# lmb-freiburg/understanding_flow_robustness

Measured on AMD Instinct MI355X. Metric: attack-iters/s, higher is better.
Workload: dtype f32

## Files before the change

include/ufr_hip.h:

```cpp
#ifndef UFR_HIP_H_
#define UFR_HIP_H_

#include <stdint.h>

#ifdef __cplusplus
extern "C" {
#endif

#define UFR_ABI_VERSION 9

enum { UFR_F32 = 0, UFR_F64 = 1, UFR_F16 = 2 };
enum {
  UFR_OK = 0,
  UFR_EINVAL = -1,
  UFR_EUNSUPPORTED = -2,
  UFR_ELAUNCH = -3
};

typedef void* ufr_stream_t;

int ufr_abi_version(void);
const char* ufr_last_error(void);
int ufr_device_count(void);
const char* ufr_build_manifest(void);
// ... 233 lines not shown
                    ufr_stream_t stream);
int ufr_window_gather(const float* src, float* dst, const int* win, int n_win, int N, int C, int Hs, int Ws,
                      int wh, int ww, int level_stride, int margin, ufr_stream_t stream);
int ufr_window_gather_pair(const float* a, const float* b, float* xw, const int* win, float* zero, int N, int C, int Hs, int Ws,
                           int wh, int ww, ufr_stream_t stream);
int ufr_attack_place(const float* patch, const float* mask_p, const float* patch_init, const int* origins, const int* origins_host,
                     float* patch_dst, float* mask_dst, float* init_dst, float* loaded_dst, int* origins_dst, float* state, int B,
                     int H, int W, int ph, int pw, const ufr_cone_chain* chain, int win_h, int win_w, int* win, int* band_win,
                     int band_width, int band_reach, int corr_width, int corr_reach, ufr_stream_t stream);
int ufr_window_scatter(const float* src, float* dst, const int* win, int n_win, int N, int C, int Hd, int Wd,
                       int wh, int ww, int level_stride, int margin, ufr_stream_t stream);

int ufr_corr_backward_window(const float* input1, const float* input2, const float* grad_output,
                             float* grad_input1, float* grad_input2, int B, int C, int H, int W, int patch,
                             int dilation_patch, const int* win, int level_stride, int wh, int ww,
                             ufr_stream_t stream);

int ufr_bias_leaky_forward(float* x, const float* bias, int B, int C, long HW, float slope, ufr_stream_t stream);
int ufr_leaky_backward(const float* y, const float* grad_y, float* grad_x, long total, float slope,
                       ufr_stream_t stream);

long ufr_conv3x3_c2_workspace_floats(int B, int Cin, int H, int W);
int ufr_conv3x3_c2_forward(const float* x, const float* weight, const float* bias, float* y, float* workspace,
                           int B, int Cin, int H, int W, ufr_stream_t stream);
int ufr_conv3x3_c2_backward_data(const float* grad_y, const float* weight, float* grad_x, int B, int Cin, int H,
                                 int W, ufr_stream_t stream);
int ufr_deconv4x4s2_c2_forward(const float* x, const float* weight, const float* bias, float* y, int B, int H, int W,
                               ufr_stream_t stream);
int ufr_deconv4x4s2_c2_backward_data(const float* grad_y, const float* weight, float* grad_x, int B, int H, int W,
                                     ufr_stream_t stream);

int ufr_affine_resample_f64(const double* src, double* dst, int C, int Hs, int Ws, int Hd, int Wd,
                            double m00, double m01, double m10, double m11, double off0, double off1,
                            int order, ufr_stream_t stream);
int ufr_patch_place(const double* patch, const double* mask, const double* init, int C, int h, int w,
                    float* canvas_patch, float* canvas_mask, float* canvas_init, int H, int W, int y, int x,
                    ufr_stream_t stream);
int ufr_patch_crop_f64(const float* canvas, const float* factor, double* dst, int C, int H, int W, int y,
                       int x, int h, int w, ufr_stream_t stream);

int ufr_resample_u8_horizontal(const unsigned char* src, unsigned char* dst, int H, int Ws, int Wd, int C, int flip,
                               const int* bounds, const int* kk, int ksize, ufr_stream_t stream);
int ufr_resample_u8_vertical(const unsigned char* src, unsigned char* dst, int Hs, int Hd, int W, int C,
                             const int* bounds, const int* kk, int ksize, ufr_stream_t stream);
int ufr_u8_to_tensor(const unsigned char* src, float* dst, int H, int W, int C, int crop_y, int crop_x, int crop_h,
                     int crop_w, float divisor, ufr_stream_t stream);
int ufr_kitti_flow_decode(const unsigned short* src, float* dst, int H, int W, ufr_stream_t stream);

int ufr_host_png_unfilter(const unsigned char* data, unsigned char* out, int rows, int stride, int bpp);

#define UFR_IGEMM_MAX_TAPS 25
typedef struct {
  int ntaps, oy0, ox0;
  long w_off;
  signed char dy[UFR_IGEMM_MAX_TAPS], dx[UFR_IGEMM_MAX_TAPS];
} ufr_igemm_phase;
typedef struct {
  const void* x; long x_plane_stride; int in_chunk0, KC;
  int B, Hi, Wi, in_sy, in_sx;
  const int* in_x0; int in_x0_stride, in_x0_div, in_xw;
  const void* w; long w_plane_stride; int Npad, N;
  int Hr, Wr;
  const int* row_x0; int row_x0_stride, row_x0_div;
  int Ho, Wo, out_sy, out_sx;
  int nphase;
  ufr_igemm_phase phase[4];
  int act; const float* bias; float slope;
  const float* add; int add_chunk0;
  const void* mask; int mask_chunk0;
  void* out_planes; long out_plane_stride; int out_chunk0;
  float* out_f32; int out_f32_chunk0;
  float* tail; int tail_n0, tail_accumulate;
  int splitk; float* ws;
  int products;
  int variant;
  int k_order;
  float* out_rowmajor; long out_ld;
  int planes_chunks, f32_first_chunk;
  int no_reduce;
  int* tickets;
} ufr_igemm_desc;
int ufr_igemm(const ufr_igemm_desc* d, ufr_stream_t stream);
typedef struct {
  const void* x; long x_plane_stride; int in_chunk0, C;
  const void* gy; long gy_plane_stride; int g_chunk0, N;
  int B, Hi, Wi, Ho, Wo, kh, kw, sy, sx, py, px;
  float* dw;
  float* db;
  int accumulate;
  int splitm; float* ws; long ws_elems;
  int products;
} ufr_igemm_wgrad_desc;
int ufr_igemm_wgrad(const ufr_igemm_wgrad_desc* d, ufr_stream_t stream);
int ufr_igemm_wgrad_dilated(const ufr_igemm_wgrad_desc* d, int dy, int dx, ufr_stream_t stream);
int ufr_igemm_variant_fallbacks(void);
int ufr_igemm_clock_probe(unsigned long long* buf, int capacity_workgroups);
int ufr_rowmajor_to_planes(const float* src, long ld, long rows, int cols, float scale, void* planes, long plane_stride, int chunk0,
                           long plane_rows, ufr_stream_t stream);
int ufr_nchw_to_planes(const float* x, void* planes, long plane_stride, int chunk0, int B, int C, int H, int W,
                       float scale, float slope, const float* bias, ufr_stream_t stream);
int ufr_window_scatter_planes(const float* src, void* planes, long plane_stride, int chunk0, const int* win, int n_win,
                              int N, int C, int Hd, int Wd, int wh, int ww, int level_stride, int margin,
                              ufr_stream_t stream);
int ufr_window_features_planes(const void* c2w, long c2w_stride, const void* c3w, long c3w_stride, void* cat2, long cat2_stride,
                               void* c3a, long c3a_stride, void* c3b, long c3b_stride, float* c3_nchw, float* c3w_nchw,
                               const int* win, int B, int H, int W, int wh, int ww, int m2, int m3, ufr_stream_t stream);
int ufr_chunks_to_nchw(const void* planes, long plane_stride, const float* f32, int chunk0, const void* mask,
                       int mask_chunk0, float* out, int B, int C, int H, int W, float scale, float slope,
                       ufr_stream_t stream);
int ufr_nchw_cat_to_planes(const float* const* srcs, const int* channels, const int* dst_channel0, int nseg, void* planes,
                           long plane_stride, int chunk0, int chunks, int B, int H, int W, ufr_stream_t stream);
int ufr_chunks_to_nchw_cat(const float* g, int chunk0, int chunks, float* const* dsts, const int* channels, const int* src_channel0,
                           int nseg, const float* act0, float pos0, float neg0, int B, int H, int W, ufr_stream_t stream);
int ufr_grad_finalize(const float* g, int g_chunk0, const void* mask, int mask_chunk0, void* out, long out_plane_stride,
                      int out_chunk0, long M, int chunks, float slope, ufr_stream_t stream);

int ufr_conv1_direct(const float* frames_a, const float* frames_b, int Ba, int Bb, int H, int W, const double* mean,
                     const void* wimg, const float* bias, float slope, void* out_planes, long plane_stride, int out_chunk0,
                     ufr_stream_t stream);
int ufr_conv1_pack_planes(const float* frames_a, const float* frames_b, void* planes, long plane_stride, int Ba, int Bb, int H,
                          int W, const double* mean, ufr_stream_t stream);
int ufr_conv1_unpack_grad(const float* G, float* grad_frames, int N, int H, int W, ufr_stream_t stream);
int ufr_unshuffle_pack_planes(const float* x, void* planes, long plane_stride, int N, int C, int H, int W, ufr_stream_t stream);
int ufr_unshuffle_unpack_grad(const float* G, float* grad_x, int N, int C, int H, int W, ufr_stream_t stream);
int ufr_nchw_grad_to_planes(const float* grad, const float* act, void* planes, long plane_stride, int chunk0, int B, int C, int H,
                            int W, float slope, ufr_stream_t stream);
int ufr_window_gather_chunks(const float* src, float* dst, const int* win, int n_win, int N, int N_dst, int chunks, int Hs, int Ws,
                             int wh, int ww, int level_stride, int margin, ufr_stream_t stream);

int ufr_normalize_frames(const float* frames_a, const float* frames_b, float* out, int Ba, int Bb, int C, int H, int W,
                         const double* mean, ufr_stream_t stream);

int ufr_corr_forward_planes_window(const void* f1_planes, const void* f2_planes, long in_plane_stride, void* out_planes,
                                   long out_plane_stride, int out_chunk0, int B, int C, int H, int W, int patch,
                                   int dilation_patch, float scale, float slope, const int* win, int level_stride,
                                   int win_cells, ufr_stream_t stream);

int ufr_corr_forward_planes_changed(const void* f1_planes, const void* f2_planes, long in_plane_stride, void* out_planes,
                                    long out_plane_stride, int out_chunk0, int B, int C, int H, int W, int patch,
                                    int dilation_patch, float scale, float slope, const int* win, int level_stride,
                                    int win_cells_h, int win_cells_w, int margin, ufr_stream_t stream);

int ufr_corr_backward_window_fused(const float* f1, const float* f2, const float* G, int g_chunk0, float g_scale,
                                   const float* G_redir, float* grad_window, int B, int C, int H, int W, int patch,
                                   int dilation_patch, const int* win, int level_stride, int wh, int ww, int margin,
                                   ufr_stream_t stream);

int ufr_corr_forward_planes(const void* f1_planes, const void* f2_planes, long in_plane_stride, void* out_planes,
                            long out_plane_stride, int out_chunk0, int B, int C, int H, int W, int patch,
                            int dilation_patch, float scale, float slope, ufr_stream_t stream);
int ufr_flow_head_planes_forward(const void* planes, long plane_stride, int chunk0, int chunks, const float* wpk, int w_chunks,
                                 const float* bias, float* out, int B, int H, int W, ufr_stream_t stream);
int ufr_flow_head_planes_forward_mfma(const void* planes, long plane_stride, int chunk0, int chunks, const void* wmf, int w_chunks,
                                      const float* bias, float* out, int B, int H, int W, ufr_stream_t stream);
int ufr_deconv_flow_tail_backward_mfma(const void* grad_planes, long plane_stride, int chunk0, int chunks, const void* wmf,
                                       int w_chunks, float* G, int g_chunks, int out_chunk, int B, int H, int W, ufr_stream_t stream);
int ufr_flow_head_planes_backward(const float* grad_y, const float* wpk, int w_chunks, float* G, int g_chunks, int chunk0, int chunks,
                                  int B, int H, int W, int accumulate, ufr_stream_t stream);
int ufr_flow_head_planes_backward_finalize(const float* grad_y, const float* wpk, int w_chunks, float* G, int g_chunks, int chunk0,
                                           int chunks, int B, int H, int W, int accumulate, const void* mask_planes, void* out_planes,
                                           long out_plane_stride, int fin_chunk0, int fin_chunks, float slope, ufr_stream_t stream);
#define UFR_PF_REGION_BAND 1
#define UFR_PF_REGION_WINDOW 2
int ufr_flow_head_planes_backward_regions(const float* grad_y, const float* wpk, int w_chunks, float* G, int g_chunks, int chunk0,
                                          int chunks, int B, int H, int W, int accumulate, int head_chunks, int region,
                                          const int* origin, int origin_stride, int origin_div, int reg_h, int reg_w, int margin,
// ... 70 lines not shown
```

understanding_flow_robustness_amd/_lib.py:

```python
from __future__ import annotations

import ctypes as C
import os

import torch

_HERE = os.path.dirname(os.path.abspath(__file__))
LIB_PATH = os.environ.get("UFR_HIP_LIB") or os.path.join(_HERE, "lib", "libufr_hip.so")
UFR_F32, UFR_F64, UFR_F16 = 0, 1, 2
ABI_VERSION = 9
_lib = None


class CorrParams(C.Structure):
    _fields_ = [(n, C.c_int) for n in (
        "kH", "kW", "patchH", "patchW", "padH", "padW", "dilationH", "dilationW",
        "dilation_patchH", "dilation_patchW", "dH", "dW")]


UFR_MAX_LEVELS = 8


class Pyramid(C.Structure):
    _fields_ = [("num_levels", C.c_int),
                ("vol", C.c_void_p * UFR_MAX_LEVELS),
                ("grad_vol", C.c_void_p * UFR_MAX_LEVELS),
                ("Hl", C.c_int * UFR_MAX_LEVELS),
                ("Wl", C.c_int * UFR_MAX_LEVELS)]


class AltCorrLevels(C.Structure):
    _fields_ = [("num_levels", C.c_int), ("fmap2", C.c_void_p * 4), ("fmap2_grad", C.c_void_p * 4),
                ("H2", C.c_int * 4), ("W2", C.c_int * 4), ("coord_scale", C.c_float * 4)]


class AltCorrPlaneLevels(C.Structure):
    _fields_ = [("num_levels", C.c_int), ("planes", C.c_void_p * 4), ("plane_stride", C.c_long * 4),
                ("H2", C.c_int * 4), ("W2", C.c_int * 4), ("coord_scale", C.c_float * 4)]


UFR_IGEMM_MAX_TAPS = 25


class IgemmPhase(C.Structure):
    _fields_ = [("ntaps", C.c_int), ("oy0", C.c_int), ("ox0", C.c_int), ("w_off", C.c_long),
                ("dy", C.c_byte * UFR_IGEMM_MAX_TAPS), ("dx", C.c_byte * UFR_IGEMM_MAX_TAPS)]


class IgemmDesc(C.Structure):
    _fields_ = [("x", C.c_void_p), ("x_plane_stride", C.c_long), ("in_chunk0", C.c_int), ("KC", C.c_int),
                ("B", C.c_int), ("Hi", C.c_int), ("Wi", C.c_int), ("in_sy", C.c_int), ("in_sx", C.c_int),
                ("in_x0", C.c_void_p), ("in_x0_stride", C.c_int), ("in_x0_div", C.c_int), ("in_xw", C.c_int),
                ("w", C.c_void_p), ("w_plane_stride", C.c_long), ("Npad", C.c_int), ("N", C.c_int),
                ("Hr", C.c_int), ("Wr", C.c_int),
                ("row_x0", C.c_void_p), ("row_x0_stride", C.c_int), ("row_x0_div", C.c_int),
                ("Ho", C.c_int), ("Wo", C.c_int), ("out_sy", C.c_int), ("out_sx", C.c_int),
                ("nphase", C.c_int),
                ("phase", IgemmPhase * 4),
                ("act", C.c_int), ("bias", C.c_void_p), ("slope", C.c_float),
                ("add", C.c_void_p), ("add_chunk0", C.c_int),
                ("mask", C.c_void_p), ("mask_chunk0", C.c_int),
                ("out_planes", C.c_void_p), ("out_plane_stride", C.c_long), ("out_chunk0", C.c_int),
                ("out_f32", C.c_void_p), ("out_f32_chunk0", C.c_int),
                ("tail", C.c_void_p), ("tail_n0", C.c_int), ("tail_accumulate", C.c_int),
                ("splitk", C.c_int), ("ws", C.c_void_p),
                ("products", C.c_int), ("variant", C.c_int), ("k_order", C.c_int),
                ("out_rowmajor", C.c_void_p), ("out_ld", C.c_long),
                ("planes_chunks", C.c_int), ("f32_first_chunk", C.c_int), ("no_reduce", C.c_int),
                ("tickets", C.c_void_p)]


UFR_IGEMM_WGRAD_MAX_TAPS = 49


class IgemmWgradDesc(C.Structure):
    _fields_ = [("x", C.c_void_p), ("x_plane_stride", C.c_long), ("in_chunk0", C.c_int), ("C", C.c_int),
                ("gy", C.c_void_p), ("gy_plane_stride", C.c_long), ("g_chunk0", C.c_int), ("N", C.c_int),
                ("B", C.c_int), ("Hi", C.c_int), ("Wi", C.c_int), ("Ho", C.c_int), ("Wo", C.c_int),
                ("kh", C.c_int), ("kw", C.c_int), ("sy", C.c_int), ("sx", C.c_int), ("py", C.c_int), ("px", C.c_int),
                ("dw", C.c_void_p), ("db", C.c_void_p), ("accumulate", C.c_int),
                ("splitm", C.c_int), ("ws", C.c_void_p), ("ws_elems", C.c_long),
                ("products", C.c_int)]


UFR_TRAIN_LOSS_MAX_SCALES = 8


class TrainLossDesc(C.Structure):
    _fields_ = [("gt", C.c_void_p), ("B", C.c_int), ("H", C.c_int), ("W", C.c_int), ("nscale", C.c_int),
                ("pred", C.c_void_p * UFR_TRAIN_LOSS_MAX_SCALES), ("grad", C.c_void_p * UFR_TRAIN_LOSS_MAX_SCALES),
                ("h", C.c_int * UFR_TRAIN_LOSS_MAX_SCALES), ("w", C.c_int * UFR_TRAIN_LOSS_MAX_SCALES),
                ("weight", C.c_double * UFR_TRAIN_LOSS_MAX_SCALES),
                ("kind", C.c_int), ("div_flow", C.c_double),
                ("ws", C.c_void_p), ("ws_elems", C.c_long), ("out", C.c_void_p)]


class AdamwSeg(C.Structure):
    _fields_ = [("p", C.c_void_p), ("g", C.c_void_p), ("m", C.c_void_p), ("v", C.c_void_p), ("n", C.c_long)]


class AdamwHyper(C.Structure):
    _fields_ = [(n, C.c_double) for n in ("lr", "beta1", "beta2", "eps", "weight_decay", "bias1", "bias2")]


class FeatureStatsSeg(C.Structure):
    _fields_ = [("src", C.c_void_p), ("plane_stride", C.c_long), ("pixels", C.c_long), ("kind", C.c_int), ("images", C.c_int),
                ("image0", C.c_int), ("B", C.c_int), ("chunk0", C.c_int), ("channels", C.c_int), ("unleaky", C.c_double),
                ("out_col", C.c_long)]


UFR_FEATURE_STATS_MAX_SEGS = 32
UFR_MAX_CONE_LAYERS = 8
UFR_PF_REGION_BAND, UFR_PF_REGION_WINDOW = 1, 2


class ConeChain(C.Structure):
    _fields_ = [("n_layers", C.c_int),
                ("kernel", C.c_int * UFR_MAX_CONE_LAYERS), ("stride", C.c_int * UFR_MAX_CONE_LAYERS),
                ("pad", C.c_int * UFR_MAX_CONE_LAYERS),
                ("n_taps", C.c_int),
                ("tap_layer", C.c_int * UFR_MAX_CONE_LAYERS), ("tap_margin", C.c_int * UFR_MAX_CONE_LAYERS)]


_vp, _i, _f, _l, _d = C.c_void_p, C.c_int, C.c_float, C.c_long, C.c_double
LOSS_PARTIALS = 1024
SIGNATURES = {
    "ufr_corr_forward": [_vp, _vp, _vp, _i, _i, _i, _i, _i, C.POINTER(CorrParams), _vp],
    "ufr_corr_forward_fused": [_vp, _vp, _vp, _i, _i, _i, _i, _i, C.POINTER(CorrParams), _f, _f, _vp],
    "ufr_corr_backward": [_vp, _vp, _vp, _vp, _vp, _i, _i, _i, _i, _i, C.POINTER(CorrParams), _vp],
    "ufr_altcorr_forward": [_vp, _vp, _vp, _vp, _i, _i, _i, _i, _i, _i, _i, _i, _vp],
    "ufr_altcorr_backward": [_vp, _vp, _vp, _vp, _vp, _vp, _vp, _i, _i, _i, _i, _i, _i, _i, _i, _vp],
    "ufr_corr_lookup_forward": [C.POINTER(Pyramid), _vp, _vp, _i, _i, _i, _i, _vp],
    "ufr_corr_lookup_backward": [C.POINTER(Pyramid), _vp, _vp, _i, _i, _i, _i, _vp],
    "ufr_resample2d_forward": [_vp, _vp, _vp, _i, _i, _i, _i, _i, _i, _i, _i, _vp],
    "ufr_resample2d_backward_owner": [_vp, _vp, _vp, _vp, _vp, _vp, _l, _i, _i, _i, _i, _vp],
    "ufr_resample2d_backward": [_vp, _vp, _vp, _vp, _vp, _i, _i, _i, _i, _i, _i, _i, _i, _vp],
    "ufr_channelnorm_forward": [_vp, _vp, _i, _i, _i, _i, _i, _vp],
    "ufr_channelnorm_backward": [_vp, _vp, _vp, _vp, _i, _i, _i, _i, _i, _vp],
    "ufr_patch_paste": [_vp, _vp, _vp, _vp, _vp, _vp, _i, _i, _l, _l, _i, _f, _f, _vp],
    "ufr_patch_update": [_vp, _vp, _vp, _vp, _vp, _vp, _vp, _vp, _i, _i, _l, _l, _f, _f, _f, _f, _vp, _vp],
    "ufr_attack_gate": [_vp, _vp, _f, _vp],
    "ufr_gru_gates_forward": [_vp, _vp, _vp, _vp, _i, _i, _i, _l, _vp],
    "ufr_gru_gates_backward": [_vp, _vp, _vp, _vp, _vp, _vp, _i, _i, _i, _l, _vp],
    "ufr_gru_blend_forward": [_vp, _vp, _vp, _vp, _l, _vp],
    "ufr_gru_blend_backward": [_vp, _vp, _vp, _vp, _vp, _vp, _vp, _l, _vp],
    "ufr_flow_loss_ex": [_vp, _vp, _vp, _vp, _i, _i, _i, _i, _f, _vp, _vp, _vp],
    "ufr_universal_update": [_vp, _vp, _vp, _vp, _vp, _vp, _vp, _vp, _i, _i, _f, _f, _f, _f, _i, _i, _i, _i,
                             _i, _vp],
    "ufr_flow_loss": [_vp, _vp, _vp, _vp, _i, _i, _i, _f, _vp, _vp],
    "ufr_flow2_upsampled_loss": [_vp, _f, _vp, _vp, _vp, _i, _i, _i, _i, _f, _vp, _vp],
    "ufr_patch_grad_crop": [_vp, _vp, _vp, _vp, _vp, _vp, _vp, _i, _i, _i, _i, _i, _i, _vp],
    "ufr_patch_apply": [_vp, _i, _vp, _vp, _i, _i, _f, _f, _vp, _vp],
    "ufr_patch_grad_crop_window": [_vp, _vp, _vp, _vp, _vp, _vp, _i, _i, _i, _i, _i, _i, _i, _i, _vp],
    "ufr_patch_paste_placed_rect": [_vp, _vp, _vp, _vp, _vp, _vp, _vp, _i, _i, _i, _i, _i, _i, _f, _f, _vp, _vp],
    "ufr_patch_paste_placed": [_vp, _vp, _vp, _vp, _vp, _vp, _vp, _vp, _vp, _i, _i, _i, _i, _i, _i, _f, _f, _vp, _vp],
    "ufr_cone_window": [_vp, _i, _l, _i, _i, _i, C.POINTER(ConeChain), _i, _i, _vp, _vp, _vp],
    "ufr_attack_place": [_vp, _vp, _vp, _vp, _vp, _vp, _vp, _vp, _vp, _vp, _vp, _i, _i, _i, _i, _i, C.POINTER(ConeChain), _i, _i,
                         _vp, _vp, _i, _i, _i, _i, _vp],
    "ufr_attack_load_frames": [_vp, _vp, _vp, _vp, _vp, _vp, _vp, _vp, _vp, _i, _i, _i, _i, _i, _vp],
    "ufr_patch_mask_placed": [_vp, _vp, _vp, _i, _i, _i, _i, _i, _vp],
    "ufr_patch_grad_crop_packed": [_vp, _vp, _vp, _vp, _vp, _vp, _i, _i, _i, _i, _i, _i, _i, _i, _vp],
    "ufr_patch_apply_paste_rect": [_vp, _i, _vp, _vp, _vp, _vp, _vp, _vp, _vp, _vp, _i, _i, _i, _i, _i, _f, _f, _i, _f, _f, _vp, _vp],
    "ufr_window_gather_pair": [_vp, _vp, _vp, _vp, _vp, _i, _i, _i, _i, _i, _i, _vp],
    "ufr_window_features_planes": [_vp, _l, _vp, _l, _vp, _l, _vp, _l, _vp, _l, _vp, _vp, _vp, _i, _i, _i, _i, _i, _i, _i, _vp],
    "ufr_window_gather": [_vp, _vp, _vp, _i, _i, _i, _i, _i, _i, _i, _i, _i, _vp],
    "ufr_window_scatter": [_vp, _vp, _vp, _i, _i, _i, _i, _i, _i, _i, _i, _i, _vp],
    "ufr_conv1_pack_planes": [_vp, _vp, _vp, _l, _i, _i, _i, _i, _vp, _vp],
    "ufr_conv1_unpack_grad": [_vp, _vp, _i, _i, _i, _vp],
    "ufr_nchw_grad_to_planes": [_vp, _vp, _vp, _l, _i, _i, _i, _i, _i, _f, _vp],
    "ufr_window_gather_chunks": [_vp, _vp, _vp, _i, _i, _i, _i, _i, _i, _i, _i, _i, _i, _vp],
    "ufr_normalize_frames": [_vp, _vp, _vp, _i, _i, _i, _i, _i, _vp, _vp],
    "ufr_corr_backward_window_fused": [_vp, _vp, _vp, _i, _f, _vp, _vp, _i, _i, _i, _i, _i, _i, _vp, _i, _i, _i, _i, _vp],
    "ufr_corr_backward_window": [_vp, _vp, _vp, _vp, _vp, _i, _i, _i, _i, _i, _i, _vp, _i, _i, _i, _vp],
    "ufr_bias_leaky_forward": [_vp, _vp, _i, _i, _l, _f, _vp],
    "ufr_leaky_backward": [_vp, _vp, _vp, _l, _f, _vp],
    "ufr_conv3x3_c2_forward": [_vp, _vp, _vp, _vp, _vp, _i, _i, _i, _i, _vp],
    "ufr_conv3x3_c2_backward_data": [_vp, _vp, _vp, _i, _i, _i, _i, _vp],
    "ufr_deconv4x4s2_c2_forward": [_vp, _vp, _vp, _vp, _i, _i, _i, _vp],
    "ufr_deconv4x4s2_c2_backward_data": [_vp, _vp, _vp, _i, _i, _i, _vp],
    "ufr_pwc_warp_forward": [_vp, _vp, _vp, _i, _i, _i, _i, _vp],
    "ufr_pwc_warp_backward": [_vp, _vp, _vp, _vp, _vp, _i, _i, _i, _i, _vp],
    "ufr_pwc_warp_backward_owner": [_vp, _vp, _vp, _vp, _vp, _vp, _l, _i, _i, _i, _i, _vp],
    "ufr_raft_normalize_pair": [_vp, _vp, _vp, _l, _vp],
    "ufr_raft_normalize_pair_backward": [_vp, _vp, _vp, _l, _vp],
    "ufr_raft_fmap_pyramid_forward": [_vp, _vp, _i, _i, _i, _i, _i, _vp],
    "ufr_raft_fmap_pyramid_backward": [_vp, _i, _vp, _i, _i, _i, _i, _vp],
    "ufr_raft_context_split_forward": [_vp, _vp, _vp, _i, _i, _i, _l, _vp],
    "ufr_raft_context_split_backward": [_vp, _vp, _vp, _vp, _vp, _i, _i, _i, _l, _vp],
    "ufr_igemm": [C.POINTER(IgemmDesc), _vp],
    "ufr_igemm_wgrad": [C.POINTER(IgemmWgradDesc), _vp],
    "ufr_igemm_wgrad_dilated": [C.POINTER(IgemmWgradDesc), _i, _i, _vp],
    "ufr_flow_upscale4_forward": [_vp, _vp, _i, _i, _i, _i, _f, _i, _vp],
    "ufr_flow_upscale4_backward": [_vp, _vp, _i, _i, _i, _i, _f, _i, _vp],
    "ufr_fn2_stage_pack": [_vp, _vp, _vp, _vp, _i, _i, _i, _f, _vp],
    "ufr_fn2_stage_unpack_grad": [_vp, _vp, _vp, _vp, _i, _i, _i, _vp],
    "ufr_fn2_stage_finish_grad": [_vp, _vp, _vp, _vp, _vp, _i, _i, _i, _f, _vp],
    "ufr_fn2_fusion_pack": [_vp, _vp, _vp, _vp, _vp, _vp, _i, _i, _i, _vp],
    "ufr_fn2_fusion_unpack_grad": [_vp, _vp, _vp, _vp, _vp, _vp, _vp, _vp, _vp, _i, _i, _i, _vp],
    "ufr_fn2_fusion_finish_grad": [_vp, _vp, _vp, _vp, _vp, _vp, _vp, _i, _i, _i, _vp],
    "ufr_rowmajor_to_planes": [_vp, _l, _l, _i, _f, _vp, _l, _i, _l, _vp],
    "ufr_nchw_to_planes": [_vp, _vp, _l, _i, _i, _i, _i, _i, _f, _f, _vp, _vp],
    "ufr_window_scatter_planes": [_vp, _vp, _l, _i, _vp, _i, _i, _i, _i, _i, _i, _i, _i, _i, _vp],
    "ufr_chunks_to_nchw": [_vp, _l, _vp, _i, _vp, _i, _vp, _i, _i, _i, _i, _f, _f, _vp],
    "ufr_nchw_cat_to_planes": [_vp, _vp, _vp, _i, _vp, _l, _i, _i, _i, _i, _i, _vp],
    "ufr_chunks_to_nchw_cat": [_vp, _i, _i, _vp, _vp, _vp, _i, _vp, _f, _f, _i, _i, _i, _vp],
    "ufr_grad_finalize": [_vp, _i, _vp, _i, _vp, _l, _i, _l, _i, _f, _vp],
    "ufr_flow_head_planes_forward": [_vp, _l, _i, _i, _vp, _i, _vp, _vp, _i, _i, _i, _vp],
    "ufr_flow_head_planes_forward_mfma": [_vp, _l, _i, _i, _vp, _i, _vp, _vp, _i, _i, _i, _vp],
    "ufr_deconv_flow_tail_backward_mfma": [_vp, _l, _i, _i, _vp, _i, _vp, _i, _i, _i, _i, _i, _vp],
    "ufr_flow_head_planes_backward": [_vp, _vp, _i, _vp, _i, _i, _i, _i, _i, _i, _i, _vp],
    "ufr_flow_head_planes_backward_finalize": [_vp, _vp, _i, _vp, _i, _i, _i, _i, _i, _i, _i, _vp, _vp, _l, _i, _i, _f, _vp],
    "ufr_flow_head_planes_backward_regions": [_vp, _vp, _i, _vp, _i, _i, _i, _i, _i, _i, _i, _i, _i, _vp, _i, _i, _i, _i, _i, _vp, _i,
                                              _vp, _vp, _l, _i, _i, _f, _vp],
    "ufr_unshuffle_pack_planes": [_vp, _vp, _l, _i, _i, _i, _i, _vp],
    "ufr_unshuffle_unpack_grad": [_vp, _vp, _i, _i, _i, _i, _vp],
    "ufr_conv3x3s2_c3_planes": [_vp, _vp, _vp, _f, _vp, _l, _i, _i, _i, _i, _i, _vp],
    "ufr_conv3x3_c16_planes": [_vp, _l, _i, _vp, _vp, _f, _vp, _l, _i, _i, _i, _i, _vp],
    "ufr_cm_norm_stats": [_vp, _vp, _vp, _l, _i, _i, _f, _vp],
    "ufr_cm_norm_apply": [_vp, _vp, _vp, _l, _i, _vp, _l, _i, _l, _i, _i, _i, _i, _vp],
    "ufr_cm_norm_stats_apply": [_vp, _vp, _vp, _f, _vp, _l, _i, _vp, _l, _i, _l, _i, _i, _i, _i, _vp],
    "ufr_cm_norm_backward": [_vp, _vp, _vp, _i, _vp, _vp, _vp, _vp, _l, _i, _l, _i, _i, _i, _vp],
    "ufr_cm_masked_copy": [_vp, _vp, _l, _vp, _l, _vp],
    "ufr_raft_flow_patches": [_vp, _vp, _l, _i, _i, _i, _i, _vp],
    "ufr_raft_motion_finish_slabs": [_vp, _i, _i, _i, _vp, _f, _vp, _l, _vp, _l, _i, _vp, _i, _i, _i, _vp],
    "ufr_raft_motion_finish": [_vp, _l, _vp, _l, _i, _vp, _i, _i, _i, _vp],
    "ufr_raft_coords_step": [_vp, _vp, _vp, _vp, _vp, _l, _vp],
    "ufr_grad_finalize_consume": [_vp, _vp, _vp, _l, _l, _i, _f, _vp],
    "ufr_gru_gates_cm_forward": [_vp, _vp, _l, _i, _vp, _l, _i, _l, _i, _vp],
    "ufr_gru_gates_cm_forward_slabs": [_vp, _i, _i, _vp, _vp, _vp, _vp, _l, _i, _vp, _l, _i, _l, _i, _vp],
    "ufr_gru_blend_cm_forward_slabs": [_vp, _i, _i, _vp, _vp, _vp, _vp, _vp, _l, _i, _vp, _l, _i, _l, _i, _vp],
    "ufr_gru_blend_cm_forward": [_vp, _vp, _vp, _l, _i, _vp, _l, _i, _l, _i, _vp],
    "ufr_gru_blend_cm_backward": [_vp, _vp, _vp, _l, _i, _vp, _vp, _l, _i, _vp, _vp, _l, _i, _vp, _vp],
    "ufr_gru_gates_cm_backward": [_vp, _vp, _l, _i, _vp, _vp, _vp, _l, _i, _vp, _l, _i, _i, _vp, _vp],
    "ufr_altcorr_pyramid_forward": [_vp, _vp, _vp, _vp, _i, _i, _i, _i, _i, _f, _vp],
    "ufr_altcorr_pyramid_backward": [_vp, _vp, _vp, _vp, _vp, _vp, _i, _i, _i, _i, _i, _f, _i, _vp],
    "ufr_altcorr_pyramid_backward_cm": [_vp, _vp, _vp, _vp, _vp, _vp, _i, _i, _i, _i, _i, _f, _i, _vp],
    "ufr_upfeat_planes_forward_mfma": [_vp, _l, _i, _i, _vp, _i, _vp, _vp, _i, _i, _i, _vp],
    "ufr_upfeat_planes_backward": [_vp, _vp, _i, _vp, _i, _i, _i, _i, _i, _i, _i, _vp],
    "ufr_flow_up_planes_forward": [_vp, _vp, _vp, _vp, _l, _i, _i, _i, _i, _vp],
    "ufr_flow_up_planes_backward": [_vp, _i, _vp, _vp, _i, _i, _i, _i, _vp],
    "ufr_corr_forward_planes_changed": [_vp, _vp, _l, _vp, _l, _i, _i, _i, _i, _i, _i, _i, _f, _f, _vp, _i, _i, _i, _i, _vp],
    "ufr_corr_forward_planes_window": [_vp, _vp, _l, _vp, _l, _i, _i, _i, _i, _i, _i, _i, _f, _f, _vp, _i, _i, _vp],
    "ufr_corr_forward_planes": [_vp, _vp, _l, _vp, _l, _i, _i, _i, _i, _i, _i, _i, _f, _f, _vp],
    "ufr_convex_upsample_forward": [_vp, _vp, _vp, _i, _i, _i, _vp],
    "ufr_convex_upsample_backward": [_vp, _vp, _vp, _vp, _vp, _vp, _i, _i, _i, _vp],
    "ufr_affine_resample_f64": [_vp, _vp, _i, _i, _i, _i, _i, _d, _d, _d, _d, _d, _d, _i, _vp],
    "ufr_patch_place": [_vp, _vp, _vp, _i, _i, _i, _vp, _vp, _vp, _i, _i, _i, _i, _vp],
    "ufr_patch_crop_f64": [_vp, _vp, _vp, _i, _i, _i, _i, _i, _i, _i, _vp],
    "ufr_resample_u8_horizontal": [_vp, _vp, _i, _i, _i, _i, _i, _vp, _vp, _i, _vp],
    "ufr_resample_u8_vertical": [_vp, _vp, _i, _i, _i, _i, _vp, _vp, _i, _vp],
    "ufr_u8_to_tensor": [_vp, _vp, _i, _i, _i, _i, _i, _i, _i, _f, _vp],
    "ufr_kitti_flow_decode": [_vp, _vp, _i, _i, _vp],
    "ufr_host_png_unfilter": [_vp, _vp, _i, _i, _i],
    "ufr_igemm_clock_probe": [_vp, _i],
    "ufr_altcorr_planes_prepare": [_vp, _vp, _l, _l, _i, _vp],
    "ufr_altcorr_planes_forward": [_vp, _l, C.POINTER(AltCorrPlaneLevels), _vp, _vp, _i, _i, _i, _i, _i, _f, _vp],
    "ufr_conv1_direct": [_vp, _vp, _i, _i, _i, _i, _vp, _vp, _vp, _f, _vp, _l, _i, _vp],
    "ufr_train_loss": [C.POINTER(TrainLossDesc), _vp],
    "ufr_grad_norm": [C.POINTER(AdamwSeg), _i, _f, _vp, _l, _vp, _vp],
    "ufr_adamw_step": [C.POINTER(AdamwSeg), _i, C.POINTER(AdamwHyper), _vp, _vp],
    "ufr_sweep_paste": [_vp, _vp, _vp, _vp, _vp, _vp, _vp, _vp, _i, _i, _i, _i, _i, _f, _f, C.POINTER(ConeChain), _i, _i, _vp, _vp, _vp],
    "ufr_sweep_metrics": [_vp, _vp, _vp, _vp, _vp, _i, _i, _i, _i, _i, _i, _i, _i, _vp, _l, _vp, _i, _i, _vp],
    "ufr_feature_stats": [C.POINTER(FeatureStatsSeg), _i, _vp, _l, _vp, _i, _l, _l, _vp],
    "ufr_abs_sums": [_vp, _vp, _l, _vp, _l, _vp, _vp],
    "ufr_momentum_update": [_vp, _vp, _vp, _vp, _vp, _vp, _vp, _vp, _vp, _vp, _i, _i, _f, _f, _f, _f, _f, _f, _i, _i, _vp],
    "ufr_diverse_table_check": [_vp, _i, _i, _i],
    "ufr_diverse_forward": [_vp, _vp, _vp, _vp, _vp, _vp, _i, _i, _i, _i, _vp, _i, _vp, _vp, _vp, _l, _vp],
    "ufr_diverse_backward": [_vp, _vp, _vp, _vp, _i, _i, _i, _vp, _i, _vp, _vp],
    "ufr_step_advance": [_vp, _vp],
}
DIVERSE_COLS = 8
PLAIN = {"ufr_abi_version": (C.c_int, []), "ufr_last_error": (C.c_char_p, []),
# ... 276 lines not shown
```

understanding_flow_robustness_amd/csrc/igemm.hip:

```cpp
#include <atomic>
#include <cstdlib>

#include "ufr_common.h"

namespace {

typedef __attribute__((ext_vector_type(8))) __bf16 bf16x8;
typedef __attribute__((ext_vector_type(4))) float f32x4;
typedef __attribute__((ext_vector_type(4))) unsigned u32x4;

constexpr int BM = 128, BN = 128, BK = 32;
__device__ constexpr int PROD_A[6] = {2, 0, 1, 1, 0, 0};
__device__ constexpr int PROD_B[6] = {0, 2, 1, 0, 1, 0};

struct RowGeom {
  int B, Hr, Wr, M;
  const int* row_x0;
  int row_x0_stride, row_x0_div;
  int Ho, Wo, out_sy, out_sx;
};

__device__ __forceinline__ void split3(float v, __bf16& a, __bf16& b, __bf16& c) {
  a = (__bf16)v;
  const float r1 = v - (float)a;
// ... 74 lines not shown
    }
#pragma unroll
    for (int j = 0; j < 8; ++j) {
      v[j] += (n0 + j < e.N) ? e.bias[n0 + j] : 0.f;
      v[j] = v[j] > 0.f ? v[j] : v[j] * e.slope;
    }
  } else {
    if (e.add) {
      const float* ap = e.add + (long)e.add_chunk0 * e.Mout * 32 + cm;
      const float4 a0 = *reinterpret_cast<const float4*>(ap), a1 = *reinterpret_cast<const float4*>(ap + 4);
      v[0] += a0.x; v[1] += a0.y; v[2] += a0.z; v[3] += a0.w; v[4] += a1.x; v[5] += a1.y; v[6] += a1.z; v[7] += a1.w;
    }
    if (e.mask) {
      const bf16x8 m = *reinterpret_cast<const bf16x8*>(e.mask + (long)e.mask_chunk0 * e.Mout * 32 + cm);
#pragma unroll
      for (int j = 0; j < 8; ++j) v[j] = ((float)m[j] > 0.f) ? v[j] : v[j] * e.slope;
    }
  }
#pragma unroll
  for (int j = 0; j < 8; ++j)
    if (n0 + j >= e.N) v[j] = 0.f;
  if (e.out_rm && n0 < e.N) {
    float* op = e.out_rm + pout * e.out_ld + n0;
    *reinterpret_cast<float4*>(op) = make_float4(v[0], v[1], v[2], v[3]);
    *reinterpret_cast<float4*>(op + 4) = make_float4(v[4], v[5], v[6], v[7]);
  }
  if (e.out_f32 && (n0 >> 5) >= e.f32_first_chunk) {
    float* op = e.out_f32 + (long)e.out_f32_chunk0 * e.Mout * 32 + cm;
    *reinterpret_cast<float4*>(op) = make_float4(v[0], v[1], v[2], v[3]);
    *reinterpret_cast<float4*>(op + 4) = make_float4(v[4], v[5], v[6], v[7]);
  }
  if (e.out_planes && (n0 >> 5) < e.planes_chunks) {
    bf16x8 q0, q1, q2;
#pragma unroll
    for (int j = 0; j < 8; ++j) {
      __bf16 x, y, z;
      split3(v[j], x, y, z);
      q0[j] = x; q1[j] = y; q2[j] = z;
    }
    __bf16* o = e.out_planes + (long)e.out_chunk0 * e.Mout * 32 + cm;
    if (e.nostore) {
      asm volatile("" ::"v"(q0), "v"(q1), "v"(q2), "v"(o));
      return;
    }
    *reinterpret_cast<bf16x8*>(o) = q0;
    *reinterpret_cast<bf16x8*>(o + e.out_plane_stride) = q1;
    *reinterpret_cast<bf16x8*>(o + 2 * e.out_plane_stride) = q2;
  }
}

__device__ __forceinline__ void xcd_tile(int swz, int& bx, int& by, int& bz) {
  bx = blockIdx.x; by = blockIdx.y; bz = blockIdx.z;
  if (!swz) return;
  const int nx = gridDim.x, nxy = nx * gridDim.y, n = nxy * gridDim.z;
  const int orig = (bz * gridDim.y + by) * nx + bx;
  const int q = n / 8, r = n % 8, xcd = orig % 8, idx = orig / 8;
  const int w = (xcd < r ? xcd * (q + 1) : r * (q + 1) + (xcd - r) * q) + idx;
  bz = w % gridDim.z;
  const int rem = w / gridDim.z;
  by = rem / nx;
  bx = rem - by * nx;
}

struct Phase {
  int ntaps, oy0, ox0;
  long w_off;
  int dyx[UFR_IGEMM_MAX_TAPS];
  int run[UFR_IGEMM_MAX_TAPS];
};

struct Args {
  const __bf16* x; long x_plane_stride; int in_chunk0, KC;
  int Hi, Wi, in_sy, in_sx;
  const int* in_x0; int in_x0_stride, in_x0_div, in_xw;
  const __bf16* w; long w_plane_stride; int Npad;
  RowGeom g;
  Epilogue e;
  int nphase, splitk, xcd;
  int korder;
  int per_k, sk[4], zoff[4];
  float* ws;
  int* tickets;
  int skip_out;
  Phase ph[4];
};

__device__ __forceinline__ void sum_slabs(const float* src, long sstride, int S, float (&v)[8]) {
#pragma unroll
  for (int j = 0; j < 8; ++j) v[j] = 0.f;
  int s = 0;
  for (; s + 8 <= S; s += 8) {
    float4 lo[8], hi[8];
#pragma unroll
    for (int u = 0; u < 8; ++u) {
      lo[u] = *reinterpret_cast<const float4*>(src + (s + u) * sstride);
      hi[u] = *reinterpret_cast<const float4*>(src + (s + u) * sstride + 4);
    }
#pragma unroll
    for (int u = 0; u < 8; ++u) {
      v[0] += lo[u].x; v[1] += lo[u].y; v[2] += lo[u].z; v[3] += lo[u].w; v[4] += hi[u].x; v[5] += hi[u].y; v[6] += hi[u].z; v[7] += hi[u].w;
    }
  }
  if (S - s >= 5) {
    float4 lo[7], hi[7];
#pragma unroll
    for (int u = 0; u < 7; ++u) {
      const int su = min(s + u, S - 1);
      lo[u] = *reinterpret_cast<const float4*>(src + su * sstride);
      hi[u] = *reinterpret_cast<const float4*>(src + su * sstride + 4);
    }
#pragma unroll
    for (int u = 0; u < 7; ++u)
      if (s + u < S) {
        v[0] += lo[u].x; v[1] += lo[u].y; v[2] += lo[u].z; v[3] += lo[u].w; v[4] += hi[u].x; v[5] += hi[u].y; v[6] += hi[u].z; v[7] += hi[u].w;
      }
    s = S;
  }
  for (; s + 4 <= S; s += 4) {
    float4 lo[4], hi[4];
#pragma unroll
    for (int u = 0; u < 4; ++u) {
      lo[u] = *reinterpret_cast<const float4*>(src + (s + u) * sstride);
      hi[u] = *reinterpret_cast<const float4*>(src + (s + u) * sstride + 4);
    }
#pragma unroll
    for (int u = 0; u < 4; ++u) {
      v[0] += lo[u].x; v[1] += lo[u].y; v[2] += lo[u].z; v[3] += lo[u].w; v[4] += hi[u].x; v[5] += hi[u].y; v[6] += hi[u].z; v[7] += hi[u].w;
    }
  }
  for (; s < S; ++s) {
    const float4 lo = *reinterpret_cast<const float4*>(src + s * sstride), hi = *reinterpret_cast<const float4*>(src + s * sstride + 4);
    v[0] += lo.x; v[1] += lo.y; v[2] += lo.z; v[3] += lo.w; v[4] += hi.x; v[5] += hi.y; v[6] += hi.z; v[7] += hi.w;
  }
}

template <int NPL, int MT, int WGR, int BNT>
__device__ __forceinline__ void igemm_write_out(const Args& a, const Phase& ph, f32x4 (&acc)[MT][4], float* lds_f32, int* flag, int z, int phase,
                                                int tile_id, int bm0, int bm, int bn0, int bn, int wrow, int wcol, int lane, int wave) {
  if (a.skip_out) {
    float keep = 0.f;
#pragma unroll
    for (int m = 0; m < MT; ++m)
#pragma unroll
      for (int n = 0; n < 4; ++n) keep += acc[m][n][0] + acc[m][n][1] + acc[m][n][2] + acc[m][n][3];
    if (keep == 1.2345678e-30f && a.ws) a.ws[0] = keep;
    return;
  }
  if (a.splitk > 1) {
    float* slab = a.ws + (long)z * a.g.M * a.Npad;
#pragma unroll
    for (int m = 0; m < MT; ++m)
#pragma unroll
      for (int j = 0; j < 4; ++j) {
        const int row = bm + wrow + m * 16 + (lane >> 4) * 4 + j;
        if (row < a.g.M) {
#pragma unroll
          for (int n = 0; n < 4; ++n) slab[(long)row * a.Npad + bn + wcol + n * 16 + (lane & 15)] = acc[m][n][j];
        }
      }
    if (!a.tickets) return;
    asm volatile("s_waitcnt vmcnt(0)" ::: "memory");
    __syncthreads();
    if (threadIdx.x == 0) {
      __builtin_amdgcn_fence(__ATOMIC_RELEASE, "agent");
      asm volatile("s_waitcnt vmcnt(0)" ::: "memory");
      const int S = a.sk[phase];
      const int t = __hip_atomic_fetch_add(a.tickets + tile_id, 1, __ATOMIC_RELAXED, __HIP_MEMORY_SCOPE_AGENT);
      const int last = t == S - 1;
      if (last) {
        __hip_atomic_store(a.tickets + tile_id, 0, __ATOMIC_RELAXED, __HIP_MEMORY_SCOPE_AGENT);
        __builtin_amdgcn_fence(__ATOMIC_ACQUIRE, "agent");
        asm volatile("s_waitcnt vmcnt(0)" ::: "memory");
      }
      *flag = last;
    }
    __syncthreads();
    if (!*flag) return;
    const float* base = a.ws + (long)a.zoff[phase] * a.g.M * a.Npad;
    const long sstride = (long)a.g.M * a.Npad;
    const int S = a.sk[phase];
    for (int it = threadIdx.x; it < WGR * (BNT / 8); it += blockDim.x) {
      const int r = it / (BNT / 8), n0 = bn0 + (it - r * (BNT / 8)) * 8, row = bm0 + r;
      if (row >= a.g.M || n0 >= a.e.Nchunks32 * 32) continue;
      float v[8];
      sum_slabs(base + (long)row * a.Npad + n0, sstride, S, v);
      epilogue_store8(a.e, out_pixel(a.g, row, ph.oy0, ph.ox0), n0, v);
    }
    return;
  }
  {
    constexpr int TS = 68;
    float* tw = lds_f32 + wave * (32 * TS);
#pragma unroll
    for (int pass = 0; pass < MT / 2; ++pass) {
      __syncthreads();
#pragma unroll
      for (int mm = 0; mm < 2; ++mm)
#pragma unroll
        for (int n = 0; n < 4; ++n)
#pragma unroll
          for (int j = 0; j < 4; ++j)
            tw[(mm * 16 + (lane >> 4) * 4 + j) * TS + n * 16 + (lane & 15)] = acc[pass * 2 + mm][n][j];
      __syncthreads();
#pragma unroll
      for (int it = 0; it < 4; ++it) {
        const int item = it * 64 + lane, r = item >> 3, g8 = item & 7;
        const int row = bm + wrow + pass * 32 + r;
        if (row < a.g.M) {
          const float4 lo = *reinterpret_cast<const float4*>(tw + r * TS + g8 * 8), hi = *reinterpret_cast<const float4*>(tw + r * TS + g8 * 8 + 4);
          float v[8] = {lo.x, lo.y, lo.z, lo.w, hi.x, hi.y, hi.z, hi.w};
          epilogue_store8(a.e, out_pixel(a.g, row, ph.oy0, ph.ox0), bn + wcol + g8 * 8, v);
        }
      }
    }
  }
}

__device__ __attribute__((aligned(64))) unsigned ufr_zero_page[16];

__device__ unsigned long long* ufr_clock_probe_buf = nullptr;
__device__ int ufr_clock_probe_cap = 0;

__device__ __forceinline__ void glds16(const __bf16* src, __bf16* lds_wave_base) {
  __builtin_amdgcn_global_load_lds(src, lds_wave_base, 16, 0, 0);
}

template <int BM_, int BN_, bool PIPE_ = false, bool BUF_ = false, int NP_ = 6>
__global__ __launch_bounds__(256) __attribute__((amdgpu_waves_per_eu(PIPE_ ? 2 : (BM_ == 64 ? 4 : 3), PIPE_ ? 2 : (BM_ == 64 ? 4 : 3)))) void igemm_glds_kernel(const Args a) {
  static_assert(!(PIPE_ && BUF_), "the buffer-resource form exists for the single-stage kernel");
  static_assert(NP_ == 6 || NP_ == 3 || NP_ == 1, "six, three or one product");
  constexpr int NPL = NP_ == 6 ? 3 : (NP_ == 3 ? 2 : 1), FIRST = 6 - NP_;
  constexpr int MT = (BN_ == 128 && BM_ == 128) ? 4 : 2;
// ... 116 lines not shown
    for (int n = 0; n < 4; ++n) acc[m][n] = f32x4{0.f, 0.f, 0.f, 0.f};
  const int frow = lane & 15;
  const int foff = frow * BK + ((((lane >> 4)) ^ ((frow >> 1) & 3)) << 3);

  if (kt0 < kt1) set_tap(tap);
  if constexpr (PIPE_) {
    if (kt0 < kt1) {
      stage_A(0);
      stage_B();
    }
    for (int kt = kt0; kt < kt1; ++kt) {
      const int cur = (kt - kt0) & 1;
      asm volatile("s_waitcnt vmcnt(0)" ::: "memory");
      __builtin_amdgcn_s_barrier();
      __builtin_amdgcn_s_setprio(2);
      const __bf16* sA = lds_all + (cur ? STAGE : 0);
      bf16x8 fa[NPL][MT], fb[4][NPL];
#pragma unroll
      for (int p = 0; p < NPL; ++p) {
#pragma unroll
        for (int m = 0; m < MT; ++m) fa[p][m] = *reinterpret_cast<const bf16x8*>(sA + p * (BM_ * BK) + (wrow + m * 16) * BK + foff);
#pragma unroll
        for (int n = 0; n < 4; ++n) fb[n][p] = *reinterpret_cast<const bf16x8*>(&ldsB[p][(wcol + n * 16) * BK + foff]);
      }
      if (kt + 1 < kt1) stage_A(cur ? 0 : STAGE);
      asm volatile("s_waitcnt lgkmcnt(0)" ::: "memory");
      __builtin_amdgcn_s_barrier();
      if (kt + 1 < kt1) stage_B();
      __builtin_amdgcn_s_setprio(0);
#pragma unroll
      for (int n = 0; n < 4; ++n)
#pragma unroll
        for (int t = FIRST; t < 6; ++t)
#pragma unroll
          for (int m = 0; m < MT; ++m)
            acc[m][n] = __builtin_amdgcn_mfma_f32_16x16x32_bf16(fa[PROD_A[t]][m], fb[n][PROD_B[t]], acc[m][n], 0, 0, 0);
    }
  } else
  for (int kt = kt0; kt < kt1; ++kt) {
    __syncthreads();
    stage_tile();
    __syncthreads();
    bf16x8 fa[NPL][MT];
#pragma unroll
    for (int p = 0; p < NPL; ++p)
#pragma unroll
      for (int m = 0; m < MT; ++m)
        fa[p][m] = *reinterpret_cast<const bf16x8*>(&ldsA[p][(wrow + m * 16) * BK + foff]);
#pragma unroll
    for (int n = 0; n < 4; ++n) {
      bf16x8 fb[NPL];
#pragma unroll
      for (int p = 0; p < NPL; ++p) fb[p] = *reinterpret_cast<const bf16x8*>(&ldsB[p][(wcol + n * 16) * BK + foff]);
#pragma unroll
      for (int t = FIRST; t < 6; ++t)
#pragma unroll
        for (int m = 0; m < MT; ++m)
          acc[m][n] = __builtin_amdgcn_mfma_f32_16x16x32_bf16(fa[PROD_A[t]][m], fb[PROD_B[t]], acc[m][n], 0, 0, 0);
    }
  }
  static_assert(PIPE_ ? 4 * 32 * 68 * 4 <= STAGE * 2 : true, "epilogue staging does not fit");
  igemm_write_out<NPL, MT, BM_, BN_>(a, ph, acc, reinterpret_cast<float*>(lds_all), reinterpret_cast<int*>(lds_all), z, phase,
                                     (phase * gridDim.y + ty) * gridDim.x + tx, bm, bm, bn, bn, wrow, wcol, lane, wave);
}
constexpr int PIPE_LDS_BYTES = (3 * (128 + 128) * BK + 3 * 128 * BK) * 2;

constexpr int PP_IMG = 3 * 128 * BK;
constexpr int pp_lds_bytes(int bn) { return (4 * PP_IMG + 2 * 3 * bn * BK) * 2; }

template <int BN_, bool BUF_ = false, int NP_ = 6>
__global__ __launch_bounds__(512) __attribute__((amdgpu_waves_per_eu(2, 2))) void igemm_pp_kernel(const Args a) {
  static_assert(NP_ == 6 || NP_ == 3 || NP_ == 1, "six, three or one product");
  constexpr int NPL = NP_ == 6 ? 3 : (NP_ == 3 ? 2 : 1), FIRST = 6 - NP_;
  constexpr int MT = BN_ == 128 ? 4 : 2, BPT = BN_ / 64;
  constexpr int PP_IMG_B = 3 * BN_ * BK;
  extern __shared__ __attribute__((aligned(16))) __bf16 lds_pp[];
  unsigned long long* const probe = ufr_clock_probe_buf;
  const unsigned long long probe_c0 = probe ? __builtin_amdgcn_s_memtime() : 0, probe_r0 = probe ? __builtin_amdgcn_s_memrealtime() : 0;
  const int tid = threadIdx.x & 255, lane = tid & 63;
  const int wave = __builtin_amdgcn_readfirstlane(tid >> 6);
  const int grp = __builtin_amdgcn_readfirstlane(threadIdx.x >> 8);
  const int wrow = BN_ == 128 ? (wave >> 1) * 64 : wave * 32, wcol = BN_ == 128 ? (wave & 1) * 64 : 0;
  int tx, ty, z;
  xcd_tile(a.xcd, tx, ty, z);
  const int bm = ty * 256 + grp * 128, bn = tx * BN_;
  int phase = 0;
#pragma unroll
  for (int p = 1; p < 4; ++p)
    if (p < a.nphase && z >= a.zoff[p]) phase = p;
  const int ks = z - a.zoff[phase];
  const Phase& ph = a.ph[phase];
  const int KC = a.KC, KT = ph.ntaps * KC;
  const int kt0 = ks * a.per_k, kt1 = min(KT, kt0 + a.per_k);
  const int nk = max(kt1 - kt0, 0);
  const long Min = (long)a.g.B * a.Hi * a.Wi;
  const long cstride = Min * 32;

  const int srow0 = tid >> 2, sch = tid & 3;
  const int csw = sch ^ ((srow0 >> 1) & 3);
  int yb[2], xb[2], xlo[2], xhi[2];
  long ibase[2];
#pragma unroll
  for (int i = 0; i < 2; ++i) {
    const int pm = bm + srow0 + 64 * i;
    const int hw = a.g.Hr * a.g.Wr;
    const int b = pm / hw, r = pm - b * hw, yr = r / a.g.Wr, xr = r - yr * a.g.Wr;
    const bool live = pm < a.g.M;
    const int bb = live ? b : 0;
    const int xg = xr + (a.g.row_x0 ? a.g.row_x0[bb * a.g.row_x0_stride] / a.g.row_x0_div : 0);
    yb[i] = live ? yr * a.in_sy : -(1 << 20);
    xb[i] = xg * a.in_sx;
    ibase[i] = (long)bb * a.Hi * a.Wi;
    xlo[i] = a.in_x0 ? a.in_x0[bb * a.in_x0_stride] / a.in_x0_div : 0;
    xhi[i] = a.in_x0 ? min(a.Wi, xlo[i] + a.in_xw) : a.Wi;
    xlo[i] = max(xlo[i], 0);
  }
  const __bf16* gx = a.x + (long)a.in_chunk0 * cstride + csw * 8;
  const __bf16* zero = reinterpret_cast<const __bf16*>(ufr_zero_page);
  int tap = a.korder ? kt0 % ph.ntaps : kt0 / KC, kc = a.korder ? kt0 / ph.ntaps : kt0 - tap * KC;
  const __bf16* wp = a.w + ph.w_off + ((long)kt0 * a.Npad + bn + srow0) * BK + csw * 8;
  const long wstep = (long)a.Npad * BK;
  const __bf16* xk = gx + (long)kc * cstride;
  bool ok[2];
  long aoff[2];
  unsigned voff[2];
  const unsigned rowbase[2] = {(unsigned)(ibase[0] * 64 + csw * 16), (unsigned)(ibase[1] * 64 + csw * 16)};
  __amdgpu_buffer_rsrc_t rsrc = __builtin_amdgcn_make_buffer_rsrc(const_cast<__bf16*>(a.x), 0, (int)min(6L * a.x_plane_stride, 0x7fffffffL),
                                                                   0x00020000);
  long xkoff = (long)(a.in_chunk0 + kc) * cstride;
  auto set_tap = [&](int t) {
    const int dyx = ph.dyx[t], dyo = (int)(short)(dyx & 0xffff), dxo = dyx >> 16;
#pragma unroll
    for (int i = 0; i < 2; ++i) {
      const int yi = yb[i] + dyo, xi = xb[i] + dxo;
      ok[i] = (unsigned)yi < (unsigned)a.Hi && xi >= xlo[i] && xi < xhi[i];
      if (BUF_) voff[i] = ok[i] ? rowbase[i] + (unsigned)(yi * a.Wi + xi) * 64u : 0x80000000u;
      else aoff[i] = ok[i] ? (ibase[i] + (long)yi * a.Wi + xi) * 32 : 0;
    }
  };
  const int imgA0 = grp * 2 * PP_IMG, imgB0 = 4 * PP_IMG;
  auto stage_A = [&](int img) {
#pragma unroll
    for (int i = 0; i < 2; ++i)
#pragma unroll
      for (int p = 0; p < NPL; ++p) {
        if (BUF_) {
          typedef __attribute__((address_space(3))) void* lds_void;
          __builtin_amdgcn_raw_ptr_buffer_load_lds(rsrc, (lds_void)(lds_pp + img + p * (128 * BK) + (64 * i + wave * 16) * BK), 16, (int)voff[i],
                                                   (unsigned)((xkoff + p * a.x_plane_stride) * 2), 0, 0);
        } else {
          const __bf16* src = ok[i] ? xk + aoff[i] + p * a.x_plane_stride : zero;
          glds16(src, lds_pp + img + p * (128 * BK) + (64 * i + wave * 16) * BK);
        }
      }
    if (a.korder) {
      if (++tap == ph.ntaps) {
        tap = 0;
        xk += cstride;
        xkoff += cstride;
      }
      set_tap(tap);
    } else {
      xk += cstride;
      xkoff += cstride;
      if (++kc == KC) {
        kc = 0;
        xk = gx;
        xkoff = (long)a.in_chunk0 * cstride;
        if (++tap < ph.ntaps) set_tap(tap);
      }
    }
  };
  auto stage_B = [&](int img) {
#pragma unroll
    for (int i = 0; i < BPT; ++i)
#pragma unroll
      for (int p = 0; p < NPL; ++p)
        glds16(wp + p * a.w_plane_stride + (long)(64 * i) * BK, lds_pp + img + p * (BN_ * BK) + (64 * i + wave * 16) * BK);
    wp += wstep;
  };

  f32x4 acc[MT][4];
#pragma unroll
  for (int m = 0; m < MT; ++m)
#pragma unroll
    for (int n = 0; n < 4; ++n) acc[m][n] = f32x4{0.f, 0.f, 0.f, 0.f};
  const int frow = lane & 15;
  const int foff = frow * BK + ((((lane >> 4)) ^ ((frow >> 1) & 3)) << 3);

  if (nk > 0) {
    set_tap(tap);
    stage_A(imgA0);
    if (grp == 0) stage_B(imgB0);
  }
  if (grp == 1) {
    asm volatile("s_waitcnt vmcnt(0)" ::: "memory");
    __builtin_amdgcn_s_barrier();
  }
  const unsigned long long probe_c2 = probe ? __builtin_amdgcn_s_memtime() : 0;
  for (int i = 0; i < nk; ++i) {
    const int cur = i & 1;
    asm volatile("s_waitcnt vmcnt(0)" ::: "memory");
    __builtin_amdgcn_s_barrier();
    __builtin_amdgcn_s_setprio(2);
    const __bf16* sA = lds_pp + imgA0 + cur * PP_IMG;
    const __bf16* sB = lds_pp + imgB0 + cur * PP_IMG_B;
    bf16x8 fa[NPL][MT], fb[4][NPL];
#pragma unroll
    for (int p = 0; p < NPL; ++p) {
#pragma unroll
      for (int m = 0; m < MT; ++m) fa[p][m] = *reinterpret_cast<const bf16x8*>(sA + p * (128 * BK) + (wrow + m * 16) * BK + foff);
#pragma unroll
      for (int n = 0; n < 4; ++n) fb[n][p] = *reinterpret_cast<const bf16x8*>(sB + p * (BN_ * BK) + (wcol + n * 16) * BK + foff);
    }
    if (i + 1 < nk) {
      stage_A(imgA0 + (cur ^ 1) * PP_IMG);
      if (grp == 0) stage_B(imgB0 + (cur ^ 1) * PP_IMG_B);
    }
    asm volatile("s_waitcnt lgkmcnt(0)" ::: "memory");
    __builtin_amdgcn_s_setprio(0);
    __builtin_amdgcn_s_barrier();
#pragma unroll
    for (int n = 0; n < 4; ++n)
#pragma unroll
      for (int t = FIRST; t < 6; ++t)
#pragma unroll
        for (int m = 0; m < MT; ++m)
          acc[m][n] = __builtin_amdgcn_mfma_f32_16x16x32_bf16(fa[PROD_A[t]][m], fb[n][PROD_B[t]], acc[m][n], 0, 0, 0);
  }
  if (grp == 0) __builtin_amdgcn_s_barrier();
  const unsigned long long probe_c3 = probe ? __builtin_amdgcn_s_memtime() : 0;
  static_assert(4 * 32 * 68 * 4 <= 2 * PP_IMG * 2, "epilogue staging does not fit a group's activation images");
  igemm_write_out<NPL, MT, 256, BN_>(a, ph, acc, reinterpret_cast<float*>(lds_pp + imgA0), reinterpret_cast<int*>(lds_pp), z, phase,
                                     (phase * gridDim.y + ty) * gridDim.x + tx, ty * 256, bm, bn, bn, wrow, wcol, lane, wave);
  if (probe && threadIdx.x == 0) {
    const int wg = (blockIdx.z * gridDim.y + blockIdx.y) * gridDim.x + blockIdx.x;
    if (wg < ufr_clock_probe_cap) {
      unsigned long long* o = probe + 8L * wg;
      o[0] = probe_c0; o[1] = __builtin_amdgcn_s_memtime(); o[2] = probe_r0; o[3] = __builtin_amdgcn_s_memrealtime();
      o[4] = probe_c2; o[5] = probe_c3; o[6] = __builtin_amdgcn_s_getreg((4 << 0) | (0 << 6) | (31 << 11)); o[7] = (unsigned long long)nk;
    }
  }
}

constexpr int PP3_ROWS = 144;
constexpr int PP3_IMG = 3 * PP3_ROWS * BK;
constexpr int pp3_lds_bytes(int bn) { return (4 * PP3_IMG + 2 * 3 * bn * BK) * 2; }

template <int BN_>
__global__ __launch_bounds__(512) __attribute__((amdgpu_waves_per_eu(2, 2))) void igemm_pp3_kernel(const Args a) {
  constexpr int NPL = 3, MT = BN_ == 128 ? 4 : 2, BPT = BN_ / 64, PP_IMG_B = 3 * BN_ * BK;
  extern __shared__ __attribute__((aligned(16))) __bf16 lds_pp[];
  const int tid = threadIdx.x & 255, lane = tid & 63, wave = __builtin_amdgcn_readfirstlane(tid >> 6);
  const int grp = __builtin_amdgcn_readfirstlane(threadIdx.x >> 8);
  const int wrow = BN_ == 128 ? (wave >> 1) * 64 : wave * 32, wcol = BN_ == 128 ? (wave & 1) * 64 : 0;
  int tx, ty, z;
  xcd_tile(a.xcd, tx, ty, z);
  const int bm = ty * 256 + grp * 128, bn = tx * BN_;
  int phase = 0;
#pragma unroll
  for (int p = 1; p < 4; ++p)
    if (p < a.nphase && z >= a.zoff[p]) phase = p;
  const int ks = z - a.zoff[phase];
  const Phase& ph = a.ph[phase];
  const int ntaps = ph.ntaps, KT = ntaps * a.KC;
  const int kt0 = ks * a.per_k, kt1 = min(KT, kt0 + a.per_k);
  const int nk = max(kt1 - kt0, 0);
  const long Min = (long)a.g.B * a.Hi * a.Wi;
  const long cstride = Min * 32;
  const int Wr = a.g.Wr, hw = a.g.Hr * Wr;

  const int srow0 = tid >> 2, sch = tid & 3;
  const int csw = sch ^ ((srow0 >> 1) & 3);
  const int xrow = lane >> 2, cswx = sch ^ ((xrow >> 1) & 3);
  int yb[3], xb[3], xlo[3], xhi[3];
  long ibase[3];
  auto cell_geometry = [&](int i, long cell, int xr_override) {
    const bool live = cell >= 0 && cell < a.g.M;
    const int c = live ? (int)cell : 0;
    const int b = c / hw, r = c - b * hw, yr = r / Wr;
    const int xr = xr_override >= 0 ? xr_override : r - yr * Wr;
    const int xg = xr + (a.g.row_x0 ? a.g.row_x0[b * a.g.row_x0_stride] / a.g.row_x0_div : 0);
    yb[i] = live ? yr * a.in_sy : -(1 << 20);
    xb[i] = xg * a.in_sx;
    ibase[i] = (long)b * a.Hi * a.Wi;
    xlo[i] = a.in_x0 ? a.in_x0[b * a.in_x0_stride] / a.in_x0_div : 0;
    xhi[i] = a.in_x0 ? min(a.Wi, xlo[i] + a.in_xw) : a.Wi;
    xlo[i] = max(xlo[i], 0);
  };
  cell_geometry(0, (long)bm + srow0, -1);
  cell_geometry(1, (long)bm + srow0 + 64, -1);
  const int grow0 = bm / Wr;
  if (xrow < 2) {
    cell_geometry(2, (long)bm + 128 + xrow, -1);
  } else {
    const int e = (xrow - 2) >> 1, w = (xrow - 2) & 1;
    const long rowcell = (long)(grow0 + e) * Wr;
    cell_geometry(2, rowcell < a.g.M ? rowcell : -1, Wr + w);
  }
  const __bf16* gx = a.x + (long)a.in_chunk0 * cstride + csw * 8;
  const __bf16* gxx = a.x + (long)a.in_chunk0 * cstride + cswx * 8;
  const __bf16* zero = reinterpret_cast<const __bf16*>(ufr_zero_page);
  const __bf16* wp = a.w + ph.w_off + ((long)kt0 * a.Npad + bn + srow0) * BK + csw * 8;
  const long wstep = (long)a.Npad * BK;

  const int imgA0 = grp * 2 * PP3_IMG, imgB0 = 4 * PP3_IMG;
  auto stage_A = [&](int img, int kc, int tap) {
    const int dyx = ph.dyx[tap], dyo = (int)(short)(dyx & 0xffff), dxo = (dyx >> 16) - (ph.run[tap] & 3) * a.in_sx;
    const long coff = (long)kc * cstride;
#pragma unroll
    for (int i = 0; i < 2; ++i) {
      const int yi = yb[i] + dyo, xi = xb[i] + dxo;
      const bool ok = (unsigned)yi < (unsigned)a.Hi && xi >= xlo[i] && xi < xhi[i];
      const long off = ok ? (ibase[i] + (long)yi * a.Wi + xi) * 32 + coff : 0;
#pragma unroll
      for (int p = 0; p < NPL; ++p)
        glds16(ok ? gx + off + p * a.x_plane_stride : zero, lds_pp + img + p * (PP3_ROWS * BK) + (64 * i + wave * 16) * BK);
// ... 103 lines not shown
  const int H = a.Hi, W = a.Wi;
  const int tiles_x = (W + TW - 1) / TW, tiles_y = (H + TH - 1) / TH;
  int t;
  {
    const int n = gridDim.x, orig = blockIdx.x, q = n / 8, r = n % 8, xcd = orig % 8, idx = orig / 8;
    t = (xcd < r ? xcd * (q + 1) : r * (q + 1) + (xcd - r) * q) + idx;
  }
  const int b = t / (tiles_x * tiles_y), rem = t - b * tiles_x * tiles_y, y0 = (rem / tiles_x) * TH, x0 = (rem % tiles_x) * TW;
  const Phase& ph = a.ph[0];
  const long Min = (long)a.g.B * H * W;
  const __bf16* zero = reinterpret_cast<const __bf16*>(ufr_zero_page);

  f32x4 acc[MTW];
#pragma unroll
  for (int m = 0; m < MTW; ++m) acc[m] = f32x4{0.f, 0.f, 0.f, 0.f};
  const int pi = lane & 15, kgrp = lane >> 4;
  for (int kc = 0; kc < a.KC; ++kc) {
    __syncthreads();
    for (int blk = wave; blk < 3 * HBLK; blk += 4) {
      const int p = blk / HBLK, hb = blk - p * HBLK;
      const int hp = hb * 16 + (lane >> 2), slot = lane & 3;
      const int hy = hp / HW_, hx = hp - hy * HW_;
      const int gy = y0 - 1 + hy, gx = x0 - 1 + hx;
      const bool ok = hp < HPIX && (unsigned)gy < (unsigned)H && (unsigned)gx < (unsigned)W;
      const int piece = slot ^ ((hp >> 1) & 3);
      const __bf16* src = ok ? a.x + (long)p * a.x_plane_stride + ((long)(a.in_chunk0 + kc) * Min + ((long)b * H + gy) * W + gx) * BK + piece * 8 : zero;
      glds16(src, sH + ((long)p * HROWS + hb * 16) * BK);
    }
    bf16x8 wr[9][3];
    const __bf16* wl = a.w + ph.w_off + ((long)kc * 9 * a.Npad + nt * 16 + pi) * BK + kgrp * 8;
#pragma unroll
    for (int tt = 0; tt < 9; ++tt)
#pragma unroll
      for (int p = 0; p < 3; ++p) wr[tt][p] = *reinterpret_cast<const bf16x8*>(wl + (long)p * a.w_plane_stride + (long)tt * a.Npad * BK);
    asm volatile("s_waitcnt vmcnt(0)" ::: "memory");
    __syncthreads();
#pragma unroll
    for (int tt = 0; tt < 9; ++tt) {
      const int dyx = ph.dyx[tt], dy = (int)(short)(dyx & 0xffff), dx = dyx >> 16;
#pragma unroll
      for (int m = 0; m < MTW; ++m) {
        const int g = pg * MTW + m;
        const int hp = ((g >> 1) + dy + 1) * HW_ + 16 * (g & 1) + pi + dx + 1;
        const int off = hp * BK + ((kgrp ^ ((hp >> 1) & 3)) << 3);
        bf16x8 fa[3];
#pragma unroll
        for (int p = 0; p < 3; ++p) fa[p] = *reinterpret_cast<const bf16x8*>(sH + p * (HROWS * BK) + off);
#pragma unroll
        for (int q = 0; q < 6; ++q) acc[m] = __builtin_amdgcn_mfma_f32_16x16x32_bf16(fa[PROD_A[q]], wr[tt][PROD_B[q]], acc[m], 0, 0, 0);
      }
    }
  }
  constexpr int TS = 20;
  __syncthreads();
  float* tw = reinterpret_cast<float*>(lds_d33) + wave * (MTW * 16 * TS);
#pragma unroll
  for (int m = 0; m < MTW; ++m)
#pragma unroll
    for (int j = 0; j < 4; ++j) tw[(m * 16 + kgrp * 4 + j) * TS + pi] = acc[m][j];
  __syncthreads();
  const int G8 = NT == 1 ? max(2, a.e.Nchunks32 * 4) : 2;
  for (int it = lane; it < MTW * 16 * G8; it += 64) {
    const int r = it / G8, g8 = it - r * G8, g = pg * MTW + (r >> 4);
    const int y = y0 + (g >> 1), x = x0 + 16 * (g & 1) + (r & 15);
    if (y < H && x < W) {
      float v[8] = {0.f, 0.f, 0.f, 0.f, 0.f, 0.f, 0.f, 0.f};
      if (g8 < 2) {
        const float4 lo = *reinterpret_cast<const float4*>(tw + r * TS + g8 * 8), hi = *reinterpret_cast<const float4*>(tw + r * TS + g8 * 8 + 4);
        v[0] = lo.x; v[1] = lo.y; v[2] = lo.z; v[3] = lo.w; v[4] = hi.x; v[5] = hi.y; v[6] = hi.z; v[7] = hi.w;
      }
      epilogue_store8(a.e, ((long)b * H + y) * W + x, nt * 16 + g8 * 8, v);
    }
  }
}

template <int NT>
constexpr int d33_lds_bytes() {
  constexpr int HROWS = ((6 * 34 + 15) / 16) * 16, stage = 3 * HROWS * BK * 2, epi = 4 * (2 * NT) * 16 * 20 * 4;
  return stage > epi ? stage : epi;
}

__global__ __launch_bounds__(256) void igemm_reduce_kernel(const Args a) {
  const int n8 = a.Npad / 8;
  const long total = (long)a.nphase * a.g.M * n8;
  for (long i = (long)blockIdx.x * blockDim.x + threadIdx.x; i < total; i += (long)gridDim.x * blockDim.x) {
    const int n0 = (int)(i % n8) * 8;
    const long rest = i / n8;
    const int row = (int)(rest % a.g.M), phase = (int)(rest / a.g.M);
    if (n0 >= a.e.Nchunks32 * 32) continue;
    float v[8];
    sum_slabs(a.ws + ((long)a.zoff[phase] * a.g.M + row) * a.Npad + n0, (long)a.g.M * a.Npad, a.sk[phase], v);
    epilogue_store8(a.e, out_pixel(a.g, row, a.ph[phase].oy0, a.ph[phase].ox0), n0, v);
  }
}

}

extern "C" int ufr_igemm_clock_probe(unsigned long long* buf, int capacity_workgroups) {
  UFR_REQUIRE((buf == nullptr) == (capacity_workgroups == 0) && capacity_workgroups >= 0, "igemm clock probe: buffer and capacity disagree");
  if (hipMemcpyToSymbol(HIP_SYMBOL(ufr_clock_probe_cap), &capacity_workgroups, sizeof(int)) != hipSuccess ||
      hipMemcpyToSymbol(HIP_SYMBOL(ufr_clock_probe_buf), &buf, sizeof(buf)) != hipSuccess)
    return ufr::fail(UFR_ELAUNCH, "igemm clock probe: %s", hipGetErrorString(hipGetLastError()));
  return UFR_OK;
}

namespace {
std::atomic<int> g_variant_fallbacks{0};
}
extern "C" int ufr_igemm_variant_fallbacks(void) { return g_variant_fallbacks.load(); }

extern "C" int ufr_igemm(const ufr_igemm_desc* d, ufr_stream_t stream) {
  UFR_REQUIRE(d, "igemm: null descriptor");
  UFR_REQUIRE(d->x && d->w, "igemm: null operand");
  UFR_REQUIRE(d->B > 0 && d->Hi > 0 && d->Wi > 0 && d->Hr > 0 && d->Wr > 0 && d->Ho > 0 && d->Wo > 0, "igemm: bad grid");
  UFR_REQUIRE(d->KC > 0 && d->in_chunk0 >= 0 && d->N > 0 && d->Npad % 64 == 0 && d->Npad >= d->N, "igemm: bad channel counts");
  UFR_REQUIRE(d->in_sy > 0 && d->in_sx > 0 && d->out_sy > 0 && d->out_sx > 0, "igemm: bad strides");
  UFR_REQUIRE(d->nphase >= 1 && d->nphase <= 4 && d->splitk >= 1 && d->splitk <= 64, "igemm: bad phase / split count");
  UFR_REQUIRE(d->products == 6 || d->products == 3 || d->products == 1, "igemm: products must be 6, 3 or 1");
  UFR_REQUIRE(d->splitk == 1 || d->ws, "igemm: split-K needs a workspace");
  UFR_REQUIRE(!d->no_reduce || (d->splitk > 1 && d->nphase == 1), "igemm: no_reduce is for single-phase split-K launches");
  UFR_REQUIRE(d->out_planes || d->out_f32 || d->out_rowmajor, "igemm: no output");
  UFR_REQUIRE(!d->out_rowmajor || (d->out_ld >= d->N && d->N % 8 == 0 && d->out_ld % 4 == 0), "igemm: bad row-major output");
  UFR_REQUIRE(!d->act || d->bias, "igemm: the forward epilogue needs the bias");
  UFR_REQUIRE(d->planes_chunks >= 0 && d->f32_first_chunk >= 0 && ((d->planes_chunks == 0 && d->f32_first_chunk == 0) || (d->out_planes && d->out_f32)),
              "igemm: planes_chunks / f32_first_chunk need both outputs");
  UFR_REQUIRE(!d->tail || (d->tail_n0 > 0 && d->tail_n0 % 32 == 0 && d->tail_n0 < d->N), "igemm: bad tail column");
  UFR_REQUIRE(!d->row_x0 || (d->row_x0_div > 0), "igemm: bad band divisor");
  UFR_REQUIRE(!d->in_x0 || (d->in_x0_div > 0 && d->in_xw > 0), "igemm: bad input band");
  const long M = (long)d->B * d->Hr * d->Wr;
  UFR_REQUIRE(M < (1L << 30) && (long)d->B * d->Hi * d->Wi < (1L << 30) && (long)d->B * d->Ho * d->Wo < (1L << 30),
              "igemm: too many pixels");
  UFR_REQUIRE((d->Hr - 1) * d->out_sy + 1 <= d->Ho && (d->row_x0 || (d->Wr - 1) * d->out_sx + 1 <= d->Wo),
              "igemm: the row grid does not fit the output grid");
  Args a;
  a.x = static_cast<const __bf16*>(d->x); a.x_plane_stride = d->x_plane_stride; a.in_chunk0 = d->in_chunk0; a.KC = d->KC;
  a.Hi = d->Hi; a.Wi = d->Wi; a.in_sy = d->in_sy; a.in_sx = d->in_sx;
  a.in_x0 = d->in_x0; a.in_x0_stride = d->in_x0_stride; a.in_x0_div = d->in_x0_div; a.in_xw = d->in_xw;
  a.w = static_cast<const __bf16*>(d->w); a.w_plane_stride = d->w_plane_stride; a.Npad = d->Npad;
  a.g.B = d->B; a.g.Hr = d->Hr; a.g.Wr = d->Wr; a.g.M = (int)M;
  a.g.row_x0 = d->row_x0; a.g.row_x0_stride = d->row_x0_stride; a.g.row_x0_div = d->row_x0_div;
  a.g.Ho = d->Ho; a.g.Wo = d->Wo; a.g.out_sy = d->out_sy; a.g.out_sx = d->out_sx;
  a.e.bias = d->bias; a.e.slope = d->slope; a.e.act = d->act;
  a.e.add = d->add; a.e.add_chunk0 = d->add_chunk0;
  a.e.mask = static_cast<const __bf16*>(d->mask); a.e.mask_chunk0 = d->mask_chunk0;
  a.e.out_planes = static_cast<__bf16*>(d->out_planes); a.e.out_plane_stride = d->out_plane_stride; a.e.out_chunk0 = d->out_chunk0;
  a.e.out_f32 = d->out_f32; a.e.out_f32_chunk0 = d->out_f32_chunk0;
  a.e.out_rm = d->out_rowmajor; a.e.out_ld = d->out_ld;
  a.e.planes_chunks = d->planes_chunks > 0 ? d->planes_chunks : (1 << 30); a.e.f32_first_chunk = d->f32_first_chunk;
  a.e.tail = d->tail; a.e.tail_n0 = d->tail_n0; a.e.tail_acc = d->tail_accumulate;
  a.e.Mout = (long)d->B * d->Ho * d->Wo; a.e.N = d->N; a.e.Nchunks32 = (d->N + 31) / 32;
  a.nphase = d->nphase; a.splitk = d->splitk; a.ws = d->ws;
  a.tickets = (d->splitk > 1 && !d->no_reduce) ? d->tickets : nullptr;
  static const int skip_out = [] { const char* e = getenv("UFR_IGEMM_DEBUG_SKIP_EPILOGUE"); return e ? atoi(e) : 0; }();
  a.skip_out = skip_out == 1;
  a.e.nostore = skip_out == 2;
  a.xcd = 1;
  a.korder = d->k_order ? 1 : 0;
  for (int z = 0; z < 4; ++z) {
    const ufr_igemm_phase& p = d->phase[z < d->nphase ? z : 0];
    UFR_REQUIRE(p.ntaps >= 1 && p.ntaps <= UFR_IGEMM_MAX_TAPS && p.w_off >= 0, "igemm: bad phase %d", z);
    UFR_REQUIRE(p.oy0 >= 0 && p.oy0 < d->out_sy && p.ox0 >= 0 && p.ox0 < d->out_sx, "igemm: bad phase offset");
    UFR_REQUIRE(p.w_off + (long)p.ntaps * d->KC * d->Npad * BK <= d->w_plane_stride, "igemm: phase %d weights out of range", z);
    a.ph[z].ntaps = p.ntaps; a.ph[z].oy0 = p.oy0; a.ph[z].ox0 = p.ox0; a.ph[z].w_off = p.w_off;
    for (int t = 0; t < UFR_IGEMM_MAX_TAPS; ++t)
      a.ph[z].dyx[t] = t < p.ntaps ? (int)(((unsigned)(int)p.dy[t] & 0xffffu) | ((unsigned)(int)p.dx[t] << 16)) : 0;
    for (int t = 0; t < UFR_IGEMM_MAX_TAPS; ++t) a.ph[z].run[t] = 1 << 4;
    for (int t = 0; t < p.ntaps;) {
      int len = 1, dir = 0;
      while (len < 3 && t + len < p.ntaps && p.dy[t + len] == p.dy[t]) {
        const int step = p.dx[t + len] - p.dx[t + len - 1];
        if ((step != d->in_sx && step != -d->in_sx) || (dir && step != dir)) break;
        dir = step;
        ++len;
      }
      int dmin = p.dx[t];
      for (int i = 1; i < len; ++i) dmin = p.dx[t + i] < dmin ? p.dx[t + i] : dmin;
      for (int i = 0; i < len; ++i) a.ph[z].run[t + i] = ((p.dx[t + i] - dmin) / d->in_sx) | (i << 2) | (len << 4);
      t += len;
    }
  }
  int ktmax = 0, nz = 0;
  for (int z = 0; z < d->nphase; ++z) ktmax = a.ph[z].ntaps * d->KC > ktmax ? a.ph[z].ntaps * d->KC : ktmax;
  a.per_k = (ktmax + d->splitk - 1) / d->splitk;
  for (int z = 0; z < 4; ++z) {
    a.zoff[z] = nz;
    a.sk[z] = z < d->nphase ? (a.ph[z].ntaps * d->KC + a.per_k - 1) / a.per_k : 0;
    nz += a.sk[z];
  }
  hipStream_t st = ufr::as_stream(stream);
  const int bn = d->Npad % BN == 0 ? BN : 64;
  const dim3 grid(d->Npad / bn, (unsigned)((M + BM - 1) / BM), nz);
  const int variant = d->variant ? d->variant : 2;
  UFR_REQUIRE(variant == 2 || variant == 4 || variant == 5 || variant == 6 || variant == 7 || variant == 8, "igemm: unknown kernel variant %d",
              d->variant);
  const bool use_buf = 6L * d->x_plane_stride < 0x7fffffffL;
  int dev = 0;
  if (hipGetDevice(&dev) != hipSuccess || dev < 0 || dev >= 64) return ufr::fail(UFR_ELAUNCH, "igemm: no current device");
  static std::atomic<bool> raised[64] = {};
  if (!raised[dev].load(std::memory_order_acquire)) {
    hipError_t e = ufr::ensure_dynamic_lds(reinterpret_cast<const void*>(igemm_pp_kernel<128>), pp_lds_bytes(128));
    if (e == hipSuccess) e = ufr::ensure_dynamic_lds(reinterpret_cast<const void*>(igemm_pp_kernel<128, true>), pp_lds_bytes(128));
    if (e == hipSuccess) e = ufr::ensure_dynamic_lds(reinterpret_cast<const void*>(igemm_glds_kernel<128, 128, true>), PIPE_LDS_BYTES);
    if (e == hipSuccess) e = ufr::ensure_dynamic_lds(reinterpret_cast<const void*>(igemm_pp3_kernel<128>), pp3_lds_bytes(128));
    if (e == hipSuccess) e = ufr::ensure_dynamic_lds(reinterpret_cast<const void*>(igemm_pp3_kernel<64>), pp3_lds_bytes(64));
    if (e != hipSuccess) return ufr::fail(UFR_ELAUNCH, "igemm: %s", hipGetErrorString(e));
    raised[dev].store(true, std::memory_order_release);
  }
  bool d33 = variant == 8 && d->nphase == 1 && d->phase[0].ntaps == 9 && d->in_sx == 1 && d->in_sy == 1 && d->out_sx == 1 && d->out_sy == 1 &&
             d->Hr == d->Hi && d->Wr == d->Wi && d->Ho == d->Hi && d->Wo == d->Wi && !d->row_x0 && !d->in_x0 && d->splitk == 1 && !d->tail &&
             !d->out_rowmajor && d->k_order && d->N <= 64 && d->products == 6;
  for (int t = 0; d33 && t < 9; ++t)
    d33 = d->phase[0].dy[t] >= -1 && d->phase[0].dy[t] <= 1 && d->phase[0].dx[t] >= -1 && d->phase[0].dx[t] <= 1;
  if ((variant == 8 && !d33) || (variant == 7 && !(d->k_order && (d->in_sx == 1 || d->in_sx == 2) && d->Wr >= 22 && d->products == 6)))
    g_variant_fallbacks.fetch_add(1);
  if (d33) {
    const int nt = d->N <= 16 ? 1 : (d->N <= 32 ? 2 : 4);
    const int tiles = d->B * ((d->Hi + 3) / 4) * ((d->Wi + 31) / 32);
    hipError_t e = hipSuccess;
#define UFR_D33(NT_)                                                                                                  \
    e = ufr::ensure_dynamic_lds(reinterpret_cast<const void*>(igemm_d33_kernel<NT_>), d33_lds_bytes<NT_>());          \
    if (e == hipSuccess) igemm_d33_kernel<NT_><<<tiles, 256, d33_lds_bytes<NT_>(), st>>>(a)
    if (nt == 1) { UFR_D33(1); } else if (nt == 2) { UFR_D33(2); } else { UFR_D33(4); }
#undef UFR_D33
    if (e != hipSuccess) return ufr::fail(UFR_ELAUNCH, "igemm (direct 3 x 3): %s", hipGetErrorString(e));
    return ufr::launched("igemm_d33_kernel");
  }
  if (d->products != 6) {
    UFR_REQUIRE(use_buf, "igemm: the reduced-product forms need activation planes below 2 GB");
#define UFR_NP_LAUNCH(NP_)                                                                                                    \
    if ((variant == 6 || variant == 7 || variant == 5) && bn == BN) {                                                          \
      const dim3 gpp(d->Npad / BN, (unsigned)((M + 255) / 256), nz);                                                           \
      hipError_t e = ufr::ensure_dynamic_lds(reinterpret_cast<const void*>(igemm_pp_kernel<128, true, NP_>), pp_lds_bytes(128)); \
      if (e != hipSuccess) return ufr::fail(UFR_ELAUNCH, "igemm: %s", hipGetErrorString(e));                                   \
      igemm_pp_kernel<128, true, NP_><<<gpp, 512, pp_lds_bytes(128), st>>>(a);                                                 \
    } else if (variant == 4 && bn == BN) {                                                                                     \
      const dim3 g64(d->Npad / BN, (unsigned)((M + 63) / 64), nz);                                                             \
      igemm_glds_kernel<64, 128, false, true, NP_><<<g64, 256, 0, st>>>(a);                                                    \
    } else if (bn == BN) {                                                                                                     \
      igemm_glds_kernel<128, 128, false, true, NP_><<<grid, 256, 0, st>>>(a);                                                  \
    } else {                                                                                                                   \
      igemm_glds_kernel<128, 64, false, true, NP_><<<grid, 256, 0, st>>>(a);                                                   \
    }
    if (d->products == 3) { UFR_NP_LAUNCH(3) } else { UFR_NP_LAUNCH(1) }
#undef UFR_NP_LAUNCH
  } else
  if (variant == 7 && d->k_order && (d->in_sx == 1 || d->in_sx == 2) && d->Wr >= 22) {
    const dim3 gpp(d->Npad / bn, (unsigned)((M + 255) / 256), nz);
    if (bn == BN) igemm_pp3_kernel<128><<<gpp, 512, pp3_lds_bytes(128), st>>>(a);
    else igemm_pp3_kernel<64><<<gpp, 512, pp3_lds_bytes(64), st>>>(a);
  } else if (variant == 4 && bn == BN) {
    const dim3 g64(d->Npad / BN, (unsigned)((M + 63) / 64), nz);
    if (use_buf) igemm_glds_kernel<64, 128, false, true><<<g64, 256, 0, st>>>(a);
    else igemm_glds_kernel<64, 128><<<g64, 256, 0, st>>>(a);
  } else if ((variant == 6 || variant == 7) && bn == BN) {
    const dim3 gpp(d->Npad / BN, (unsigned)((M + 255) / 256), nz);
    if (use_buf) igemm_pp_kernel<128, true><<<gpp, 512, pp_lds_bytes(128), st>>>(a);
    else igemm_pp_kernel<128><<<gpp, 512, pp_lds_bytes(128), st>>>(a);
  } else if (variant == 5 && bn == BN) {
    igemm_glds_kernel<128, 128, true><<<grid, 256, PIPE_LDS_BYTES, st>>>(a);
  } else if (bn == BN) {
    if (use_buf) igemm_glds_kernel<128, 128, false, true><<<grid, 256, 0, st>>>(a);
    else igemm_glds_kernel<128, 128><<<grid, 256, 0, st>>>(a);
  } else {
    if (use_buf) igemm_glds_kernel<128, 64, false, true><<<grid, 256, 0, st>>>(a);
    else igemm_glds_kernel<128, 64><<<grid, 256, 0, st>>>(a);
  }
  int rc = ufr::launched("igemm_kernel");
  if (rc != UFR_OK || d->splitk == 1 || d->no_reduce || a.tickets) return rc;
  const long total = (long)d->nphase * M * (d->Npad / 8);
  igemm_reduce_kernel<<<ufr::stream_grid(total, 256), 256, 0, st>>>(a);
  return ufr::launched("igemm_reduce_kernel");
}
```

understanding_flow_robustness_amd/flownetc_engine.py:

```python
from __future__ import annotations

import os

import torch
from ._lib import engine_cache as _engine_cache

from . import _lib as L
from . import igemm as ig

_HEADS = ((6, 1024), (5, 1026), (4, 770), (3, 386), (2, 194))


def _pack_flow_head(weight: torch.Tensor) -> torch.Tensor:
    cin = weight.shape[1]
    chunks = ig.pad32(cin) // 32
    w = torch.zeros(2, chunks * 32, 9, dtype=torch.float32, device=weight.device)
    w[:, :cin] = weight.detach().float().reshape(2, cin, 9)
    return w.view(2, chunks, 32, 9).permute(1, 3, 0, 2).contiguous()


def _pack_flow_head_mfma(weight: torch.Tensor) -> torch.Tensor:
    cin = weight.shape[1]
    chunks = ig.pad32(cin) // 32
    w = torch.zeros(chunks * 32, 32, dtype=torch.float32, device=weight.device)
# ... 44 lines not shown
        self.flow_out, self.flow_scale = self.flow[2], float(getattr(net, "div_flow", 20.0))
        self._wprefixes, self._wprefix = {}, None
        self._win_m3 = 0
        self._build_launches()

    def _conv(self, name):
        return getattr(self.net, name)[0]

    def _bias(self, conv):
        if conv.bias is None:
            return torch.zeros(conv.out_channels, dtype=torch.float32, device=self.dev)
        return conv.bias.detach().float().contiguous()

    def _stem_layers(self):
        from .plane_graph import stem_stages
        return [(name, block[0], lvl) for lvl, stage in enumerate(stem_stages(self.net), 1) for name, block in stage]

    def _build_launches(self):
        net, g, B = self.net, self.grid, self.B
        plans = []

        def plan(wi, x, in_chunk0, rows, out_hw, **kw):
            M = B * rows[0] * rows[1]
            pk = [len(t) * wi.KC for _, _, t in wi.phases]
            kw.setdefault("variant", self._variant_for(wi))
            bm, target = self._tile_rows_and_slots(wi, kw)
            S = ig.splitk_for(M, wi.Npad, max(pk), len(wi.phases), phase_ktiles=pk, bm=bm, target=target)
            kw["variant"], S = ig.tuned(wi, M, kw, kw["variant"], S, rows=rows)
            plans.append((wi, x, in_chunk0, rows, out_hw, S, kw))
            return len(plans) - 1

        self._pipe_variant = {"0": 2, "5": 5}.get(os.environ.get("UFR_IGEMM_PIPE", "6"), 6)

        fwd, bwd = {}, {}
        cw = lambda n, s, p: ig.conv_forward_weights(self._conv(n).weight, s, p)
        cb = lambda n, s, p: ig.conv_backward_weights(self._conv(n).weight, s, p)
        bias = lambda n: self._bias(self._conv(n))
        if self.siamese:
            fwd["conv_redir"] = plan(cw("conv_redir", 1, 0), self.c3a_p, 0, g[8], g[8], out_planes=self.in31, out_chunk0=0,
                                     bias=bias("conv_redir"))
        fwd["conv3_1"] = plan(cw("conv3_1", 1, 1), self.in31, 0, g[8], g[8], out_planes=self.cat3, out_chunk0=0, bias=bias("conv3_1"))
        fwd["conv4"] = plan(cw("conv4", 2, 1), self.cat3, 0, g[16], g[16], out_planes=self.c4a, bias=bias("conv4"))
        fwd["conv4_1"] = plan(cw("conv4_1", 1, 1), self.c4a, 0, g[16], g[16], out_planes=self.cat4, out_chunk0=0, bias=bias("conv4_1"))
        fwd["conv5"] = plan(cw("conv5", 2, 1), self.cat4, 0, g[32], g[32], out_planes=self.c5a, bias=bias("conv5"))
        fwd["conv5_1"] = plan(cw("conv5_1", 1, 1), self.c5a, 0, g[32], g[32], out_planes=self.cat5, out_chunk0=0, bias=bias("conv5_1"))
        fwd["conv6"] = plan(cw("conv6", 2, 1), self.cat5, 0, g[64], g[64], out_planes=self.c6a, bias=bias("conv6"))
        fwd["conv6_1"] = plan(cw("conv6_1", 1, 1), self.c6a, 0, g[64], g[64], out_planes=self.c6, bias=bias("conv6_1"))
        dec = {5: (self.c6, 64, self.cat5, 16), 4: (self.cat5, 32, self.cat4, 16), 3: (self.cat4, 16, self.cat3, 8),
               2: (self.cat3, 8, self.cat2, 4)}
        for k, (src, s_in, dst, chunk0) in dec.items():
            n = f"deconv{k}"
            fwd[n] = plan(ig.deconv_forward_weights(self._conv(n).weight, 1), src, 0, g[s_in], g[s_in // 2], out_planes=dst,
                          out_chunk0=chunk0, bias=bias(n))
        gz = {5: (self.gz_cat5, 16, 16), 4: (self.gz_cat4, 16, 8), 3: (self.gz_cat3, 8, 4), 2: (self.gz_cat2, 4, 2)}
        Gabove = {2: self.G_cat3, 3: self.G_cat4, 4: self.G_cat5}
        self.tail_w, self.tail_args = {}, {}
        for k in (2, 3, 4):
            src, chunk0, _ = gz[k]
            s_in = {2: 8, 3: 16, 4: 32}[k]
            w = self._conv(f"deconv{k}").weight
            main = w.shape[0] - 2
            bwd[f"deconv{k}"] = plan(ig.deconv_backward_weights(w[:main], 1), src, chunk0, g[s_in], g[s_in], out_f32=Gabove[k])
            self.tail_w[k] = _pack_flow_tail_mfma(w[main:])
            self.tail_args[k] = (src, chunk0, ig.pad32(w.shape[1]) // 32, Gabove[k], main // 32, g[s_in])
        bwd["deconv5"] = plan(ig.deconv_backward_weights(self._conv("deconv5").weight, 1), self.gz_cat5, 16, g[64], g[64],
                              add=self.G_c6, mask=self.c6, out_planes=self.gz_c6)
        bwd["conv6_1"] = plan(cb("conv6_1", 1, 1), self.gz_c6, 0, g[64], g[64], mask=self.c6a, out_planes=self.gz_c6a)
        bwd["conv6"] = plan(cb("conv6", 2, 1), self.gz_c6a, 0, g[64], g[32], add=self.G_cat5, mask=self.cat5, out_planes=self.gz_cat5)
        bwd["conv5_1"] = plan(cb("conv5_1", 1, 1), self.gz_cat5, 0, g[32], g[32], mask=self.c5a, out_planes=self.gz_c5a)
        bwd["conv5"] = plan(cb("conv5", 2, 1), self.gz_c5a, 0, g[32], g[16], add=self.G_cat4, mask=self.cat4, out_planes=self.gz_cat4)
        bwd["conv4_1"] = plan(cb("conv4_1", 1, 1), self.gz_cat4, 0, g[16], g[16], mask=self.c4a, out_planes=self.gz_c4a)
        bwd["conv4"] = plan(cb("conv4", 2, 1), self.gz_c4a, 0, g[16], g[8], add=self.G_cat3, mask=self.cat3, out_planes=self.gz_cat3)
        if self.siamese:
            bwd["conv3_1"] = plan(cb("conv3_1", 1, 1), self.gz_cat3, 0, g[8], g[8], mask=self.in31, out_planes=self.gz_in31,
                                  out_f32=self.G_in31, planes_chunks=1, f32_first_chunk=1)
            bwd["conv_redir"] = plan(cb("conv_redir", 1, 0), self.gz_in31, 0, g[8], g[8], out_f32=self.G_c3a)
        else:
            bwd["conv3_1"] = plan(cb("conv3_1", 1, 1), self.gz_cat3, 0, g[8], g[8], out_f32=self.G_in31)
        need = max([len(wi.phases) * S * B * rows[0] * rows[1] * wi.Npad for wi, _, _, rows, _, S, _ in plans if S > 1] + [1])
        self.ws = torch.empty(need, dtype=torch.float32, device=self.dev)
        launches = [ig.make_launch(wi, x, c0, rows, out_hw, splitk=S, ws=self.ws if S > 1 else None, **kw)
                    for wi, x, c0, rows, out_hw, S, kw in plans]
        self.fwd = {k: launches[i] for k, i in fwd.items()}
        self.bwd = {k: launches[i] for k, i in bwd.items()}
        self._plans = {("fwd", k): plans[i] for k, i in fwd.items()}
        self._plans.update({("bwd", k): plans[i] for k, i in bwd.items()})
        self._band, self.fwd_band, self.bwd_band = None, {}, {}
        self.bwd_band_wide, self.bwd_rest, self._band_plans, self._pf_band, self._split_w = {}, {}, {}, {}, {}
        self.pf_w = {k: _pack_flow_head(getattr(net, f"predict_flow{k}").weight) for k, _ in _HEADS}
        self.pf_wm = {k: _pack_flow_head_mfma(getattr(net, f"predict_flow{k}").weight) for k, _ in _HEADS}
        self.pf_b = {k: getattr(net, f"predict_flow{k}").bias.detach().float().contiguous() for k, _ in _HEADS}
        self.up = {k: getattr(net, f"upsampled_flow{k}_to_{k - 1}") for k in (6, 5, 4, 3)}
        self.up_w = {k: m.weight.detach().float().contiguous() for k, m in self.up.items()}
        self.up_b = {k: (m.bias.detach().float().contiguous() if m.bias is not None else None) for k, m in self.up.items()}
        self.pf_src = {6: (self.c6, 32), 5: (self.cat5, 33), 4: (self.cat4, 25), 3: (self.cat3, 13), 2: (self.cat2, 7)}
        self.pf_G = {6: self.G_c6, 5: self.G_cat5, 4: self.G_cat4, 3: self.G_cat3, 2: self.G_cat2}
        self.up_dst = {6: (self.cat5, 32), 5: (self.cat4, 24), 4: (self.cat3, 12), 3: (self.cat2, 6)}
        self.up_G = {6: (self.G_cat5, 32), 5: (self.G_cat4, 24), 4: (self.G_cat3, 12), 3: (self.G_cat2, 6)}

    def _variant_for(self, wi):
        return self._pipe_variant if wi.Npad % 128 == 0 else 2

    @staticmethod
    def _tile_rows_and_slots(wi, kw):
        v = kw.get("variant", 0)
        if wi.Npad % 128:
            return 128, 768
        if v == 4:
            return 64, 1024
        if v == 5:
            return 128, 512
        if v == 6:
            return 256, 256
        return 128, 768

    def _build_prefix(self):
        B, dev = self.B, self.dev
        H, W = self.H, self.W
        layers = self._stem_layers()
        wis = [None] + [ig.conv_forward_weights(conv.weight, conv.stride[0], conv.padding[0]) for _, conv, _ in layers[1:]]
        scratch = {}

        def level_buffer(lvl, slot, chunks):
            if (lvl, slot) not in scratch:
                scratch[(lvl, slot)] = ig.Planes(B, H >> lvl, W >> lvl, chunks, dev)
            return scratch[(lvl, slot)]
        halves = {}
        for h, taps in (("a", {2: self.cat2, 3: self.c3a_p}), ("b", {3: self.c3b_p})):
            outs = []
            for i, (_, conv, lvl) in enumerate(layers):
                later = sum(1 for _, _, l in layers[i + 1:] if l == lvl)
                outs.append(taps[lvl] if later == 0 and lvl in taps else level_buffer(lvl, later % 2, ig.pad32(conv.out_channels) // 32))
            chain = []
            for i in range(1, len(layers)):
                name, conv, lvl = layers[i]
                launch = ig.make_launch(wis[i], outs[i - 1], 0, (H >> lvl, W >> lvl), (H >> lvl, W >> lvl), out_planes=outs[i],
                                        out_chunk0=0, bias=self._bias(conv), variant=self._variant_for(wis[i]))
                chain.append((name, launch, wis[i]))
            conv1 = layers[0][1]
            P = dict(c1=outs[0], layers=chain, b1=self._bias(conv1), w1=conv1.weight.detach())
            P.update({name: launch for name, launch, _ in chain})
            P.update({name + "_wi": wi for name, _, wi in chain})
            P.update(self._conv1_launch(B, H, W, outs[0]))
            halves[h] = P
        self._prefix = halves

    def _conv1_launch(self, n: int, H: int, W: int, c1: ig.Planes) -> dict:
        conv1 = self._stem_layers()[0][1]
        bias = self._bias(conv1)
        if os.environ.get("UFR_CONV1_DIRECT", "1") != "0":
            return dict(direct=dict(wimg=ig.conv1_direct_weights(conv1.weight), bias=bias, c1=c1, n=n, hw=(H, W),
                                    gflop=2.0 * n * (H // 2) * (W // 2) * 147 * 64 / 1e9))
        packed = ig.Planes(n, H // 2 + 3, W // 2 + 2, 1, self.dev)
        wi = ig.conv1_packed_weights(conv1.weight)
        launch = ig.make_launch(wi, packed, 0, (H // 2, W // 2), (H // 2, W // 2), out_planes=c1, bias=bias, variant=2)
        return dict(packed=packed, conv1=launch, conv1_wi=wi)

    def _conv1(self, P: dict, a: torch.Tensor, b: torch.Tensor | None):
        a = a.contiguous()
        L.require_hip(a, "frames")
        nb = 0 if b is None else int(b.shape[0])
        mean = self.net._mean64.reshape(-1).contiguous()
        D = P.get("direct")
        if D is not None:
            c1 = D["c1"]
            L.check(L.lib().ufr_conv1_direct(L.ptr(a), L.ptr(b.contiguous()) if b is not None else None, int(a.shape[0]), nb,
                                             int(a.shape[2]), int(a.shape[3]), L.ptr(mean), L.ptr(D["wimg"]), L.ptr(D["bias"]),
                                             float(ig.LEAKY), L.ptr(c1.t), c1.plane_stride, 0, L.stream()), "conv1 direct")
            return
        pk = P["packed"]
        L.check(L.lib().ufr_conv1_pack_planes(L.ptr(a), L.ptr(b.contiguous()) if b is not None else None, L.ptr(pk.t),
                                              pk.plane_stride, int(a.shape[0]), nb, int(a.shape[2]), int(a.shape[3]),
                                              L.ptr(mean), L.stream()), "conv1 pack")
        P["conv1"]()

    def prefix_full(self, frames_a: torch.Tensor, frames_b: torch.Tensor):
        if self._prefix is None:
            self._build_prefix()
        B = self.B

        def chain(h, frames, out):
# ... 57 lines not shown
        for wi, x, rows, out_hw, kw in plans:
            pk = [len(t) * wi.KC for _, _, t in wi.phases]
            kw.setdefault("variant", self._variant_for(wi))
            bm, target = self._tile_rows_and_slots(wi, kw) if kw.get("variant") in (5, 6) else (128, 768)
            sized.append(ig.splitk_for(B2 * rows[0] * rows[1], wi.Npad, max(pk), len(wi.phases), phase_ktiles=pk, bm=bm, target=target))
        need = max([len(wi.phases) * S * B2 * rows[0] * rows[1] * wi.Npad for (wi, _, rows, _, _), S in zip(plans, sized) if S > 1] + [1])
        ws = torch.empty(need, **f32)
        launches = [ig.make_launch(wi, x, 0, rows, out_hw, splitk=S, ws=ws if S > 1 else None, **kw)
                    for (wi, x, rows, out_hw, kw), S in zip(plans, sized)]
        chain = [(name, launch, p[0]) for name, launch, p in zip(names, launches, plans)]
        P = dict(hw=(wh, ww), c1=acts[0], c2=acts[tap2], c3=acts[-1], gz_c3=gz[-1], gz_c2=gz[tap2], G_gw2=G_gw2, ws=ws,
                 acts=acts, gz=gz, fwd=chain[:n - 1], bwd=chain[n - 1:],
                 G_p=G_p, gxw=torch.zeros(B2, 3, wh, ww, **f32),
                 c2_nchw=torch.zeros(B2, 128, h4, w4, **f32), c3_nchw=torch.zeros(B2, 256, h8, w8, **f32))
        P.update({name: launch for name, launch, _ in chain})
        P.update({name + "_wi": wi for name, _, wi in chain})
        P.update(self._conv1_launch(B2, wh, ww, acts[0]))
        self._wprefixes[(wh, ww)] = P
        self._bound_wprefixes()
        return P

    MAX_WINDOW_PREFIXES = 4

    def _bound_wprefixes(self):
        while len(self._wprefixes) > self.MAX_WINDOW_PREFIXES:
            del self._wprefixes[next(iter(self._wprefixes))]

    def window_prefix(self, wh: int, ww: int) -> dict:
        P = self._wprefixes.pop((int(wh), int(ww)), None)
        if P is None:
            P = self._build_window_prefix(int(wh), int(ww))
        else:
            self._wprefixes[(int(wh), int(ww))] = P
        self._wprefix = P
        return P

    def window_prefix_forward(self, xw: torch.Tensor, win: torch.Tensor, m2: int, m3: int, c2_nchw: bool = True):
        wh, ww = int(xw.shape[2]), int(xw.shape[3])
        P = self.window_prefix(wh, ww)
        self._win_m3 = int(m3)
        self._conv1(P, xw.detach(), None)
        for _, launch, _ in P["fwd"]:
            launch()
        c2, c3, H, W = P["c2"], P["c3"], self.H, self.W
        L.check(L.lib().ufr_window_features_planes(
            L.ptr(c2.t), c2.plane_stride, L.ptr(c3.t), c3.plane_stride, L.ptr(self.cat2.t), self.cat2.plane_stride,
            L.ptr(self.c3a_p.t), self.c3a_p.plane_stride, L.ptr(self.c3b_p.t), self.c3b_p.plane_stride, L.ptr(self.c3_nchw),
            L.ptr(P["c3_nchw"]), L.ptr(win), self.B, H, W, wh, ww, int(m2), int(m3), L.stream()), "window features -> planes")
        if c2_nchw:
            c2.to_nchw(128, 0, out=P["c2_nchw"])

    def window_gather_conv2_gradient(self, win: torch.Tensor, m2: int):
        P = self._wprefix
        wh, ww = P["hw"]
        h4, w4 = self.grid[4]
        L.check(L.lib().ufr_window_gather_chunks(L.ptr(self.G_cat2.t), L.ptr(P["G_gw2"].t), L.ptr(win), self.B, self.B, 2 * self.B, 4,
                                                 h4, w4, wh // 4, ww // 4, 4, int(m2), L.stream()), "window gather (chunks)")

    def window_prefix_backward(self, gw3: torch.Tensor, gw2: torch.Tensor | None = None, unpack: bool = True) -> torch.Tensor:
        P, B = self._wprefix, self.B
        wh, ww = P["hw"]
        if gw2 is not None:
            full = torch.zeros(2 * B, 128, wh // 4, ww // 4, dtype=torch.float32, device=self.dev)
            full[:B] = gw2
            P["G_gw2"].t.copy_(full.view(2 * B, 4, 32, wh // 4, ww // 4).permute(1, 0, 3, 4, 2).reshape(4, -1, 32))
        gz = P["gz_c3"]
        L.check(L.lib().ufr_nchw_grad_to_planes(L.ptr(gw3), L.ptr(P["c3_nchw"]), L.ptr(gz.t), gz.plane_stride, 0, 2 * B, 256, wh // 8,
                                                ww // 8, ig.LEAKY, L.stream()), "window gradient -> planes")
        for _, launch, _ in P["bwd"]:
            launch()
        if not unpack:
            return P["G_p"].t
        L.check(L.lib().ufr_conv1_unpack_grad(L.ptr(P["G_p"].t), L.ptr(P["gxw"]), 2 * B, wh, ww, L.stream()), "conv1 unpack")
        return P["gxw"]

    _FWD_BAND = {"conv_redir": (8, 8), "conv3_1": (8, 8), "conv4": (16, 8), "conv4_1": (16, 16)}
    _BWD_BAND = {"conv5": (32, None), "conv4_1": (16, 16), "conv4": (16, 16), "conv3_1": (8, 8), "conv_redir": (8, 8)}

    def attach_band(self, band):
        if self._band is band:
            return
        self._band, self.fwd_band, self.bwd_band = band, {}, {}
        self.bwd_band_wide, self.bwd_rest, self._band_plans, self._pf_band = {}, {}, {}, {}
        if not band.width:
            return
        W = self.W
        if band.width % 32 or band.width > W:
            raise ValueError("band width must be a multiple of 32 pixels inside the frame")
        origin = band.win[:, 1]

        def derive(kind, name, ls_rows, ls_in):
            wi, x, c0, rows, out_hw, S, kw = self._plans[(kind, name)]
            rows_b = (rows[0], band.width // ls_rows)
            extra = dict(row_band=(origin, 8, ls_rows))
            if ls_in is not None:
                extra["in_band"] = (origin, 8, ls_in, band.width // ls_in)
            M = self.B * rows_b[0] * rows_b[1]
            pk = [len(t) * wi.KC for _, _, t in wi.phases]
            bm, target = self._tile_rows_and_slots(wi, kw)
            Sb = ig.splitk_for(M, wi.Npad, max(pk), len(wi.phases), phase_ktiles=pk, bm=bm, target=target)
            if len(wi.phases) * Sb * M * wi.Npad > self.ws.numel():
                Sb = 1
            return ig.make_launch(wi, x, c0, rows_b, out_hw, splitk=Sb, ws=self.ws if Sb > 1 else None, **kw, **extra)

        for name, (ls_rows, _) in self._FWD_BAND.items():
            if ("fwd", name) in self._plans:
                self.fwd_band[name] = derive("fwd", name, ls_rows, None)
        for name, (ls_rows, ls_in) in self._BWD_BAND.items():
            if ("bwd", name) in self._plans:
                self.bwd_band[name] = derive("bwd", name, ls_rows, ls_in)
        if self.siamese:
            self._attach_unread(band, origin)

    _SPLIT_DECONV = {2: ("conv3_1", 8), 3: ("conv4_1", 16)}

    def _attach_unread(self, band, origin):
        B = self.B

        def planned(name, wi, x, c0, rows, out_hw, kw):
            M = B * rows[0] * rows[1]
            pk = [len(t) * wi.KC for _, _, t in wi.phases]
            kw.setdefault("variant", self._variant_for(wi))
            bm, target = self._tile_rows_and_slots(wi, kw)
            S = ig.splitk_for(M, wi.Npad, max(pk), len(wi.phases), phase_ktiles=pk, bm=bm, target=target)
            kw["variant"], S = ig.tuned(wi, M, kw, kw["variant"], S, rows=rows)
            if len(wi.phases) * S * M * wi.Npad > self.ws.numel():
                S = 1
            self._band_plans[name] = (wi, x, c0, rows, out_hw, kw)
            return ig.make_launch(wi, x, c0, rows, out_hw, splitk=S, ws=self.ws if S > 1 else None, **kw)

        for k, (lead, ls) in self._SPLIT_DECONV.items():
            src, chunk0, _, Gd, _, rows = self.tail_args[k]
            w = self._conv(f"deconv{k}").weight
            main, n_band = w.shape[0] - 2, self._conv(lead).out_channels
            if n_band % 32 or not 0 < n_band < main:
                continue
            name = f"deconv{k}"
            if name not in self._split_w:
                self._split_w[name] = (ig.deconv_backward_weights(w[:n_band], 1), ig.deconv_backward_weights(w[n_band:main], 1))
            w_band, w_rest = self._split_w[name]
            self.bwd_band[name] = planned(name, w_band, src, chunk0, (rows[0], band.width // ls), rows,
                                          dict(out_f32=Gd, out_f32_chunk0=0, row_band=(origin, 8, ls)))
            self.bwd_rest[name + " rest"] = planned(name + " rest", w_rest, src, chunk0, rows, rows,
                                                    dict(out_f32=Gd, out_f32_chunk0=n_band // 32))
            self._pf_band[k + 1] = (n_band // 32, ls)
        cw = int(getattr(band, "corr_width", 0))
        if cw:
            if cw % 8 or cw > band.width:
                raise ValueError("correlation band: a multiple of 8 pixels inside the band")
            for name in ("conv3_1", "conv_redir"):
                wi, x, c0, rows, out_hw, _, kw = self._plans[("bwd", name)]
                self.bwd_band_wide[name] = self.bwd_band[name]
                kw = dict(kw, row_band=(band.win[:, 2], 8, 8), in_band=(origin, 8, 8, band.width // 8))
                self.bwd_band[name] = planned(name, wi, x, c0, (rows[0], cw // 8), out_hw, kw)

    def replan(self, kind: str, name: str, tag: str):
        if kind == "bwd" and name in self._band_plans and tag == ("full" if name in self.bwd_rest else "band"):
            wi, x, c0, rows, out_hw, kw = self._band_plans[name]
            return wi, x, c0, rows, out_hw, dict(kw)
        wi, x, c0, rows, out_hw, _, kw = self._plans[(kind, name)]
        kw = dict(kw)
        if tag == "band":
            band = self._band
            ls_rows, ls_in = (self._FWD_BAND[name][0], None) if kind == "fwd" else self._BWD_BAND[name]
            origin = band.win[:, 1]
            rows = (rows[0], band.width // ls_rows)
            kw["row_band"] = (origin, 8, ls_rows)
            if ls_in is not None:
                kw["in_band"] = (origin, 8, ls_in, band.width // ls_in)
        return wi, x, c0, rows, out_hw, kw

    def launch_table(self):
        rows = []
        for kind, table, tag in (("fwd", self.fwd, "full"), ("bwd", self.bwd, "full"), ("fwd", self.fwd_band, "band"),
                                 ("bwd", self.bwd_band, "band"), ("bwd", self.bwd_rest, "full")):
            for name, launch in table.items():
                wi = self._band_plans[name][0] if kind == "bwd" and table is not self.bwd and name in self._band_plans else \
                    self._plans[(kind, name)][0]
                d = launch.desc
                rows.append((name, kind, tag, launch, wi.flops(d.B * d.Hr * d.Wr) / 1e9))
        if self._prefix is not None:
            for h, suffix in (("a", ""), ("b", " 2nd frames")):
                F = self._prefix[h]
                packed = [("conv1", F["conv1"], F["conv1_wi"])] if "conv1" in F else []
                for key, launch, wi in packed + F["layers"]:
                    d = launch.desc
                    rows.append((key + suffix, "fwd", "prefix", launch, wi.flops(d.B * d.Hr * d.Wr) / 1e9))
        P = getattr(self, "_wprefix", None)
        if P is not None:
            packed = [("conv1", P["conv1"], P["conv1_wi"])] if "conv1" in P else []
            for kind, chain in (("fwd", packed + P["fwd"]), ("bwd", P["bwd"])):
                for key, launch, wi in chain:
                    d = launch.desc
                    rows.append((key[:-4] if kind == "bwd" else key, kind, "window", launch, wi.flops(d.B * d.Hr * d.Wr) / 1e9))
        return rows

    def conv1_direct_table(self):
        rows = []
        sets = []
        if self._prefix is not None:
            sets += [("conv1 direct" + sfx, "prefix", self._prefix[h]) for h, sfx in (("a", ""), ("b", " 2nd frames"))]
        if getattr(self, "_wprefix", None) is not None:
            sets.append(("conv1 direct", "window", self._wprefix))
        for label, tag, P in sets:
            D = P.get("direct")
            if D is None:
                continue
            n, (H, W) = D["n"], D["hw"]
            frames = torch.rand(n, 3, H, W, device=self.dev)
            nbytes = n * 3 * H * W * 4 + n * (H // 2) * (W // 2) * 64 * 6
            rows.append((label, tag, (lambda P=P, frames=frames: self._conv1(P, frames, None)), float(nbytes), D["gflop"]))
        return rows

    def _pf_forward(self, k):
        src, chunks = self.pf_src[k]
        L.check(L.lib().ufr_flow_head_planes_forward_mfma(L.ptr(src.t), src.plane_stride, 0, chunks, L.ptr(self.pf_wm[k]),
                                                          self.pf_wm[k].shape[0], L.ptr(self.pf_b[k]), L.ptr(self.flow[k]), self.B, src.H, src.W,
                                                          L.stream()), "predict_flow forward (mfma)")

    def _pf_backward(self, k, gy, accumulate, finalize=None, region=None):
        src, chunks = self.pf_src[k]
        if region is not None:
            head, kind, origin, stride, div, rh, rw, margin, wout = region
            act, out, c0, n = finalize if finalize is not None else (None, None, 0, 0)
            L.check(L.lib().ufr_flow_head_planes_backward_regions(
                L.ptr(gy), L.ptr(self.pf_w[k]), self.pf_w[k].shape[0], L.ptr(self.pf_G[k].t), self.pf_G[k].chunks, 0, chunks, self.B,
                src.H, src.W, int(accumulate), int(head), int(kind), L.ptr(origin), int(stride), int(div), int(rh), int(rw), int(margin),
                L.ptr(wout.t) if wout is not None else None, wout.B if wout is not None else 0,
                L.ptr(act.t) if act is not None else None, L.ptr(out.t) if out is not None else None,
                out.plane_stride if out is not None else 0, int(c0), int(n), float(ig.LEAKY), L.stream()),
                "predict_flow backward (regions)")
            return
        if finalize is not None:
            act, out, c0, n = finalize
            L.check(L.lib().ufr_flow_head_planes_backward_finalize(L.ptr(gy), L.ptr(self.pf_w[k]), self.pf_w[k].shape[0], L.ptr(self.pf_G[k].t),
# ... 9 lines not shown
    def _up_forward(self, k):
        dst, chunk = self.up_dst[k]
        f = self.flow[k]
        L.check(L.lib().ufr_flow_up_planes_forward(L.ptr(f), L.ptr(self.up_w[k]), L.ptr(self.up_b[k]) if self.up_b[k] is not None else None,
                                                   L.ptr(dst.t), dst.plane_stride, chunk, self.B, f.shape[2], f.shape[3],
                                                   L.stream()), "upsampled_flow forward")

    def _deconv_tail(self, k):
        src, chunk0, chunks, Gd, out_chunk, (h, w) = self.tail_args[k]
        L.check(L.lib().ufr_deconv_flow_tail_backward_mfma(L.ptr(src.t), src.plane_stride, chunk0, chunks, L.ptr(self.tail_w[k]),
                                                           self.tail_w[k].shape[0], L.ptr(Gd.t), Gd.chunks, out_chunk, self.B, h, w, L.stream()),
                "deconv data gradient, flow channels")

    def _up_backward(self, k):
        G, chunk = self.up_G[k]
        f = self.g_flow[k]
        L.check(L.lib().ufr_flow_up_planes_backward(L.ptr(G.t), chunk, L.ptr(self.up_w[k]), L.ptr(f), self.B, f.shape[2],
                                                    f.shape[3], 0, L.stream()), "upsampled_flow backward")

    def _finalize(self, Gs, mask, out, chunk0, chunks):
        L.check(L.lib().ufr_grad_finalize(L.ptr(Gs.t), chunk0, L.ptr(mask.t), chunk0, L.ptr(out.t), out.plane_stride, chunk0,
                                          Gs.M, chunks, ig.LEAKY, L.stream()), "gradient finalize")

    def _forward_trunk(self, c2: torch.Tensor, c3: torch.Tensor) -> torch.Tensor:
        L.require_hip(c2, "c2")
        L.require_hip(c3, "c3")
        self.cat2.load_nchw(c2, 0)
        self.in31.load_nchw(c3, 0)
        for name in ("conv3_1", "conv4", "conv4_1", "conv5", "conv5_1", "conv6", "conv6_1"):
            self.fwd[name]()
        self._pf_forward(6)
        for k in (5, 4, 3, 2):
            self._up_forward(k + 1)
            self.fwd[f"deconv{k}"]()
            self._pf_forward(k)
        return self.flow[2]

    def forward_cached(self, band=None, corr_changed: bool = True) -> torch.Tensor:
        return self.forward(None, self._c3a, self._c3b, band, corr_changed=corr_changed)

    def forward(self, c2a: torch.Tensor | None, c3a: torch.Tensor, c3b: torch.Tensor, band=None,
                corr_changed: bool = True) -> torch.Tensor:
        if not self.siamese:
            return self._forward_trunk(c2a, c3a)
        for t, name in ((c3a, "c3a"), (c3b, "c3b")):
            L.require_hip(t, name)
        self._c3a, self._c3b = c3a, c3b
        inc = False
        if band is not None:
            self.attach_band(band)
            inc = bool(band.width and band.incremental and band.inc_layers)
        if c2a is not None:
            L.require_hip(c2a, "c2a")
            self.cat2.load_nchw(c2a, 0)
            self.c3a_p.load_nchw(c3a, 0)
            self.c3b_p.load_nchw(c3b, 0)
        if inc and band.cone_win is not None and band.cone_hw[1] // 8 <= 23:
            if corr_changed:
                L.check(L.lib().ufr_corr_forward_planes_changed(L.ptr(self.c3a_p.t), L.ptr(self.c3b_p.t), self.c3a_p.plane_stride,
                                                                L.ptr(self.in31.t), self.in31.plane_stride, 1, self.B, 256, *self.grid[8],
                                                                21, 2, 1.0 / 256.0, ig.LEAKY, L.ptr(band.cone_win), 8,
                                                                band.cone_hw[0] // 8, band.cone_hw[1] // 8, self._win_m3, L.stream()),
                        "correlation forward (planes, changed)")
            else:
                L.check(L.lib().ufr_corr_forward_planes_window(L.ptr(self.c3a_p.t), L.ptr(self.c3b_p.t), self.c3a_p.plane_stride,
                                                               L.ptr(self.in31.t), self.in31.plane_stride, 1, self.B, 256, *self.grid[8],
                                                               21, 2, 1.0 / 256.0, ig.LEAKY, L.ptr(band.cone_win), 8,
                                                               band.cone_hw[1] // 8, L.stream()), "correlation forward (planes, window)")
        else:
            L.check(L.lib().ufr_corr_forward_planes(L.ptr(self.c3a_p.t), L.ptr(self.c3b_p.t), self.c3a_p.plane_stride,
                                                    L.ptr(self.in31.t), self.in31.plane_stride, 1, self.B, 256, *self.grid[8], 21, 2,
                                                    1.0 / 256.0, ig.LEAKY, L.stream()), "correlation forward (planes)")
        for name in ("conv_redir", "conv3_1", "conv4", "conv4_1"):
            (self.fwd_band if inc else self.fwd)[name]()
        for name in ("conv5", "conv5_1", "conv6", "conv6_1"):
            self.fwd[name]()
        self._pf_forward(6)
        for k in (5, 4, 3, 2):
            self._up_forward(k + 1)
            self.fwd[f"deconv{k}"]()
            self._pf_forward(k)
        return self.flow[2]

    def backward(self, g_flow2: torch.Tensor, band=None, fused_window: bool = True, skip_unread: bool = True):
        L.require_hip(g_flow2, "g_flow2")
        B = self.B
        banded = band is not None and bool(band.width)
        if band is not None:
            self.attach_band(band)
        gz = {2: (self.G_cat2, self.cat2, self.gz_cat2, 4, 2), 3: (self.G_cat3, self.cat3, self.gz_cat3, 8, 4),
              4: (self.G_cat4, self.cat4, self.gz_cat4, 16, 8), 5: (self.G_cat5, self.cat5, self.gz_cat5, 16, 16)}
        fuse = os.environ.get("UFR_FUSE_FINALIZE", "1") != "0"
        fin = lambda k: (gz[k][1], gz[k][2], gz[k][3], gz[k][4]) if fuse else None
        eng_window = bool(fused_window and band is not None and getattr(band, "eng_window", False)
                          and getattr(self, "_wprefix", None) is not None)
        skip = bool(skip_unread and banded and fused_window and self.siamese)
        if skip and eng_window:
            P = self._wprefix
            wh, ww = P["hw"]
            self._pf_backward(2, g_flow2, accumulate=False, finalize=fin(2),
                              region=(4, L.UFR_PF_REGION_WINDOW, band.cone_win, 8, 4, wh // 4, ww // 4, band.g2_margin, P["G_gw2"]))
        else:
            self._pf_backward(2, g_flow2, accumulate=False, finalize=fin(2))
            if eng_window:
                self.window_gather_conv2_gradient(band.cone_win, band.g2_margin)
            else:
                self.G_cat2.to_nchw(128, 0, out=self.g_c2a)
        for k in (2, 3, 4):
            Gs, act, out, chunk0, chunks = gz[k]
            if not fuse:
                self._finalize(Gs, act, out, chunk0, chunks)
            self._up_backward(k + 1)
            region = None
            if skip and k + 1 in self._pf_band:
                self.bwd_band[f"deconv{k}"]()
                self.bwd_rest[f"deconv{k} rest"]()
                head, ls = self._pf_band[k + 1]
                region = (head, L.UFR_PF_REGION_BAND, band.win[:, 1], 8, ls, self.grid[ls][0], band.width // ls, 0, None)
            else:
                self.bwd[f"deconv{k}"]()
            self._deconv_tail(k)
            self._pf_backward(k + 1, self.g_flow[k + 1], accumulate=True, finalize=fin(k + 1), region=region)
        Gs, act, out, chunk0, chunks = gz[5]
        if not fuse:
            self._finalize(Gs, act, out, chunk0, chunks)
        self._up_backward(6)
        self._pf_backward(6, self.g_flow[6], accumulate=False)
        for name in ("deconv5", "conv6_1", "conv6", "conv5_1"):
            self.bwd[name]()
        if not self.siamese:
            for name in ("conv5", "conv4_1", "conv4", "conv3_1"):
                self.bwd[name]()
            self.G_in31.to_nchw(256, 0, out=self.g_c3a)
            return self.g_c2a, self.g_c3a, None
        for name in ("conv5", "conv4_1", "conv4", "conv3_1", "conv_redir"):
            if banded and not skip and name in self.bwd_band_wide:
                self.bwd_band_wide[name]()
            else:
                (self.bwd_band if banded else self.bwd)[name]()
        gw = getattr(band, "g3_window", None) if (band is not None and fused_window) else None
        h8, w8 = self.grid[8]
        if gw is not None and band.cone_win is not None and band.cone_hw[1] // 8 <= 16 and w8 % 4 == 0:
            L.check(L.lib().ufr_corr_backward_window_fused(L.ptr(self._c3a), L.ptr(self._c3b), L.ptr(self.G_in31.t), 1, 1.0 / 256.0,
                                                           L.ptr(self.G_c3a.t), L.ptr(gw), B, 256, h8, w8, 21, 2,
                                                           L.ptr(band.cone_win), 8, band.cone_hw[0] // 8, band.cone_hw[1] // 8,
                                                           int(band.g3_margin), L.stream()), "correlation backward (window, fused)")
            return (None if eng_window else self.g_c2a), None, None
        self.G_c3a.to_nchw(256, 0, out=self.g_c3a_redir)
        self.G_in31.to_nchw(441, 1, scale=1.0 / 256.0, out=self.g_corr.view(B, 441, *self.grid[8]))
        self._corr_backward(self.g_corr, band)
        return (None if eng_window else self.g_c2a), self.g_c3a, self.g_c3b

    def _corr_backward(self, g_corr, band):
        from . import spatial_correlation_sampler_backend as correlation
        import ctypes as C
        h8, w8 = self.grid[8]
        if band is not None and band.cone_win is not None:
            L.check(L.lib().ufr_corr_backward_window(L.ptr(self._c3a), L.ptr(self._c3b), L.ptr(g_corr), L.ptr(self.g_c3a),
                                                     L.ptr(self.g_c3b), self.B, 256, h8, w8, 21, 2, L.ptr(band.cone_win), 8,
                                                     band.cone_hw[0] // 8, band.cone_hw[1] // 8, L.stream()),
                    "correlation backward (window)")
        else:
            p = correlation._params(1, 1, 21, 21, 0, 0, 1, 1, 2, 2, 1, 1)
            L.check(L.lib().ufr_corr_backward(L.ptr(self._c3a), L.ptr(self._c3b), L.ptr(g_corr), L.ptr(self.g_c3a),
                                              L.ptr(self.g_c3b), L.UFR_F32, self.B, 256, h8, w8, C.byref(p), L.stream()),
                    "correlation backward")
        self.g_c3a.add_(self.g_c3a_redir)

    REPLACEABLE = ("conv3a", "conv3b", "corr", "conv_redir", "conv3_1")
    _HEAD_SEGMENTS = {
        "conv_redir": ("in31", 0, 32), "corr": ("in31", 1, 441), "conv3_1": ("cat3", 0, 256), "deconv3": ("cat3", 8, 128),
        "upsampled_flow4_to_3": ("cat3", 12, 2), "conv4": ("c4a", 0, 512), "conv4_1": ("cat4", 0, 512), "deconv4": ("cat4", 16, 256),
        "upsampled_flow5_to_4": ("cat4", 24, 2), "conv5": ("c5a", 0, 512), "conv5_1": ("cat5", 0, 512), "deconv5": ("cat5", 16, 512),
        "upsampled_flow6_to_5": ("cat5", 32, 2), "conv6": ("c6a", 0, 1024), "conv6_1": ("c6", 0, 1024), "deconv2": ("cat2", 4, 64),
        "upsampled_flow3_to_2": ("cat2", 6, 2)}
    _FLOW_KEYS = {"flow6": 6, "flow5": 5, "flow4": 4, "flow3": 3, "predict": 2}

    def segment_map(self, stem=None) -> dict:
        if not self.siamese:
            raise RuntimeError("feature-map segments: the FlowNetC head (the FlowNetS trunk has no correlation)")
        seg = {}
        if stem is not None:
            for lvl, cn in ((1, 64), (2, 128), (3, 256)):
                p = stem.bufs[f"c{lvl}"].planes
                seg[f"conv{lvl}a"], seg[f"conv{lvl}b"] = (p, 0, cn, 0, None), (p, 0, cn, self.B, None)
        for key, (buf, c0, cn) in self._HEAD_SEGMENTS.items():
            seg[key] = (getattr(self, buf), c0, cn, 0, "unleaky" if key == "corr" else None)
        for key, k in self._FLOW_KEYS.items():
            seg[key] = (self.flow[k], 0, 2, 0, None)
        return seg

    def capture(self, keys=None, stem=None) -> dict:
        seg = self.segment_map(stem)
        out = {}
        for key in (list(seg) if keys is None else keys):
            if key not in seg:
                raise KeyError(f"capture: {key!r} is not a feature map of this forward ({', '.join(seg)})")
            src, c0, cn, img0, post = seg[key]
            if isinstance(src, ig.Planes):
                t = src.to_nchw(cn, c0)[img0:img0 + self.B]
                out[key] = _unleaky(t, ig.LEAKY) if post == "unleaky" else (t if t.shape[0] == src.B else t.clone())
            else:
                out[key] = src[:, c0:c0 + cn].clone()
        return out

    def forward_replaced(self, c2a, c3a, c3b, overwrite=None, keep=(), computed=None) -> torch.Tensor:
        if not self.siamese:
            raise RuntimeError("feature-map replacement: the FlowNetC head")
        ow = {k: v for k, v in (overwrite or {}).items() if k in self.REPLACEABLE}
        keep = {k for k in keep if k in self.REPLACEABLE and k not in ow}
        pair = lambda d: "conv3a" in d and "conv3b" in d
        for t, name in ((c2a, "c2a"), (c3a, "c3a"), (c3b, "c3b")):
            L.require_hip(t, name)
        self.generation = getattr(self, "generation", 0) + 1
        self._c3a, self._c3b = c3a, c3b
        self.cat2.load_nchw(c2a, 0)
        if pair(ow):
            self.c3a_p.load_nchw(ow["conv3a"].contiguous(), 0)
            self.c3b_p.load_nchw(ow["conv3b"].contiguous(), 0)
        elif not pair(keep):
            self.c3a_p.load_nchw(c3a, 0)
            self.c3b_p.load_nchw(c3b, 0)
# ... 85 lines not shown
```

understanding_flow_robustness_amd/igemm.py:

```python
from __future__ import annotations

import ctypes as C

import os

import torch

from . import _lib as L

LEAKY = 0.1


def pad32(c: int) -> int:
    return (c + 31) // 32 * 32


def pad128(c: int) -> int:
    return (c + 127) // 128 * 128


def pad_n(c: int) -> int:
    p64, p128 = (c + 63) // 64 * 64, pad128(c)
    return p64 if p64 * 4 <= p128 * 3 else p128

# ... 145 lines not shown
def planes_as_weights(p: Planes, N: int | None = None) -> WeightImage:
    if p.M % 64:
        raise ValueError("planes_as_weights: the pixel count must be a multiple of 64")
    planes = p.t.view(3, -1)
    wi = WeightImage(planes, [0], [(0, 0, [(0, 0)])], p.M if N is None else N, p.M, p.chunks, dict(in_s=1, out_s=1), C=p.chunks * 32.0)
    wi._keep = p
    return wi


def conv1_direct_weights(weight: torch.Tensor) -> torch.Tensor:
    N, Cn, k, _ = weight.shape
    if (N, Cn, k) != (64, 3, 7):
        raise ValueError("conv1_direct_weights: Conv2d(3, 64, 7, 2, 3) only")
    w = weight.detach().float()
    img = torch.zeros(7, 64, 32, dtype=torch.float32, device=weight.device)
    for kx in range(7):
        for c in range(3):
            img[:, :, (kx >> 1) * 8 + (kx & 1) * 4 + c] = w[:, c, :, kx].t()
    return _split3(img).view(3, 7, 64, 32).contiguous()


def conv1_packed_backward_weights(weight: torch.Tensor) -> WeightImage:
    N, Cn, k, _ = weight.shape
    if (Cn, k) != (3, 7):
        raise ValueError("conv1_packed_backward_weights: Conv2d(3, N, 7, 2, 3) only")
    w = weight.detach().float()
    mat = torch.zeros(24, 8, N, dtype=torch.float32, device=weight.device)
    for a in range(4):
        for b2 in range(2):
            for j in range(2):
                for c in range(3):
                    for p in range(2):
                        for q in range(2):
                            ky, kx = 2 * a - 1 + p, 4 * b2 - 1 + 2 * j + q
                            if 0 <= ky < 7 and 0 <= kx < 7:
                                mat[j * 12 + (c * 2 + p) * 2 + q, a * 2 + b2, :] = w[:, c, ky, kx]
    taps = [(-a, -2 * b2) for a in range(4) for b2 in range(2)]
    planes, offsets, n, npad, KC, _ = _pack([mat], weight.device)
    return WeightImage(planes, offsets, [(0, 0, taps)], n, npad, KC, dict(in_s=1, out_s=1), C=147.0 * N / (8.0 * 24.0))


def conv_backward_weights(weight: torch.Tensor, stride: int, padding, dilation: int = 1) -> WeightImage:
    N, Cn, kh, kw = weight.shape
    ph, pw = _pair(padding)
    w = weight.detach().float()
    if stride == 1:
        mat = w.permute(1, 2, 3, 0).reshape(Cn, kh * kw, N)
        taps = [(ph - ky * dilation, pw - kx * dilation) for ky in range(kh) for kx in range(kw)]
        planes, offsets, n, npad, KC, cr = _pack([mat], weight.device)
        return WeightImage(planes, offsets, [(0, 0, taps)], n, npad, KC, dict(in_s=1, out_s=1), cr)
    k, padding = kh, ph
    if kh != kw or ph != pw:
        raise NotImplementedError("data gradient of a strided convolution: square kernels only")
    if stride != 2 or dilation != 1:
        raise NotImplementedError("data gradient: stride 1 (any dilation) or 2")
    phases = _deconv_phases(k, padding)
    mats = [torch.stack([w[:, :, ky, kx].t() for ky, kx, _, _ in taps], dim=1) for _, _, taps in phases]
    planes, offsets, n, npad, KC, cr = _pack(mats, weight.device)
    return WeightImage(planes, offsets, [(oy, ox, [(dy, dx) for _, _, dy, dx in taps]) for oy, ox, taps in phases], n, npad, KC,
                       dict(in_s=1, out_s=2), cr)


def deconv_forward_weights(weight: torch.Tensor, padding: int) -> WeightImage:
    cin, cout, k, _ = weight.shape
    w = weight.detach().float()
    phases = _deconv_phases(k, padding)
    mats = [torch.stack([w[:, :, ky, kx].t() for ky, kx, _, _ in taps], dim=1) for _, _, taps in phases]
    planes, offsets, n, npad, KC, cr = _pack(mats, weight.device)
    return WeightImage(planes, offsets, [(oy, ox, [(dy, dx) for _, _, dy, dx in taps]) for oy, ox, taps in phases], n, npad, KC,
                       dict(in_s=1, out_s=2), cr)


def deconv_backward_weights(weight: torch.Tensor, padding: int) -> WeightImage:
    cin, cout, k, _ = weight.shape
    w = weight.detach().float()
    mat = w.permute(0, 2, 3, 1).reshape(cin, k * k, cout)
    taps = [(ky - padding, kx - padding) for ky in range(k) for kx in range(k)]
    planes, offsets, n, npad, KC, cr = _pack([mat], weight.device)
    return WeightImage(planes, offsets, [(0, 0, taps)], n, npad, KC, dict(in_s=2, out_s=1), cr)


class Launch:

    def __init__(self, desc, keep):
        self.desc, self._keep = desc, keep

    def __call__(self):
        L.check(L.lib().ufr_igemm(C.byref(self.desc), L.stream()), "igemm")

    def algorithmic_bytes(self) -> float:
        d = self.desc
        rows = d.B * d.Hr * d.Wr
        pix_in = min(d.B * d.Hi * d.Wi, rows * d.in_sy * d.in_sx)
        taps = sum(d.phase[z].ntaps for z in range(d.nphase))
        out_el = rows * d.nphase * ((d.tail_n0 if d.tail else d.N) + 31) // 32 * 32
        b = pix_in * d.KC * 32 * 6 + taps * d.KC * d.Npad * 32 * 6
        b += out_el * ((4 if d.add else 0) + (2 if d.mask else 0))
        nch = out_el // (rows * d.nphase * 32)
        pl = min(nch, d.planes_chunks) if d.planes_chunks else nch
        b += rows * d.nphase * 32 * ((6 * pl if d.out_planes else 0) + (4 * (nch - min(nch, d.f32_first_chunk)) if d.out_f32 else 0))
        if d.tail:
            b += rows * (d.N - d.tail_n0) * 4
        return float(b)


_TUNING = None
FUSE_REDUCE = os.environ.get("UFR_IGEMM_FUSE_REDUCE", "0") == "1"
_PRODUCTS = [6]


class products:
    def __init__(self, n: int):
        if n not in (6, 3, 1):
            raise ValueError("igemm.products: 6, 3 or 1")
        self.n = n

    def __enter__(self):
        _PRODUCTS.append(self.n)

    def __exit__(self, *exc):
        _PRODUCTS.pop()


RECORD = None


def launch_signature(wi: "WeightImage", M: int, kw: dict, rows=None) -> str:
    out = ("slabs" if kw.get("no_reduce") else "rowmajor" if kw.get("out_rowmajor") is not None else
           ("planes" if kw.get("out_planes") is not None else "") + ("f32" if kw.get("out_f32") is not None else ""))
    out += ("+add" if kw.get("add") is not None else "") + ("+mask" if kw.get("mask") is not None else "") + ("+tail" if kw.get("tail") is not None else "")
    taps = "-".join(str(len(t)) for _, _, t in wi.phases)
    grid = f"_g{int(rows[0])}x{int(rows[1])}" if rows is not None else ""
    return f"M{M}_N{wi.Npad}_KC{wi.KC}_t{taps}_s{wi.geometry['in_s']}{wi.geometry['out_s']}_{out}{grid}"


def _tuning_table() -> dict:
    global _TUNING
    if _TUNING is None:
        _TUNING = {}
        path = os.environ.get("UFR_IGEMM_TUNING_FILE") or os.path.join(os.path.dirname(os.path.abspath(__file__)), "igemm_tuning.json")
        if os.environ.get("UFR_IGEMM_TUNING", "1") != "0" and os.path.exists(path):
            import json
            with open(path) as f:
                raw = json.load(f)
            if raw.get("_arch", "gfx950") == "gfx950":
                _TUNING = {k: tuple(v) for k, v in raw.items() if not k.startswith("_")}
    return _TUNING


def variant_fallbacks() -> int:
    return int(L.lib().ufr_igemm_variant_fallbacks())


def tuned(wi: "WeightImage", M: int, kw: dict, variant: int, splitk: int, rows=None):
    table, sig = _tuning_table(), launch_signature(wi, M, kw)
    if rows is not None and launch_signature(wi, M, kw, rows) in table:
        return table[launch_signature(wi, M, kw, rows)]
    if sig in table:
        return table[sig]
    head, _, out = sig.rpartition("_")
    twin = out.replace("+add", "") if "+add" in out else (out.replace("+mask", "+add+mask") if "+mask" in out else
                                                         (out.replace("+tail", "+add+tail") if "+tail" in out else out + "+add"))
    return table.get(f"{head}_{twin}", (variant, splitk))


def make_launch(wi: WeightImage, x: Planes, in_chunk0: int, rows_hw, out_hw, *, out_planes: Planes | None = None,
                out_chunk0: int = 0, out_f32: GradSum | None = None, out_f32_chunk0: int = 0, bias: torch.Tensor | None = None,
                add: GradSum | None = None, add_chunk0: int = 0, mask: Planes | None = None, mask_chunk0: int = 0,
                slope: float = LEAKY, splitk: int = 1, ws: torch.Tensor | None = None, row_band=None, in_band=None,
                products: int | None = None, variant: int = 0, tail: GradSum | None = None, tail_n0: int = 0, tail_chunk0: int = 0,
                tail_accumulate: bool = False, out_rowmajor=None, planes_chunks: int = 0, f32_first_chunk: int = 0,
                no_reduce: bool = False, fuse_reduce: bool | None = None) -> Launch:
    if RECORD is not None:
        RECORD.append(dict(wi=wi, x=x, in_chunk0=in_chunk0, rows=tuple(rows_hw), out_hw=tuple(out_hw), splitk=splitk, variant=variant,
                           kw=dict(out_planes=out_planes, out_chunk0=out_chunk0, out_f32=out_f32, out_f32_chunk0=out_f32_chunk0, bias=bias,
                                   add=add, add_chunk0=add_chunk0, mask=mask, mask_chunk0=mask_chunk0, slope=slope, row_band=row_band,
                                   in_band=in_band, tail=tail, tail_n0=tail_n0, tail_chunk0=tail_chunk0, tail_accumulate=tail_accumulate,
                                   out_rowmajor=out_rowmajor, planes_chunks=planes_chunks, f32_first_chunk=f32_first_chunk,
                                   no_reduce=no_reduce)))
    d = L.IgemmDesc()
    d.x, d.x_plane_stride, d.in_chunk0, d.KC = x.t.data_ptr(), x.plane_stride, int(in_chunk0), wi.KC
    if in_chunk0 + wi.KC > x.chunks:
        raise RuntimeError("igemm: the reduced chunks leave the input buffer")
    d.B, d.Hi, d.Wi = x.B, x.H, x.W
    d.in_sy = d.in_sx = int(wi.geometry["in_s"])
    if in_band is not None:
        d.in_x0, d.in_x0_stride, d.in_x0_div, d.in_xw = in_band[0].data_ptr(), int(in_band[1]), int(in_band[2]), int(in_band[3])
    d.w, d.w_plane_stride, d.Npad, d.N = wi.planes.data_ptr(), wi.planes.stride(0), wi.Npad, wi.N
    d.Hr, d.Wr = int(rows_hw[0]), int(rows_hw[1])
    if row_band is not None:
        d.row_x0, d.row_x0_stride, d.row_x0_div = row_band[0].data_ptr(), int(row_band[1]), int(row_band[2])
    d.Ho, d.Wo = int(out_hw[0]), int(out_hw[1])
    d.out_sy = d.out_sx = int(wi.geometry["out_s"])
    d.nphase = len(wi.phases)
    for z, ((oy0, ox0, taps), off) in enumerate(zip(wi.phases, wi.offsets)):
        ph = d.phase[z]
        if len(taps) > L.UFR_IGEMM_MAX_TAPS:
            raise RuntimeError("igemm: too many taps")
        ph.ntaps, ph.oy0, ph.ox0, ph.w_off = len(taps), oy0, ox0, off
        for t, (dy, dx) in enumerate(taps):
            ph.dy[t], ph.dx[t] = dy, dx
    Mout = x.B * d.Ho * d.Wo
    nch = pad32(wi.N) // 32
    if tail is not None:
        if tail_n0 % 32 or not 0 < tail_n0 < wi.N or tail.M != Mout or tail_chunk0 + (wi.N - tail_n0 + 31) // 32 > tail.chunks:
            raise RuntimeError("igemm: tail geometry")
        d.tail, d.tail_n0 = tail.t.data_ptr() + int(tail_chunk0) * tail.M * 32 * 4, int(tail_n0)
        d.tail_accumulate = 1 if tail_accumulate else 0
        nch = tail_n0 // 32
    keep = [wi, x, bias, add, mask, out_planes, out_f32, ws, row_band, in_band, tail]
    if bias is not None:
        d.act, d.bias = 1, bias.data_ptr()
    d.slope = float(slope)
    if add is not None:
        if add.M != Mout or add_chunk0 + nch > add.chunks:
            raise RuntimeError("igemm: addend geometry")
        d.add, d.add_chunk0 = add.t.data_ptr(), int(add_chunk0)
    if mask is not None:
        if mask.M != Mout or mask_chunk0 + nch > mask.chunks:
            raise RuntimeError("igemm: mask geometry")
        d.mask, d.mask_chunk0 = mask.t.data_ptr(), int(mask_chunk0)
    if out_planes is not None:
        if out_planes.M != Mout or out_chunk0 + nch > out_planes.chunks:
            raise RuntimeError("igemm: output plane geometry")
        d.out_planes, d.out_plane_stride, d.out_chunk0 = out_planes.t.data_ptr(), out_planes.plane_stride, int(out_chunk0)
    if out_f32 is not None:
        if out_f32.M != Mout or out_f32_chunk0 + nch > out_f32.chunks:
            raise RuntimeError("igemm: fp32 output geometry")
        d.out_f32, d.out_f32_chunk0 = out_f32.t.data_ptr(), int(out_f32_chunk0)
    if out_rowmajor is not None:
        rm, rm_off, ld = out_rowmajor
        if rm.dtype != torch.float32 or wi.N % 8 or ld < wi.N or ld % 4 or rm_off % 4 or rm.numel() < rm_off + (Mout - 1) * ld + wi.N:
            raise RuntimeError("igemm: row-major output geometry")
        d.out_rowmajor, d.out_ld = rm.data_ptr() + 4 * int(rm_off), int(ld)
        keep.append(rm)
    if planes_chunks or f32_first_chunk:
        if out_planes is None or out_f32 is None:
            raise RuntimeError("igemm: planes_chunks / f32_first_chunk need both outputs")
        d.planes_chunks, d.f32_first_chunk = int(planes_chunks), int(f32_first_chunk)
    d.splitk = int(splitk)
    if splitk > 1:
        need = d.nphase * splitk * x.B * d.Hr * d.Wr * wi.Npad
        if ws is None or ws.numel() < need or ws.dtype != torch.float32:
            raise RuntimeError(f"igemm: split-K workspace of {need} floats needed")
        d.ws = ws.data_ptr()
    d.no_reduce = 1 if (no_reduce and splitk > 1) else 0
    if splitk > 1 and not d.no_reduce and (FUSE_REDUCE if fuse_reduce is None else fuse_reduce):
        tickets = torch.zeros(d.nphase * (-(-(x.B * d.Hr * d.Wr) // 64)) * (wi.Npad // 64), dtype=torch.int32, device=x.t.device)
        d.tickets = tickets.data_ptr()
        keep.append(tickets)
    d.products = int(_PRODUCTS[-1] if products is None else products)
    d.k_order = int(wi.k_order)
    d.variant = int(variant)
    return Launch(d, keep)


def splitk_for(M: int, Npad: int, ktiles: int, phases: int = 1, target: int = 768, phase_ktiles=None, bm: int = 128,
               min_ktiles: int = 16) -> int:
    tiles_mn = -(-M // bm) * (Npad // (128 if Npad % 128 == 0 else 64))
    if phase_ktiles is not None and len(set(phase_ktiles)) > 1:
        best, best_cost = 1, None
        s = 1
        while s <= 16:
            per = -(-max(phase_ktiles) // s)
            if s > 1 and per < min(8, min_ktiles):
                break
            wgs = tiles_mn * sum(-(-k // per) for k in phase_ktiles)
            cost = -(-wgs // target) * (per + 6) + (10 if s > 1 else 0)
            if best_cost is None or cost < best_cost:
                best, best_cost = s, cost
            s *= 2
        return best
    tiles = tiles_mn * phases
    s = 1
    while tiles * s * 2 <= target and ktiles // (s * 2) >= min_ktiles and s < 32:
        s *= 2
    return s


class WgradLaunch(Launch):

    def __init__(self, descs, keep, dilation=(1, 1)):
        super().__init__(descs[0], keep)
        self.descs = descs
        self.dilation = dilation

    def __call__(self):
        dy, dx = self.dilation
        for d in self.descs:
            L.check(L.lib().ufr_igemm_wgrad_dilated(C.byref(d), dy, dx, L.stream()), "igemm wgrad")

    def algorithmic_bytes(self) -> float:
        d = self.desc
        return float(6 * 32 * (d.B * d.Hi * d.Wi * (pad32(d.C) // 32) + d.B * d.Ho * d.Wo * (pad32(d.N) // 32)) + 4 * d.N * d.C * d.kh * d.kw)


def splitm_for(M: int, N: int, Cn: int, taps: int, target: int = 1024) -> int:
    nch = pad32(N) // 32
    tiles = -(-nch // (4 if nch > 2 else 2)) * -(-pad32(Cn) // 64) * taps
    return max(1, min(-(-target // tiles), M // 128, 256))


def _wgrad_desc(x, in_chunk0, Cn, gy, g_chunk0, N, kernel, stride, padding, dw, db, accumulate, splitm, keep):
    kh, kw = _pair(kernel)
    sy, sx = _pair(stride)
    py, px = _pair(padding)
    if x.B != gy.B:
        raise RuntimeError("igemm wgrad: the operands' batch sizes differ")
    if in_chunk0 + pad32(Cn) // 32 > x.chunks or g_chunk0 + pad32(N) // 32 > gy.chunks:
        raise RuntimeError("igemm wgrad: the reduced chunks leave an operand's buffer")
    if kh * kw > L.UFR_IGEMM_WGRAD_MAX_TAPS:
        raise RuntimeError("igemm wgrad: too many taps")
    if dw.dtype != torch.float32 or not dw.is_contiguous() or dw.numel() != N * Cn * kh * kw or not dw.is_cuda:
        raise RuntimeError(f"igemm wgrad: dw must be a contiguous HIP float32 tensor of {N} x {Cn} x {kh} x {kw} elements")
    if db is not None and (db.dtype != torch.float32 or not db.is_contiguous() or db.numel() != N or not db.is_cuda):
        raise RuntimeError(f"igemm wgrad: db must be a contiguous HIP float32 tensor of {N} elements")
    d = L.IgemmWgradDesc()
    d.x, d.x_plane_stride, d.in_chunk0, d.C = x.t.data_ptr(), x.plane_stride, int(in_chunk0), int(Cn)
    d.gy, d.gy_plane_stride, d.g_chunk0, d.N = gy.t.data_ptr(), gy.plane_stride, int(g_chunk0), int(N)
    d.B, d.Hi, d.Wi, d.Ho, d.Wo = x.B, x.H, x.W, gy.H, gy.W
    d.kh, d.kw, d.sy, d.sx, d.py, d.px = kh, kw, sy, sx, py, px
    d.dw, d.db = dw.data_ptr(), (db.data_ptr() if db is not None else None)
    d.accumulate = 1 if accumulate else 0
    d.splitm = int(splitm) if splitm is not None else splitm_for(gy.M, N, Cn, kh * kw)
    if d.splitm > 1:
        slab = N * Cn * kh * kw + (N if db is not None else 0)
        ws = torch.empty(d.splitm * slab, dtype=torch.float32, device=dw.device)
        d.ws, d.ws_elems = ws.data_ptr(), ws.numel()
        keep.append(ws)
    d.products = 6
    return d


def make_wgrad_launch(x: Planes, in_chunk0: int, C: int, gy: Planes, g_chunk0: int, N: int, kernel, stride, padding, *,
                      transposed: bool = False, dw: torch.Tensor, db: torch.Tensor | None = None, accumulate: bool = False,
                      splitm: int | None = None, dilation=1) -> Launch:
    keep = [x, gy, dw, db]
# ... 15 lines not shown
```

understanding_flow_robustness_amd/patch_attack.py:

```python
from __future__ import annotations

import ctypes as C
import os
from argparse import Namespace

import numpy as np
import torch
from ._lib import engine_cache as _engine_cache

from . import _lib as L
from .flownets.utils_model import predict_flow

LOSS_THRESHOLD = 0.1
CLAMP_BOUND = 2.0


def _pixel_range(flownet: str):
    return (0.0, 1.0) if any(k in flownet for k in ("FlowNetC", "FlowNetS", "FlowNet2", "RAFT", "PWC")) else (-1.0, 1.0)


class ShardedExchange:

    def __init__(self, group=None):
        import torch.distributed as dist
        self.dist, self.group = dist, group
        self.world = dist.get_world_size(group) if dist.is_initialized() else 1
        self.rank = dist.get_rank(group) if dist.is_initialized() else 0

    def __call__(self, packed: torch.Tensor) -> torch.Tensor:
        if self.world > 1:
            self.dist.all_reduce(packed, op=self.dist.ReduceOp.SUM, group=self.group)
        return packed

    def gather(self, rows_local: torch.Tensor, rows_all: torch.Tensor) -> torch.Tensor:
        if self.world > 1:
            self.dist.all_gather_into_tensor(rows_all, rows_local, group=self.group)
        return rows_all


class PatchAttackStep:

    def __init__(self, flow_net, args, batch, height, width, device="cuda:0", shared_patch=True,
                 exchange: ShardedExchange | None = None, use_graph=True, warmup=3, use_cone=None, patch_hw=None,
                 sum_groups=1, skip_unread=True, corr_changed=True):
        L.lib()
        self.net, self.args = flow_net, args
        self.skip_unread = bool(skip_unread)
        self.corr_changed = bool(corr_changed)
        self.B, self.H, self.W = batch, height, width
        self.dev = torch.device(device)
        self.shared = shared_patch
        self.exchange = exchange
        self.world = exchange.world if exchange is not None else 1
        if self.world > 1 and not shared_patch:
            raise ValueError("per-sample patches need no exchange; shard them as independent replicas")
        self.placed = patch_hw is not None
        if shared_patch and batch * self.world > 1 and not self.placed:
            raise ValueError("one patch behind several pairs is defined in patch coordinates: pass patch_hw=(ph, pw) "
                             "and load() a [1,3,ph,pw] patch / mask with per-pair origins (SURVEY.md 8e)")
        if self.placed and not shared_patch:
            raise ValueError("patch_hw: per-sample patches stay canvas-sized like the reference's")
        self.groups = int(sum_groups)
        if self.groups < 1 or batch % self.groups or (self.groups > 1 and not self.placed):
            raise ValueError("sum_groups must divide the pairs of a patch-coordinate step")
        self.lo, self.hi = _pixel_range(args.flownet)
        self.kind = 1 if getattr(args, "l2", False) else 0
        self.alpha = float(getattr(args, "alpha", 0.0))
        self.step = 0.5 * float(args.lr)
        self.CHW = 3 * height * width
        f32 = dict(dtype=torch.float32, device=self.dev)
        pb = 1 if shared_patch else batch
        self.tgt = torch.zeros(batch, 3, height, width, **f32)
        self.ref = torch.zeros_like(self.tgt)
        self._mask_canvas = None if self.placed else torch.zeros_like(self.tgt)
        self._mask_stale = self.placed
        if self.placed:
            ph, pw = (int(v) for v in patch_hw)
            if not (0 < ph <= height and 0 < pw <= width):
                raise ValueError("patch_hw does not fit the frame")
            self.ph, self.pw, self.n_p = ph, pw, 3 * ph * pw
            self.patch = torch.zeros(1, 3, ph, pw, **f32)
            self.mask_p = torch.zeros(1, 3, ph, pw, **f32)
            self.origins = torch.zeros(batch, 2, dtype=torch.int32, device=self.dev)
            self.origins_host = None
            self.rows_local = torch.zeros(self.groups, self.n_p + 1, **f32)
            self.rows_all = torch.zeros(self.world * self.groups, self.n_p + 1, **f32) if self.world > 1 else self.rows_local
            self.loss_local = torch.zeros(1, **f32)
            self.loss_cur = torch.zeros(1, **f32)
        else:
            self.patch = torch.zeros(pb, 3, height, width, **f32)
            self.loss_cur = torch.zeros(1, **f32)
            self.loss_local = self.loss_cur
        self.patch_init = torch.zeros_like(self.patch)
        self.target = torch.zeros(batch, 2, height, width, **f32)
        self.adv_tgt = torch.zeros_like(self.tgt).requires_grad_(True)
        self.adv_ref = torch.zeros_like(self.tgt).requires_grad_(True)
        self.g_flow = torch.zeros_like(self.target)
        self.loss_ws = torch.zeros(L.LOSS_PARTIALS, **f32)
        self._fused_loss = (batch * -(-(height // 4) // 16) * -(-(width // 4) // 16) <= L.LOSS_PARTIALS
                            and height % 4 == 0 and width % 4 == 0)
        self.g_flow2 = torch.zeros(batch, 2, height // 4, width // 4, **f32)
        self.state = torch.zeros(4, **f32)
        L.freeze_parameters(self.net)
        self.net.eval()
        self.graph = self.graph_b = self.graph_next = self.graph_b_next = None
        self._first = True
        self._rect_paste = False
        self.use_graph = use_graph
        self._warmup = warmup
        if use_cone is None:
            use_cone = os.environ.get("UFR_CONE", "1") != "0"
        spec = getattr(flow_net, "CONE", None)
        self.cone = spec if (use_cone and spec is not None and height % spec.total_stride == 0
                             and width % spec.total_stride == 0) else None
        self.win_hw = None
        self.win = torch.zeros(batch, 8, dtype=torch.int32, device=self.dev)
        self.patch_loaded = torch.zeros_like(self.patch) if self.cone is not None else None

    @property
    def mask(self):
        if self.placed and self._mask_stale:
            if self._mask_canvas is None:
                self._mask_canvas = torch.zeros_like(self.tgt)
            with torch.cuda.device(self.dev):
                L.check(L.lib().ufr_patch_mask_placed(L.ptr(self.mask_p), L.ptr(self.origins), L.ptr(self._mask_canvas), self.B,
                                                      self.H, self.W, self.ph, self.pw, L.stream()), "placed mask")
            self._mask_stale = False
        return self._mask_canvas

    def _paste(self, do_clamp, gate=False, write_mask=False):
        if self.placed and self._rect_paste and not write_mask:
# ... 18 lines not shown
        L.check(L.lib().ufr_patch_update(L.ptr(self.tgt), L.ptr(self.ref), L.ptr(g_tgt), L.ptr(g_ref),
                                         L.ptr(self.patch), L.ptr(self.mask), L.ptr(self.adv_tgt),
                                         L.ptr(self.adv_ref), self.B, self.CHW, 0 if self.shared else self.CHW,
                                         self.CHW, self.step, CLAMP_BOUND, self.lo, self.hi,
                                         L.ptr(self.state), L.stream()), "patch update")

    def _crop(self, g_tgt, g_ref):
        L.check(L.lib().ufr_patch_grad_crop(L.ptr(g_tgt), L.ptr(g_ref), L.ptr(self.mask_p), L.ptr(self.origins), None,
                                            L.ptr(self.loss_local), L.ptr(self.rows_local), self.B, self.H, self.W,
                                            self.ph, self.pw, self.groups, L.stream()), "patch grad crop")

    def _apply(self):
        if self._rect_paste:
            return self._apply_rect()
        L.check(L.lib().ufr_patch_apply(L.ptr(self.rows_all), self.rows_all.shape[0], L.ptr(self.patch),
                                        L.ptr(self.loss_cur), self.ph, self.pw, self.step, CLAMP_BOUND,
                                        L.ptr(self.state), L.stream()), "patch apply")
        self._paste(do_clamp=True, gate=True)

    def _apply_rect(self):
        L.check(L.lib().ufr_patch_apply_paste_rect(
            L.ptr(self.rows_all), self.rows_all.shape[0], L.ptr(self.patch), L.ptr(self.loss_cur), L.ptr(self.tgt), L.ptr(self.ref),
            L.ptr(self.mask_p), L.ptr(self.origins), L.ptr(self.adv_tgt), L.ptr(self.adv_ref), self.B, self.H, self.W, self.ph,
            self.pw, self.step, CLAMP_BOUND, 1, self.lo, self.hi, L.ptr(self.state), L.stream()), "patch apply + rect paste")

    def _mask_extent(self):
        m = self.mask.amax(dim=1) != 0
        rows, cols = m.any(dim=2).cpu(), m.any(dim=1).cpu()
        ext = lambda v: max([int(r.nonzero().max() - r.nonzero().min()) + 1 if bool(r.any()) else 0 for r in v] + [1])
        eh, ew = ext(rows), ext(cols)
        if self.world > 1:
            both = torch.tensor([eh, ew], dtype=torch.float32, device=self.dev)
            self.exchange.dist.all_reduce(both, op=self.exchange.dist.ReduceOp.MAX, group=self.exchange.group)
            eh, ew = (int(v) for v in both.tolist())
        return eh, ew

    def _setup_cone(self):
        spec, B, H, W = self.cone, self.B, self.H, self.W
        eh, ew = self._mask_extent()
        wh, ww = spec.window_size(eh, H), spec.window_size(ew, W)
        self.graph = self.graph_b = self.graph_next = self.graph_b_next = None
        if self._warmup < 0:
            self._warmup = 1
        if wh * ww * 2 > H * W:
            self.cone = None
            return
        self.win_hw = (wh, ww)
        f32 = dict(dtype=torch.float32, device=self.dev)
        self.xw = torch.zeros(2 * B, 3, wh, ww, **f32).requires_grad_(True)
        self.eng = self.eng_kind = None
        if getattr(self.net, "engine_available", None) is not None and self.net.engine_available(H, W, self.dev):
            self.eng_kind = getattr(self.net, "ENGINE", "flownetc")
            if self.eng_kind == "pwc":
                from .pwc_engine import get_engine
            else:
                from .flownetc_engine import get_engine
            self.eng = get_engine(self.net, B, H, W, self.dev)
            self.eng.flow_out.requires_grad_(True)
            self._wp_hold = self.eng.window_prefix(wh, ww)
        self.taps = []
        with torch.no_grad(), L.shape_probe():
            feats = self.net.encode(torch.zeros(2, 3, spec.total_stride * 2, spec.total_stride * 2, **f32))
        for t, m, fr, f in zip(spec.taps, spec.tap_margins(), spec.frames, feats):
            ls = spec.level_stride(t)
            n = B * fr
            full = None if self.eng is not None else torch.zeros(n, f.shape[1], H // ls, W // ls, **f32).requires_grad_(True)
            gwin = torch.zeros(n, f.shape[1], wh // ls, ww // ls, **f32)
            self.taps.append((ls, m, n, full, gwin))
        if not self.placed:
            self.g_tgt_full = torch.zeros_like(self.tgt)
            self.g_ref_full = torch.zeros_like(self.tgt)
        self._chain = spec.to_c()
        self.band, reach = None, getattr(self.net, "BAND_REACH", None)
        if reach is not None and os.environ.get("UFR_BAND", "1") != "0":
            from .band_conv import Band, corr_band_width
            bw = -(-(ww + 2 * reach + 31) // 32) * 32
            if W % 32 != 0 or bw * 4 > W * 3:
                bw = 0
            self._band_reach = reach
            self.band = Band(torch.zeros(B, 8, dtype=torch.int32, device=self.dev), bw, cone_win=self.win,
                             cone_hw=(wh, ww))
            if bw and corr_band_width(ww) <= bw:
                self.band.corr_width = corr_band_width(ww)
            if bw and os.environ.get("UFR_INCREMENTAL", "1") != "0":
                self.band.inc_layers = tuple(getattr(self.net, "INCREMENTAL_LAYERS", ()))

    def _win_copy(self, fn, src, dst, n, c, hf, wf, ls, margin):
        wh, ww = self.win_hw
        L.check(fn(L.ptr(src), L.ptr(dst), L.ptr(self.win), self.B, n, c, hf, wf, wh // ls, ww // ls, ls, margin,
                   L.stream()), "window copy")

    def _cone_refresh(self, prefix_features=None):
        lib = L.lib()
        wh, ww = self.win_hw
        L.check(lib.ufr_cone_window(L.ptr(self.mask), self.B, self.CHW, 3, self.H, self.W, C.byref(self._chain),
                                    wh, ww, L.ptr(self.win), L.ptr(self.state[3:]), L.stream()), "cone window")
        if not self.placed:
            self.g_tgt_full.zero_(); self.g_ref_full.zero_()
        if self.band is not None and self.band.width:
            start = torch.div(self.win[:, 1] - self._band_reach, 32, rounding_mode="floor") * 32
            self.band.win[:, 1] = start.clamp(0, self.W - self.band.width)
            if self.band.corr_width:
                from .band_conv import corr_band_origin
                self.band.win[:, 2] = corr_band_origin(self.win[:, 1], self.band.corr_width, self.W)
        self._cone_prefix(prefix_features)

    def _cone_prefix(self, prefix_features=None):
        if self.eng is not None:
            if prefix_features is not None:
                self.eng.load_prefix_features(*prefix_features)
            else:
                self.eng.prefix_full(self.adv_tgt.detach(), self.adv_ref.detach())
            return
        feats = prefix_features if prefix_features is not None else \
            self.net.encode(torch.cat((self.adv_tgt.detach(), self.adv_ref.detach()), 0))
        for (ls, m, n, full, _), f in zip(self.taps, feats):
            if f.shape[0] < n or f.shape[1:] != full.shape[1:]:
                raise ValueError("prefix_features do not match this step's frames")
            full.detach().copy_(f[:n])

    def _forward_cone(self):
        lib, B, H, W = L.lib(), self.B, self.H, self.W
        wh, ww = self.win_hw
        L.check(lib.ufr_window_gather_pair(L.ptr(self.adv_tgt), L.ptr(self.adv_ref), L.ptr(self.xw), L.ptr(self.win),
                                           L.ptr(self.loss_local), B, 3, H, W, wh, ww, L.stream()), "window gather (pair)")
        if self.eng is not None:
            self._feats_w = None
            if self.eng_kind == "pwc":
                self.eng.window_prefix_forward(self.xw, self.win, self.taps[0][1])
                self.eng.forward_cached()
            else:
                (_, m2, _, _, _), (_, m3, _, _, _) = self.taps
                self.eng.window_prefix_forward(self.xw, self.win, m2, m3, c2_nchw=False)
                self.eng.forward_cached(self.band, corr_changed=self.corr_changed)
            if self._fused_loss:
                return None
            return torch.nn.functional.interpolate(self.eng.flow_out * self.eng.flow_scale, scale_factor=4, mode="bilinear",
                                                   align_corners=False)
        self._feats_w = [f[:n] for f, (_, _, n, _, _) in zip(self.net.encode(self.xw), self.taps)]
        for f, (ls, m, n, full, _) in zip(self._feats_w, self.taps):
            self._win_copy(lib.ufr_window_scatter, f, full, n, f.shape[1], H // ls, W // ls, ls, m)
        full = [t[3] for t in self.taps]
        extra = {"band": self.band} if self.band is not None else {}
        return self.net.head(*full[:-1], full[-1][:B], full[-1][B:], **extra)

    def _backward_cone(self, flow):
        lib, B, H, W = L.lib(), self.B, self.H, self.W
        self._packed_grad = False
        if self.eng is not None:
            if flow is None:
                g_flow2 = self.g_flow2
            else:
                (g_flow2,) = torch.autograd.grad(flow, (self.eng.flow_out,), self.g_flow)
            if self.eng_kind == "pwc":
                ls, m, n, _, gw = self.taps[0]
                g_f2 = self.eng.backward(g_flow2.contiguous())
                self._win_copy(lib.ufr_window_gather, g_f2, gw, n, g_f2.shape[1], H // ls, W // ls, ls, m)
                gxw = self.eng.window_prefix_backward(gw)
            else:
                (ls2, m2, _, _, gw2), (ls3, m3, _, _, gw3) = self.taps
                if self.band is not None:
                    self.band.g3_window, self.band.g3_margin = gw3, m3
                    self.band.eng_window, self.band.g2_margin = True, m2
                g2a, g3a, g3b = self.eng.backward(g_flow2.contiguous(), self.band, skip_unread=self.skip_unread)
                if g2a is not None:
                    self._win_copy(lib.ufr_window_gather, g2a, gw2, B, 128, H // ls2, W // ls2, ls2, m2)
                if g3a is not None:
                    self._win_copy(lib.ufr_window_gather, g3a, gw3, B, 256, H // ls3, W // ls3, ls3, m3)
                    self._win_copy(lib.ufr_window_gather, g3b, gw3[B:], B, 256, H // ls3, W // ls3, ls3, m3)
                self._packed_grad = self.placed
                gxw = self.eng.window_prefix_backward(self.taps[1][4], None if g2a is None else self.taps[0][4],
                                                      unpack=not self.placed)
        else:
            g_full = torch.autograd.grad(flow, [t[3] for t in self.taps], self.g_flow)
            for g, (ls, m, n, _, gwin) in zip(g_full, self.taps):
                self._win_copy(lib.ufr_window_gather, g.contiguous(), gwin, n, g.shape[1], H // ls, W // ls, ls, m)
            gxw, = torch.autograd.grad(self._feats_w, (self.xw,), [t[4] for t in self.taps])
        self._feats_w = None
        gxw = gxw.contiguous()
        if self.placed:
            return gxw, None
        self._win_copy(lib.ufr_window_scatter, gxw, self.g_tgt_full, B, 3, H, W, 1, 0)
        self._win_copy(lib.ufr_window_scatter, gxw[B:], self.g_ref_full, B, 3, H, W, 1, 0)
        return self.g_tgt_full, self.g_ref_full

    def _part_a(self):
        if self.cone is not None:
            flow = self._forward_cone()
        else:
            self.loss_local.zero_()
            flow = predict_flow(self.net, None, self.adv_tgt, self.adv_ref, self.args)
        weight = (1.0 - self.alpha) * ((1.0 / self.world) if self.shared else float(self.B))
        if flow is None:
            L.check(L.lib().ufr_flow2_upsampled_loss(L.ptr(self.eng.flow_out), float(self.eng.flow_scale), L.ptr(self.target),
                                                     L.ptr(self.g_flow2), L.ptr(self.loss_local), self.B, self.H // 4, self.W // 4,
                                                     self.kind, weight, L.ptr(self.loss_ws), L.stream()), "upsampled flow loss")
        else:
            if not flow.is_contiguous():
                flow = flow.contiguous()
            L.check(L.lib().ufr_flow_loss(L.ptr(flow), L.ptr(self.target), L.ptr(self.g_flow), L.ptr(self.loss_local),
                                          self.B, self.H * self.W, self.kind, weight, L.ptr(self.loss_ws), L.stream()),
                    "flow loss")
        if not self.shared:
            self.loss_local.div_(float(self.B))
        if self.alpha != 0.0:
            if self.placed:
                reg = (self.mask_p * self.patch - self.mask_p * self.patch_init).abs().sum() / float(self.CHW)
            else:
                reg = torch.nn.functional.l1_loss(self.mask * self.patch, self.mask * self.patch_init)
            self.loss_local.add_(self.alpha * reg / self.world)
        if self.cone is not None:
            g_tgt, g_ref = self._backward_cone(flow)
        else:
            g_tgt, g_ref = torch.autograd.grad(flow, (self.adv_tgt, self.adv_ref), self.g_flow)
            g_tgt, g_ref = g_tgt.contiguous(), g_ref.contiguous()
        if not self.placed:
            self._update(g_tgt, g_ref)
            self._gate()
            return
        if g_ref is None:
            wh, ww = self.win_hw
            crop = L.lib().ufr_patch_grad_crop_packed if self._packed_grad else L.lib().ufr_patch_grad_crop_window
            L.check(crop(L.ptr(g_tgt), L.ptr(self.win), L.ptr(self.mask_p), L.ptr(self.origins),
                                                       L.ptr(self.loss_local), L.ptr(self.rows_local), self.B, self.H, self.W, wh, ww,
                                                       self.ph, self.pw, self.groups, L.stream()), "patch grad crop (window)")
        else:
            self._crop(g_tgt, g_ref)
        if self.world == 1:
            self._apply()
            self._gate()

    def _part_b(self):
        self._apply()
        self._gate()

    def _gate(self):
        L.check(L.lib().ufr_attack_gate(L.ptr(self.loss_cur), L.ptr(self.state), LOSS_THRESHOLD, L.stream()),
                "attack gate")

    def _incremental_now(self):
        band = getattr(self, "band", None)
        return bool(self.cone is not None and band is not None and band.inc_layers and not self._first)

    def _set_later(self, later: bool):
        band = getattr(self, "band", None) if self.cone is not None else None
        if band is not None:
            band.incremental = bool(later and band.inc_layers)
# ... 292 lines not shown
```

Baseline: 1511.

## Split-K only the last partial wave of igemm tiles to balance CU load

Adds a tail-balancing plan for the pipelined igemm kernel: when the tile count leaves a partial last wave across resident workgroups, the full row tiles run unsplit and the leftover tail row tiles are split along K into slices written to a workspace, then reduced. A custom XCD-aware block-to-tile mapping assigns full and tail tiles. It is applied to FlowNetC backward igemm launches that were not already split-K, and is enabled by default. It adds a reduce kernel launch and workspace traffic for the tail, and relies on the CU count estimate for resident workgroups.

```diff
diff --git a/include/ufr_hip.h b/include/ufr_hip.h
--- a/include/ufr_hip.h
+++ b/include/ufr_hip.h
@@ -339,6 +339,18 @@
 } ufr_igemm_desc;
 int ufr_igemm(const ufr_igemm_desc* d, ufr_stream_t stream);
 typedef struct {
+  int on;
+  int row_tiles, col_tiles;
+  int full_row_tiles, tail_row_tiles;
+  int tail_row0, tail_rows;
+  int slices, slice_ktiles, ktiles;
+  int workgroups;
+  long ws_floats;
+  int steps_before, steps_after;
+} ufr_igemm_tail_plan_t;
+int ufr_igemm_tail_plan(const ufr_igemm_desc* d, int resident_workgroups, ufr_igemm_tail_plan_t* plan);
+int ufr_igemm_balanced(const ufr_igemm_desc* d, int resident_workgroups, float* ws, long ws_floats, ufr_stream_t stream);
+typedef struct {
   const void* x; long x_plane_stride; int in_chunk0, C;
   const void* gy; long gy_plane_stride; int g_chunk0, N;
   int B, Hi, Wi, Ho, Wo, kh, kw, sy, sx, py, px;
diff --git a/understanding_flow_robustness_amd/_lib.py b/understanding_flow_robustness_amd/_lib.py
--- a/understanding_flow_robustness_amd/_lib.py
+++ b/understanding_flow_robustness_amd/_lib.py
@@ -68,6 +68,12 @@
                 ("out_rowmajor", C.c_void_p), ("out_ld", C.c_long),
                 ("planes_chunks", C.c_int), ("f32_first_chunk", C.c_int), ("no_reduce", C.c_int),
                 ("tickets", C.c_void_p)]
+
+
+class IgemmTailPlan(C.Structure):
+    _fields_ = [("on", C.c_int), ("row_tiles", C.c_int), ("col_tiles", C.c_int), ("full_row_tiles", C.c_int), ("tail_row_tiles", C.c_int),
+                ("tail_row0", C.c_int), ("tail_rows", C.c_int), ("slices", C.c_int), ("slice_ktiles", C.c_int), ("ktiles", C.c_int),
+                ("workgroups", C.c_int), ("ws_floats", C.c_long), ("steps_before", C.c_int), ("steps_after", C.c_int)]
 
 
 UFR_IGEMM_WGRAD_MAX_TAPS = 49
@@ -188,6 +194,8 @@
     "ufr_raft_context_split_forward": [_vp, _vp, _vp, _i, _i, _i, _l, _vp],
     "ufr_raft_context_split_backward": [_vp, _vp, _vp, _vp, _vp, _i, _i, _i, _l, _vp],
     "ufr_igemm": [C.POINTER(IgemmDesc), _vp],
+    "ufr_igemm_tail_plan": [C.POINTER(IgemmDesc), _i, C.POINTER(IgemmTailPlan)],
+    "ufr_igemm_balanced": [C.POINTER(IgemmDesc), _i, _vp, _l, _vp],
     "ufr_igemm_wgrad": [C.POINTER(IgemmWgradDesc), _vp],
     "ufr_igemm_wgrad_dilated": [C.POINTER(IgemmWgradDesc), _i, _i, _vp],
     "ufr_flow_upscale4_forward": [_vp, _vp, _i, _i, _i, _i, _f, _i, _vp],
diff --git a/understanding_flow_robustness_amd/csrc/igemm.hip b/understanding_flow_robustness_amd/csrc/igemm.hip
--- a/understanding_flow_robustness_amd/csrc/igemm.hip
+++ b/understanding_flow_robustness_amd/csrc/igemm.hip
@@ -180,8 +180,28 @@
   float* ws;
   int* tickets;
   int skip_out;
+  int tl_S, tl_full, tl_nt, tl_rt0, tl_row0, tl_rows, tl_per_k;
   Phase ph[4];
 };
+
+__device__ __forceinline__ int xcd_before(int m, int x) { return (m >> 3) * x + min(m & 7, x); }
+__device__ __forceinline__ bool tail_tile(const Args& a, int& bx, int& by, int& bz) {
+  const int orig = blockIdx.x, x = orig & 7;
+  const bool tail = orig >= a.tl_full;
+  const int lo = tail ? a.tl_full : 0, hi = tail ? (int)gridDim.x : a.tl_full;
+  const int w = xcd_before(hi, x) - xcd_before(lo, x) + (orig >> 3) - ((lo + 7 - x) >> 3);
+  if (!tail) {
+    bz = 0;
+    by = w / a.tl_nt;
+    bx = w - by * a.tl_nt;
+    return false;
+  }
+  bz = w % a.tl_S;
+  const int rem = w / a.tl_S, rt = rem / a.tl_nt;
+  by = a.tl_rt0 + rt;
+  bx = rem - rt * a.tl_nt;
+  return true;
+}
 
 __device__ __forceinline__ void sum_slabs(const float* src, long sstride, int S, float (&v)[8]) {
 #pragma unroll
@@ -234,7 +254,8 @@
 
 template <int NPL, int MT, int WGR, int BNT>
 __device__ __forceinline__ void igemm_write_out(const Args& a, const Phase& ph, f32x4 (&acc)[MT][4], float* lds_f32, int* flag, int z, int phase,
-                                                int tile_id, int bm0, int bm, int bn0, int bn, int wrow, int wcol, int lane, int wave) {
+                                                int tile_id, int bm0, int bm, int bn0, int bn, int wrow, int wcol, int lane, int wave,
+                                                bool tail_slice = false) {
   if (a.skip_out) {
     float keep = 0.f;
 #pragma unroll
@@ -244,8 +265,8 @@
     if (keep == 1.2345678e-30f && a.ws) a.ws[0] = keep;
     return;
   }
-  if (a.splitk > 1) {
-    float* slab = a.ws + (long)z * a.g.M * a.Npad;
+  if (a.splitk > 1 || tail_slice) {
+    float* slab = a.ws + (tail_slice ? (long)z * a.tl_rows - a.tl_row0 : (long)z * a.g.M) * a.Npad;
 #pragma unroll
     for (int m = 0; m < MT; ++m)
 #pragma unroll
@@ -528,7 +549,9 @@
   const int grp = __builtin_amdgcn_readfirstlane(threadIdx.x >> 8);
   const int wrow = BN_ == 128 ? (wave >> 1) * 64 : wave * 32, wcol = BN_ == 128 ? (wave & 1) * 64 : 0;
   int tx, ty, z;
-  xcd_tile(a.xcd, tx, ty, z);
+  bool tail_slice = false;
+  if (a.tl_S) tail_slice = tail_tile(a, tx, ty, z);
+  else xcd_tile(a.xcd, tx, ty, z);
   const int bm = ty * 256 + grp * 128, bn = tx * BN_;
   int phase = 0;
 #pragma unroll
@@ -537,7 +560,8 @@
   const int ks = z - a.zoff[phase];
   const Phase& ph = a.ph[phase];
   const int KC = a.KC, KT = ph.ntaps * KC;
-  const int kt0 = ks * a.per_k, kt1 = min(KT, kt0 + a.per_k);
+  const int per_k = tail_slice ? a.tl_per_k : a.per_k;
+  const int kt0 = ks * per_k, kt1 = min(KT, kt0 + per_k);
   const int nk = max(kt1 - kt0, 0);
   const long Min = (long)a.g.B * a.Hi * a.Wi;
   const long cstride = Min * 32;
@@ -678,7 +702,7 @@
   const unsigned long long probe_c3 = probe ? __builtin_amdgcn_s_memtime() : 0;
   static_assert(4 * 32 * 68 * 4 <= 2 * PP_IMG * 2, "epilogue staging does not fit a group's activation images");
   igemm_write_out<NPL, MT, 256, BN_>(a, ph, acc, reinterpret_cast<float*>(lds_pp + imgA0), reinterpret_cast<int*>(lds_pp), z, phase,
-                                     (phase * gridDim.y + ty) * gridDim.x + tx, ty * 256, bm, bn, bn, wrow, wcol, lane, wave);
+                                     (phase * gridDim.y + ty) * gridDim.x + tx, ty * 256, bm, bn, bn, wrow, wcol, lane, wave, tail_slice);
   if (probe && threadIdx.x == 0) {
     const int wg = (blockIdx.z * gridDim.y + blockIdx.y) * gridDim.x + blockIdx.x;
     if (wg < ufr_clock_probe_cap) {
@@ -948,14 +972,15 @@
 
 __global__ __launch_bounds__(256) void igemm_reduce_kernel(const Args a) {
   const int n8 = a.Npad / 8;
-  const long total = (long)a.nphase * a.g.M * n8;
+  const int rows = a.tl_S ? a.tl_rows : a.g.M, row0 = a.tl_S ? a.tl_row0 : 0;
+  const long total = (long)a.nphase * rows * n8;
   for (long i = (long)blockIdx.x * blockDim.x + threadIdx.x; i < total; i += (long)gridDim.x * blockDim.x) {
     const int n0 = (int)(i % n8) * 8;
     const long rest = i / n8;
-    const int row = (int)(rest % a.g.M), phase = (int)(rest / a.g.M);
+    const int r = (int)(rest % rows), row = row0 + r, phase = (int)(rest / rows);
     if (n0 >= a.e.Nchunks32 * 32) continue;
     float v[8];
-    sum_slabs(a.ws + ((long)a.zoff[phase] * a.g.M + row) * a.Npad + n0, (long)a.g.M * a.Npad, a.sk[phase], v);
+    sum_slabs(a.ws + ((long)a.zoff[phase] * rows + r) * a.Npad + n0, (long)rows * a.Npad, a.tl_S ? a.tl_S : a.sk[phase], v);
     epilogue_store8(a.e, out_pixel(a.g, row, a.ph[phase].oy0, a.ph[phase].ox0), n0, v);
   }
 }
@@ -975,7 +1000,8 @@
 }
 extern "C" int ufr_igemm_variant_fallbacks(void) { return g_variant_fallbacks.load(); }
 
-extern "C" int ufr_igemm(const ufr_igemm_desc* d, ufr_stream_t stream) {
+namespace {
+int igemm_run(const ufr_igemm_desc* d, const ufr_igemm_tail_plan_t* tp, float* tws, ufr_stream_t stream) {
   UFR_REQUIRE(d, "igemm: null descriptor");
   UFR_REQUIRE(d->x && d->w, "igemm: null operand");
   UFR_REQUIRE(d->B > 0 && d->Hi > 0 && d->Wi > 0 && d->Hr > 0 && d->Wr > 0 && d->Ho > 0 && d->Wo > 0, "igemm: bad grid");
@@ -1020,6 +1046,12 @@
   static const int skip_out = [] { const char* e = getenv("UFR_IGEMM_DEBUG_SKIP_EPILOGUE"); return e ? atoi(e) : 0; }();
   a.skip_out = skip_out == 1;
   a.e.nostore = skip_out == 2;
+  a.tl_S = a.tl_full = a.tl_nt = a.tl_rt0 = a.tl_row0 = a.tl_rows = a.tl_per_k = 0;
+  if (tp) {
+    a.tl_S = tp->slices; a.tl_full = tp->full_row_tiles * tp->col_tiles; a.tl_nt = tp->col_tiles; a.tl_rt0 = tp->full_row_tiles;
+    a.tl_row0 = tp->tail_row0; a.tl_rows = tp->tail_rows; a.tl_per_k = tp->slice_ktiles;
+    a.ws = tws;
+  }
   a.xcd = 1;
   a.korder = d->k_order ? 1 : 0;
   for (int z = 0; z < 4; ++z) {
@@ -1119,7 +1151,7 @@
     if (use_buf) igemm_glds_kernel<64, 128, false, true><<<g64, 256, 0, st>>>(a);
     else igemm_glds_kernel<64, 128><<<g64, 256, 0, st>>>(a);
   } else if ((variant == 6 || variant == 7) && bn == BN) {
-    const dim3 gpp(d->Npad / BN, (unsigned)((M + 255) / 256), nz);
+    const dim3 gpp = tp ? dim3(tp->workgroups) : dim3(d->Npad / BN, (unsigned)((M + 255) / 256), nz);
     if (use_buf) igemm_pp_kernel<128, true><<<gpp, 512, pp_lds_bytes(128), st>>>(a);
     else igemm_pp_kernel<128><<<gpp, 512, pp_lds_bytes(128), st>>>(a);
   } else if (variant == 5 && bn == BN) {
@@ -1132,8 +1164,67 @@
     else igemm_glds_kernel<128, 64><<<grid, 256, 0, st>>>(a);
   }
   int rc = ufr::launched("igemm_kernel");
-  if (rc != UFR_OK || d->splitk == 1 || d->no_reduce || a.tickets) return rc;
-  const long total = (long)d->nphase * M * (d->Npad / 8);
+  if (rc != UFR_OK || (!tp && (d->splitk == 1 || d->no_reduce || a.tickets))) return rc;
+  const long total = tp ? (long)tp->tail_rows * (d->Npad / 8) : (long)d->nphase * M * (d->Npad / 8);
   igemm_reduce_kernel<<<ufr::stream_grid(total, 256), 256, 0, st>>>(a);
   return ufr::launched("igemm_reduce_kernel");
 }
+}
+
+extern "C" int ufr_igemm(const ufr_igemm_desc* d, ufr_stream_t stream) { return igemm_run(d, nullptr, nullptr, stream); }
+
+extern "C" int ufr_igemm_tail_plan(const ufr_igemm_desc* d, int resident_workgroups, ufr_igemm_tail_plan_t* plan) {
+  UFR_REQUIRE(d && plan, "igemm tail plan: null argument");
+  UFR_REQUIRE(resident_workgroups >= 0 && resident_workgroups <= (1 << 20), "igemm tail plan: bad resident workgroup count");
+  UFR_REQUIRE(d->B > 0 && d->Hr > 0 && d->Wr > 0 && d->KC > 0 && d->Npad > 0 && d->Npad % 64 == 0 && d->nphase >= 1 && d->nphase <= 4,
+              "igemm tail plan: bad descriptor");
+  const long M = (long)d->B * d->Hr * d->Wr;
+  UFR_REQUIRE(M < (1L << 30), "igemm tail plan: too many pixels");
+  UFR_REQUIRE(d->phase[0].ntaps >= 1 && d->phase[0].ntaps <= UFR_IGEMM_MAX_TAPS && (long)d->phase[0].ntaps * d->KC < (1L << 24),
+              "igemm tail plan: bad phase");
+  *plan = ufr_igemm_tail_plan_t{};
+  const int R = resident_workgroups ? resident_workgroups : 256;
+  const int Mt = (int)((M + 255) / 256), ktiles = d->phase[0].ntaps * d->KC;
+  plan->row_tiles = Mt; plan->ktiles = ktiles;
+  plan->full_row_tiles = Mt;
+  if (d->Npad % 128 != 0 || d->nphase != 1 || d->variant != 6 || d->products != 6 || d->tickets || d->no_reduce || d->tail || d->splitk > 1)
+    return UFR_OK;
+  const int Nt = d->Npad / 128;
+  plan->col_tiles = Nt;
+  const long T = (long)Mt * Nt;
+  const long q = T / R;
+  plan->steps_before = (int)((T + R - 1) / R) * (ktiles + 6);
+  plan->steps_after = plan->steps_before;
+  if (q == 0 || T % R == 0) return UFR_OK;
+  const int full = (int)(q * R / Nt), tail_rt = Mt - full;
+  const long tail_tiles = (long)tail_rt * Nt;
+  long S = R / tail_tiles;
+  if (S > ktiles / 8) S = ktiles / 8;
+  if (S > 8) S = 8;
+  if (S < 2) return UFR_OK;
+  const int per = (int)((ktiles + S - 1) / S);
+  const int after = (int)q * (ktiles + 6) + (per + 6) + 10;
+  if (after > plan->steps_before) return UFR_OK;
+  plan->on = 1;
+  plan->full_row_tiles = full; plan->tail_row_tiles = tail_rt;
+  plan->tail_row0 = full * 256; plan->tail_rows = (int)(M - (long)full * 256);
+  plan->slices = (int)S; plan->slice_ktiles = per;
+  plan->workgroups = (int)((long)full * Nt + tail_tiles * S);
+  plan->ws_floats = S * (long)plan->tail_rows * d->Npad;
+  plan->steps_after = after;
+  return UFR_OK;
+}
+
+extern "C" int ufr_igemm_balanced(const ufr_igemm_desc* d, int resident_workgroups, float* ws, long ws_floats, ufr_stream_t stream) {
+  UFR_REQUIRE(d, "igemm: null descriptor");
+  UFR_REQUIRE(resident_workgroups >= 0, "igemm (balanced): bad resident workgroup count");
+  int R = resident_workgroups, dev = 0;
+  if (!R && (hipGetDevice(&dev) != hipSuccess || hipDeviceGetAttribute(&R, hipDeviceAttributeMultiprocessorCount, dev) != hipSuccess || R < 1))
+    return ufr::fail(UFR_ELAUNCH, "igemm (balanced): no current device");
+  ufr_igemm_tail_plan_t plan;
+  const int rc = ufr_igemm_tail_plan(d, R, &plan);
+  if (rc != UFR_OK) return rc;
+  UFR_REQUIRE(!plan.on || (ws && ws_floats >= plan.ws_floats), "igemm (balanced): workspace of %ld floats needed, %ld given", plan.ws_floats,
+              ws ? ws_floats : 0L);
+  return igemm_run(d, plan.on ? &plan : nullptr, ws, stream);
+}
diff --git a/understanding_flow_robustness_amd/flownetc_engine.py b/understanding_flow_robustness_amd/flownetc_engine.py
--- a/understanding_flow_robustness_amd/flownetc_engine.py
+++ b/understanding_flow_robustness_amd/flownetc_engine.py
@@ -150,7 +150,8 @@
         launches = [ig.make_launch(wi, x, c0, rows, out_hw, splitk=S, ws=self.ws if S > 1 else None, **kw)
                     for wi, x, c0, rows, out_hw, S, kw in plans]
         self.fwd = {k: launches[i] for k, i in fwd.items()}
-        self.bwd = {k: launches[i] for k, i in bwd.items()}
+        self.plain = {}
+        self.bwd = {k: self._with_tail(("full", k), launches[i], plans[i][:5], plans[i][6], plans[i][5]) for k, i in bwd.items()}
         self._plans = {("fwd", k): plans[i] for k, i in fwd.items()}
         self._plans.update({("bwd", k): plans[i] for k, i in bwd.items()})
         self._band, self.fwd_band, self.bwd_band = None, {}, {}
@@ -165,6 +166,21 @@
         self.pf_G = {6: self.G_c6, 5: self.G_cat5, 4: self.G_cat4, 3: self.G_cat3, 2: self.G_cat2}
         self.up_dst = {6: (self.cat5, 32), 5: (self.cat4, 24), 4: (self.cat3, 12), 3: (self.cat2, 6)}
         self.up_G = {6: (self.G_cat5, 32), 5: (self.G_cat4, 24), 4: (self.G_cat3, 12), 3: (self.G_cat2, 6)}
+
+    def _with_tail(self, key, plain, args, kw, S, resident=None):
+        self.plain.pop(key, None)
+        if S != 1 and resident is None:
+            return plain
+        wi, x, c0, rows, out_hw = args
+        launch = ig.make_launch(wi, x, c0, rows, out_hw, ws=self.ws, balance=True, resident=resident, **kw)
+        if launch.tail_plan is None:
+            return plain
+        self.plain[key] = plain
+        return launch
+
+    def tail_launches(self):
+        tables = {"full": self.bwd, "band": self.bwd_band, "rest": self.bwd_rest}
+        return [(tag, name, tables[tag][name].tail_plan) for tag, name in sorted(self.plain)]
 
     def _variant_for(self, wi):
         return self._pipe_variant if wi.Npad % 128 == 0 else 2
@@ -388,12 +404,14 @@
             return
         self._band, self.fwd_band, self.bwd_band = band, {}, {}
         self.bwd_band_wide, self.bwd_rest, self._band_plans, self._pf_band = {}, {}, {}, {}
+        self.plain = {k: v for k, v in self.plain.items() if k[0] == "full"}
         if not band.width:
             return
         W = self.W
         if band.width % 32 or band.width > W:
             raise ValueError("band width must be a multiple of 32 pixels inside the frame")
         origin = band.win[:, 1]
+        resident = getattr(band, "tail_resident", None)
 
         def derive(kind, name, ls_rows, ls_in):
             wi, x, c0, rows, out_hw, S, kw = self._plans[(kind, name)]
@@ -407,7 +425,10 @@
             Sb = ig.splitk_for(M, wi.Npad, max(pk), len(wi.phases), phase_ktiles=pk, bm=bm, target=target)
             if len(wi.phases) * Sb * M * wi.Npad > self.ws.numel():
                 Sb = 1
-            return ig.make_launch(wi, x, c0, rows_b, out_hw, splitk=Sb, ws=self.ws if Sb > 1 else None, **kw, **extra)
+            launch = ig.make_launch(wi, x, c0, rows_b, out_hw, splitk=Sb, ws=self.ws if Sb > 1 else None, **kw, **extra)
+            if kind == "bwd":
+                launch = self._with_tail(("band", name), launch, (wi, x, c0, rows_b, out_hw), dict(kw, **extra), Sb, resident)
+            return launch
 
         for name, (ls_rows, _) in self._FWD_BAND.items():
             if ("fwd", name) in self._plans:
@@ -433,7 +454,9 @@
             if len(wi.phases) * S * M * wi.Npad > self.ws.numel():
                 S = 1
             self._band_plans[name] = (wi, x, c0, rows, out_hw, kw)
-            return ig.make_launch(wi, x, c0, rows, out_hw, splitk=S, ws=self.ws if S > 1 else None, **kw)
+            launch = ig.make_launch(wi, x, c0, rows, out_hw, splitk=S, ws=self.ws if S > 1 else None, **kw)
+            return self._with_tail(("rest" if name.endswith(" rest") else "band", name), launch, (wi, x, c0, rows, out_hw), kw, S,
+                                   getattr(band, "tail_resident", None))
 
         for k, (lead, ls) in self._SPLIT_DECONV.items():
             src, chunk0, _, Gd, _, rows = self.tail_args[k]
@@ -456,7 +479,7 @@
                 raise ValueError("correlation band: a multiple of 8 pixels inside the band")
             for name in ("conv3_1", "conv_redir"):
                 wi, x, c0, rows, out_hw, _, kw = self._plans[("bwd", name)]
-                self.bwd_band_wide[name] = self.bwd_band[name]
+                self.bwd_band_wide[name] = self.plain.get(("band", name), self.bwd_band[name])
                 kw = dict(kw, row_band=(band.win[:, 2], 8, 8), in_band=(origin, 8, 8, band.width // 8))
                 self.bwd_band[name] = planned(name, wi, x, c0, (rows[0], cw // 8), out_hw, kw)
 
@@ -632,9 +655,10 @@
             self._pf_forward(k)
         return self.flow[2]
 
-    def backward(self, g_flow2: torch.Tensor, band=None, fused_window: bool = True, skip_unread: bool = True):
+    def backward(self, g_flow2: torch.Tensor, band=None, fused_window: bool = True, skip_unread: bool = True, tail_split: bool = True):
         L.require_hip(g_flow2, "g_flow2")
         B = self.B
+        run = lambda table, tag, name: (table[name] if tail_split else self.plain.get((tag, name), table[name]))()
         banded = band is not None and bool(band.width)
         if band is not None:
             self.attach_band(band)
@@ -663,12 +687,12 @@
             self._up_backward(k + 1)
             region = None
             if skip and k + 1 in self._pf_band:
-                self.bwd_band[f"deconv{k}"]()
-                self.bwd_rest[f"deconv{k} rest"]()
+                run(self.bwd_band, "band", f"deconv{k}")
+                run(self.bwd_rest, "rest", f"deconv{k} rest")
                 head, ls = self._pf_band[k + 1]
                 region = (head, L.UFR_PF_REGION_BAND, band.win[:, 1], 8, ls, self.grid[ls][0], band.width // ls, 0, None)
             else:
-                self.bwd[f"deconv{k}"]()
+                run(self.bwd, "full", f"deconv{k}")
             self._deconv_tail(k)
             self._pf_backward(k + 1, self.g_flow[k + 1], accumulate=True, finalize=fin(k + 1), region=region)
         Gs, act, out, chunk0, chunks = gz[5]
@@ -677,17 +701,19 @@
         self._up_backward(6)
         self._pf_backward(6, self.g_flow[6], accumulate=False)
         for name in ("deconv5", "conv6_1", "conv6", "conv5_1"):
-            self.bwd[name]()
+            run(self.bwd, "full", name)
         if not self.siamese:
             for name in ("conv5", "conv4_1", "conv4", "conv3_1"):
-                self.bwd[name]()
+                run(self.bwd, "full", name)
             self.G_in31.to_nchw(256, 0, out=self.g_c3a)
             return self.g_c2a, self.g_c3a, None
         for name in ("conv5", "conv4_1", "conv4", "conv3_1", "conv_redir"):
             if banded and not skip and name in self.bwd_band_wide:
                 self.bwd_band_wide[name]()
+            elif banded:
+                run(self.bwd_band, "band", name)
             else:
-                (self.bwd_band if banded else self.bwd)[name]()
+                run(self.bwd, "full", name)
         gw = getattr(band, "g3_window", None) if (band is not None and fused_window) else None
         h8, w8 = self.grid[8]
         if gw is not None and band.cone_win is not None and band.cone_hw[1] // 8 <= 16 and w8 % 4 == 0:
diff --git a/understanding_flow_robustness_amd/igemm.py b/understanding_flow_robustness_amd/igemm.py
--- a/understanding_flow_robustness_amd/igemm.py
+++ b/understanding_flow_robustness_amd/igemm.py
@@ -251,10 +251,15 @@
 
 class Launch:
 
-    def __init__(self, desc, keep):
+    def __init__(self, desc, keep, tail_plan=None, resident=0, tail_ws=None):
         self.desc, self._keep = desc, keep
+        self.tail_plan, self._resident, self._tail_ws = tail_plan, int(resident), tail_ws
 
     def __call__(self):
+        if self.tail_plan is not None:
+            L.check(L.lib().ufr_igemm_balanced(C.byref(self.desc), self._resident, L.ptr(self._tail_ws), self._tail_ws.numel(), L.stream()),
+                    "igemm (balanced)")
+            return
         L.check(L.lib().ufr_igemm(C.byref(self.desc), L.stream()), "igemm")
 
     def algorithmic_bytes(self) -> float:
@@ -339,7 +344,7 @@
                 slope: float = LEAKY, splitk: int = 1, ws: torch.Tensor | None = None, row_band=None, in_band=None,
                 products: int | None = None, variant: int = 0, tail: GradSum | None = None, tail_n0: int = 0, tail_chunk0: int = 0,
                 tail_accumulate: bool = False, out_rowmajor=None, planes_chunks: int = 0, f32_first_chunk: int = 0,
-                no_reduce: bool = False, fuse_reduce: bool | None = None) -> Launch:
+                no_reduce: bool = False, fuse_reduce: bool | None = None, balance: bool = False, resident: int | None = None) -> Launch:
     if RECORD is not None:
         RECORD.append(dict(wi=wi, x=x, in_chunk0=in_chunk0, rows=tuple(rows_hw), out_hw=tuple(out_hw), splitk=splitk, variant=variant,
                            kw=dict(out_planes=out_planes, out_chunk0=out_chunk0, out_f32=out_f32, out_f32_chunk0=out_f32_chunk0, bias=bias,
@@ -421,7 +426,25 @@
     d.products = int(_PRODUCTS[-1] if products is None else products)
     d.k_order = int(wi.k_order)
     d.variant = int(variant)
+    if balance:
+        R = int(resident) if resident else resident_workgroups(x.t.device)
+        plan = tail_plan(d, R)
+        if plan.on:
+            tws = ws if (ws is not None and ws.dtype == torch.float32 and ws.numel() >= plan.ws_floats) else \
+                torch.empty(plan.ws_floats, dtype=torch.float32, device=x.t.device)
+            return Launch(d, keep + [tws], tail_plan=plan, resident=R, tail_ws=tws)
     return Launch(d, keep)
+
+
+def resident_workgroups(device) -> int:
+    device = torch.device(device)
+    return int(torch.cuda.get_device_properties(device).multi_processor_count) if device.type == "cuda" else 256
+
+
+def tail_plan(desc, resident: int = 0) -> "L.IgemmTailPlan":
+    plan = L.IgemmTailPlan()
+    L.check(L.lib().ufr_igemm_tail_plan(C.byref(desc), int(resident), C.byref(plan)), "igemm tail plan")
+    return plan
 
 
 def splitk_for(M: int, Npad: int, ktiles: int, phases: int = 1, target: int = 768, phase_ktiles=None, bm: int = 128,
diff --git a/understanding_flow_robustness_amd/patch_attack.py b/understanding_flow_robustness_amd/patch_attack.py
--- a/understanding_flow_robustness_amd/patch_attack.py
+++ b/understanding_flow_robustness_amd/patch_attack.py
@@ -42,11 +42,12 @@
 
     def __init__(self, flow_net, args, batch, height, width, device="cuda:0", shared_patch=True,
                  exchange: ShardedExchange | None = None, use_graph=True, warmup=3, use_cone=None, patch_hw=None,
-                 sum_groups=1, skip_unread=True, corr_changed=True):
+                 sum_groups=1, skip_unread=True, corr_changed=True, tail_split=True, tail_resident=None):
         L.lib()
         self.net, self.args = flow_net, args
         self.skip_unread = bool(skip_unread)
         self.corr_changed = bool(corr_changed)
+        self.tail_split, self.tail_resident = bool(tail_split), tail_resident
         self.B, self.H, self.W = batch, height, width
         self.dev = torch.device(device)
         self.shared = shared_patch
@@ -231,6 +232,8 @@
                              cone_hw=(wh, ww))
             if bw and corr_band_width(ww) <= bw:
                 self.band.corr_width = corr_band_width(ww)
+            if self.tail_resident:
+                self.band.tail_resident = int(self.tail_resident)
             if bw and os.environ.get("UFR_INCREMENTAL", "1") != "0":
                 self.band.inc_layers = tuple(getattr(self.net, "INCREMENTAL_LAYERS", ()))
 
@@ -311,7 +314,8 @@
                 if self.band is not None:
                     self.band.g3_window, self.band.g3_margin = gw3, m3
                     self.band.eng_window, self.band.g2_margin = True, m2
-                g2a, g3a, g3b = self.eng.backward(g_flow2.contiguous(), self.band, skip_unread=self.skip_unread)
+                g2a, g3a, g3b = self.eng.backward(g_flow2.contiguous(), self.band, skip_unread=self.skip_unread,
+                                                  tail_split=self.tail_split)
                 if g2a is not None:
                     self._win_copy(lib.ufr_window_gather, g2a, gw2, B, 128, H // ls2, W // ls2, ls2, m2)
                 if g3a is not None:
```

New measurement: 1526 (median of 6 runs). 1.01x the previous value.
